# indrajeetadityaroy9/vit-inductive-bias-distillation

Measured on AMD Instinct MI355X. Metric: distillation images/sec (BASD loss fwd+bwd+grad all-reduce), DeiT-S<-ResNet-50 @ bs256/GPU, higher is better.
Workload: dtype f32; 1 GPU; cfg2 DeiT-S<-ResNet-50 224x224; per_gpu_batch=256, global_batch=256, input_dtype=float32, layout=strided (CLS-sliced / channel-major views), backward=True, grad_allreduce_bytes=88202672, grad_allreduce=none at world size 1 (bucket packed, nothing to exchange), rank_readback=auto, readback_deferred_steps=1756, selector=basd_selector_chain mode 0, parallelism=dp1

## Files before the change

### include/basd_hip.h

```cpp
#ifndef BASD_HIP_H
#define BASD_HIP_H

#include <stdint.h>

#ifdef __cplusplus
extern "C" {
#endif

#ifndef __HIP_PLATFORM_AMD__
typedef struct ihipStream_t* hipStream_t;
#endif

#define BASD_OK 0
#define BASD_EINVAL (-1)
#define BASD_EUNSUPPORTED (-2)
#define BASD_DTYPE_F32 0
#define BASD_DTYPE_BF16 1


int basd_gemm_nt(const void* a, int a_dtype, long a_sb, long a_sn, long a_sd, int a_rows_per_batch,
                 long a_batch_stride, const float* b, long ldb, long b_batch_stride, int M, int N, int K, int batch,
                 float* c, long ldc, long c_batch_stride, float scale, const float* bias, float beta,
                 float* colsum_part, float* col_mean, hipStream_t stream);

int basd_gemm_tn_splits(int krows);

int basd_gemm_tn(const void* a, const void* b, int dtype, long a_sb, long a_sn, long a_sd, long a_batch_stride,
                 long b_sb, long b_sn, long b_sd, long b_batch_stride, int rows_per_batch, int krows, int M, int N,
                 int batch, const float* mean_a, const float* mean_b, int splits, float* slabs, float* c, long ldc,
                 long c_batch_stride, float scale, hipStream_t stream);

int basd_colmean_parts(int rows);

int basd_colmean(const void* x, int dtype, long sb, long sn, long sd, int rows_per_batch, long batch_stride,
                 int rows, int cols, int batch, int parts, float* partial, float* mean, hipStream_t stream);

int basd_gemm_tuning(int split_bf16);
int basd_gemm_tuning_get(void);

int basd_colmean_multi(const void* const* x_ptrs, int dtype, long sb, long sn, long sd, int rows_per_batch, int rows,
                       int cols, int n_mats, int parts, float* partial, float* means, int vec_ok,
                       hipStream_t stream);

int basd_syrk_splits(int krows, int cols, int n_mats);

int basd_syrk_multi(const void* const* x_ptrs, int dtype, long sb, long sn, long sd, int rows_per_batch, int krows,
                    int cols, int n_mats, const float* means, const float* scales, int splits, float* slabs,
                    float* out, long out_stride, int vec_ok, const float* fold, int fold_parts, int fold_from,
                    hipStream_t stream);


int basd_jacobi_workspace_ints(int batch, int max_sweeps);
int basd_jacobi_plain4_fits(int n);

int basd_jacobi_tuning(int lanes_per_pair);
int basd_jacobi_ordering(int odd_even);

int basd_jacobi_onesided(float* W, long batch_stride, int rows_dot, int rows_tot, int n, int batch,
                         const int* n_arr, float* colnorm, int colnorm_stride, int max_sweeps, float tol_cos,
                         int* flags, int* sweeps_out, hipStream_t stream);

long basd_jacobi_twopass_workspace_bytes(int n, int batch, int max_sweeps);
int basd_jacobi_stacked_twopass(float* W, long batch_stride, int n, int batch, float* colnorm, int colnorm_stride,
                                int max_sweeps, float tol_cos, void* workspace, int* sweeps_out, hipStream_t stream);

int basd_sort_extract(const float* W, long batch_stride, int rows, int rows_tot, int n, int batch,
                      const float* colnorm, int colnorm_stride, float* vals_desc, float* vecs, int kmax,
                      hipStream_t stream);


long basd_tridiag_workspace_bytes(int n, int batch);

int basd_tridiag(float* a, long a_batch_stride, int n, int batch, float* d, float* e, float* tau, float* vh,
                 void* work, hipStream_t stream);

int basd_tridiag_ranked(float* a, long a_batch_stride, int n, int batch, float* d, float* e, float* tau, float* vh,
                        void* work, int rank_count, double factor, int cap, int* rank_out, int* host_mirror,
                        void* mid_event ,
                        hipStream_t stream);

int basd_tridiag_tuning(int members, int pad, int lag, int threads, int tail, int reset);

int basd_tridiag_eigenvalues(const float* d, const float* e, int n, int batch, float* vals_desc, hipStream_t stream);

int basd_tridiag_apply_q(const float* tau, const float* vh, int n, int k, int batch, const float* x, float* out,
                         int k_stride, int transpose, hipStream_t stream);

int basd_tridiag_shifted_solve(const float* d, const float* e, const float* shifts, int shift_stride, int n, int k,
                               int batch, const float* rhs, float* x, hipStream_t stream);

int basd_tridiag_mp_rank(const float* d, const float* e, int n, int batch, double factor, int cap, int* rank_out,
                         float* thr_out, const int* status, int* host_mirror, hipStream_t stream);

int basd_tridiag_eigenvectors(const float* d, const float* e, const float* tau, const float* vh,
                              const float* vals_desc, int n, int k, int batch, float* z, float* vecs, int k_stride,
                              hipStream_t stream);


int basd_mp_rank(const float* vals_desc, int n, int batch, double factor, int cap, int* rank_out, float* thr_out,
                 hipStream_t stream);

int basd_grassmann_distance(const float* colnorm, int stride, const int* k_arr, const float* sw, int sw_stride,
                            const int* sw_index, int items, float* d_out, float* theta_out, hipStream_t stream);

int basd_grassmann_distance_padded(const float* colnorm, int stride, int n_valid, const int* k_arr, const float* sw,
                                   int sw_stride, const int* sw_index, int items, float* d_out, hipStream_t stream);

int basd_sqrt_clamp(const float* in, float* out, long count, hipStream_t stream);

int basd_gram_finish(const float* c, const float* zbar, int n, int batch, long m_rows, float* out_u, float* out_c,
                     hipStream_t stream);

int basd_selector_tail(const float* t_d, const float* t_e, const float* t_tau, const float* t_vh, const float* t_vals,
                       const float* s_d, const float* s_e, const float* s_tau, const float* s_vh, const float* s_vals,
                       int d_s, int E, int L, int kmax, const int* ranks, const float* proj_s_t, float* z_s,
                       float* v_s, float* z_t, float* u_t, float* u_rot, float* sw, float* cos, int* k_arr,
                       const int* sw_index, float* sigma, int* flags, float* d_out, hipStream_t stream);

int basd_tridiag_mp_rank_rank1(const float* d, const float* e, const float* w, int n, int batch, double rho,
                               double factor, int cap, int* rank_out, const int* status, int* host_mirror,
                               hipStream_t stream);

int basd_tridiag_ranked_gated(float* a, long a_batch_stride, int n, int batch, float* d, float* e, float* tau, float* vh,
                              void* work, int rank_count, double factor, int cap, int* rank_out, int* host_mirror,
                              const unsigned* go_flag, unsigned go_value, int go_budget, hipStream_t stream);
int basd_flag_set(unsigned* flag, unsigned value, hipStream_t stream);

typedef struct BasdSelectorChain {
    const void* const* teacher_host_ptrs;
    long t_dtype, t_sb, t_sn, t_sd;
    const void* const* student_ptrs;
    long s_dtype, s_sb, s_sn, s_sd, s_vec_ok;
    const float* proj_t;
    const float* proj_s_t;
    long E, L, B, n_s, n_t, d_s, d_t;
    double mp_factor;
    long rank_cap;
    long kmax, kmax_cap, mode;
    float* z; float* z_sums; const void* const* z_ptrs; float* z_means; float* t_slabs; long t_splits;
    float* s_partial; float* s_means; float* s_slabs; long s_splits, s_parts;
    float* grams; float* d; float* e; float* tau; float* vh; float* vals; void* tri_work; void* tri_work_s;
    int* ranks; int* host_mirror;
    int* student_status_mirror;
    float* zv; float* vecs; float* u_rot; float* sw; float* cos; float* sigma; float* d_out;
    int* k_arr; const int* sw_index; int* jflags;
    hipStream_t main_stream, chain_stream, student_stream, tail_stream;
    void* ev_fork; void* ev_student; void* ev_ranks; void* ev_tail; void* ev_slot_free; void* ev_tgram; void* ev_tg0;
    long release_delay;
    hipStream_t fact_stream; unsigned* go_flag; long go_value; long go_budget;
    void* tm_proj; void* tm_tgram; void* tm_scol0; void* tm_scol1; void* tm_sgram; void* tm_tri0; void* tm_mid; void* tm_spec;
    hipStream_t cert_stream; int* cert_mirror; void* ev_cert;
    double* cert_scratch;
} BasdSelectorChain;
int basd_selector_chain(const BasdSelectorChain* args);
int basd_rank_certificate(const float* grams, const float* zbar, int n, int batch, double factor, double* scratch,
                          int* flag, hipStream_t stream);
long basd_rank_certificate_scratch_bytes(int batch);
int basd_debug_fill_lds(unsigned pattern, hipStream_t stream);
int basd_selector_chain_tail(const BasdSelectorChain* args, int kmax, int exact_k);
int basd_jacobi_lds_square_fits(int n);


int basd_token_weights(const void* const* attn_ptrs, int dtype, const float* mix, int L, long sb, long sh, long sq,
                       long sk, int B, int H, int A, int has_cls, int n_a, int n_t, int n_s, const int* atap0,
                       const int* atap1, const float* alam, const int* tap0, const int* tap1, const float* lam,
                       float* omega, float* omega_t, float* raw_out, hipStream_t stream);

int basd_student_project(const void* x, int dtype, long sb, long sn, int B, int n_s, int n_t, int D,
                         const float* omega, const int* tap0, const int* tap1, const float* lam, const int* range0,
                         const int* range1, float* mu, float* tr_s, float* a_prime, hipStream_t stream);

int basd_teacher_center(const void* const* tok_ptrs, int dtype, const float* mix, int L, long sb, long sn, long sd,
                        int B, int n, int D, const int* g0, const int* g1, const float* glam, const float* omega_t,
                        float* mu, float* tc, hipStream_t stream);
int basd_teacher_center_multi(const void* const* tok_ptrs, int dtype, const float* mix, int L, int G, long sb, long sn,
                              long sd, int B, int n, int D, const int* g0, const int* g1, const float* glam,
                              const float* omega_t, float* mu, float* tc, hipStream_t stream);
long basd_teacher_center_stream_scratch_floats(int G, int B, int n, int D);
int basd_teacher_center_stream(const void* const* tok_ptrs, int dtype, const float* mix, int L, int G, long sb, long sn,
                               long sd, int B, int n, int D, const int* g0, const int* g1, const float* glam,
                               const float* omega_t, float* mu, float* tc, float* scratch, hipStream_t stream);

int basd_gram_f64(const float* p, long p_batch_stride, int n, int D, int batch, double* g, long g_batch_stride,
                  hipStream_t stream);

int basd_gram_f64_split(const float* p, long p_batch_stride, int n, int D, int batch, int splits, double* slabs,
                        double* g, hipStream_t stream);

int basd_chol_f64(const double* g, long g_batch_stride, int n, int batch, double* l, long l_batch_stride,
                  hipStream_t stream);

int basd_stack_product(const double* la, const double* lb, long l_batch_stride, int n, int batch, int lb_period,
                       float* w, long w_batch_stride, hipStream_t stream);

int basd_procrustes_finalize(const float* w, long w_batch_stride, const float* sigma, int n, int n_s, int batch,
                             int t_period ,
                             const double* gb, long g_batch_stride, const float* omega, const int* tap0,
                             const int* tap1, const float* lam, const float* tr_s_part, int tr_slabs, float* tr_s,
                             float* tr_t, float* nuc, float* loss, float* k_prime, hipStream_t stream);

int basd_student_grad(const void* x, int dtype, long sb, long sn, int B, int n_s, int n_t, int D, const float* omega,
                      const float* mu, const float* h, const int* tap0, const int* tap1, const float* lam,
                      const float* scale_ptr, float scale_const, float* dx, const float* tnorm2, float* gomega,
                      hipStream_t stream);

int basd_student_project_multi(const void* const* x_ptrs, int dtype, long sb, long sn, int E, int B, int n_s, int n_t,
                               int D, int ptrs_16B_aligned, const float* omega, long omega_e_stride, const int* tap0,
                               const int* tap1, const float* lam, const int* range0, const int* range1, float* mu,
                               float* tr_s, float* a_prime, hipStream_t stream);
int basd_student_grad_multi(const void* const* x_ptrs, int dtype, long sb, long sn, int E, int B, int n_s, int n_t,
                            int D, const float* omega, long omega_e_stride, const float* mu, const float* h,
                            const int* tap0, const int* tap1, const float* lam, const float* scale_ptr,
                            float scale_const, float* dx, const float* tnorm2, float* gomega, hipStream_t stream);
int basd_student_grad_fused(const void* const* x_ptrs, int dtype, long sb, long sn, int E, int B, int n_s, int n_t,
                            int D, int ptrs_16B_aligned, const float* omega, long omega_e_stride, const float* mu,
                            const float* k_prime, const float* a_prime, const int* tap0, const int* tap1,
                            const float* lam, const float* scale_ptr, float scale_const, float* dx,
                            hipStream_t stream);

typedef struct BasdProcrustesArgs {
    const void* const* student_ptrs;
    const void* const* student_host_ptrs;
    long s_dtype, s_sb, s_sn, s_aligned;
    const void* const* tok_ptrs;
    long t_dtype, t_sb, t_sn, t_sd;
    const void* const* attn_ptrs;
    long a_dtype, a_sb, a_sh, a_sq, a_sk;
    const float* mix;
    long E, L, G, B, n_s, n_t, d_s, d_t, H, A, has_cls, n_a, n, max_sweeps;
    const int* atap0; const int* atap1; const float* alam;
    const int* tap0; const int* tap1; const float* lam; const int* range0; const int* range1;
    const int* g0; const int* g1; const float* glam;
    float* omega; float* omega_t; float* raw; float* mu_t; float* tc; float* mu_s; float* tr_part; float* tr_s;
    float* a_prime;
    double* g_all; double* l_all;
    float* W; float* sigma; int* jflags; int* sweeps;
    float* tr_t; float* nuc; float* loss_b; float* k_prime;
    float* h; float* dx; const float* grad_layers;
    double* g_slabs; long g_splits;
    const float* uw_ce; float* uw_out;
    void* jac_ws;
    float* w_stack; float* sigma_u;
} BasdProcrustesArgs;
int basd_procrustes_forward_fused(const BasdProcrustesArgs* args, hipStream_t stream);
int basd_procrustes_tuning(int transposed_cores);

int basd_stack_product_t(const double* la, const double* lb, long l_batch_stride, int n, int batch, int lb_period,
                         float* w, long w_batch_stride, hipStream_t stream);
int basd_kprime_from_transposed(const float* w, long w_batch_stride, const float* sigma, int n, int batch,
                                const double* lb, long l_batch_stride, int lb_period, float* z, long z_batch_stride,
                                float* k_prime, hipStream_t stream);
int basd_ustack_stash(const float* wc, long wc_batch_stride, int n, int batch, float* w_stack, long w_stack_stride,
                      hipStream_t stream);
int basd_ustack_from_transposed(const float* x, long x_batch_stride, const float* sigma, int n, int batch,
                                float* w_stack, long w_stack_stride, float* scratch, long scratch_batch_stride,
                                float* sigma_u, int max_sweeps, int* jflags, hipStream_t stream);

int basd_scale_unless_one(float* x, long count, const float* num, const float* den, hipStream_t stream);

int basd_cross_entropy(const void* logits, int dtype, long ld, int B, int C, const long* labels, const float* probs,
                       long pld, float label_smoothing, long ignore_index, float* row_loss, float* dlogits,
                       hipStream_t stream);


int basd_event_create(void** out);
int basd_event_destroy(void* event);
int basd_stream_wait_event(hipStream_t stream, void* event);
int basd_event_record(void* event, hipStream_t stream);
int basd_event_synchronize(void* event);
int basd_event_query(void* event);
int basd_stream_create_priority(void** out, int level);
int basd_event_create_timed(void** out);
int basd_event_elapsed_ms(void* from, void* to, float* ms_out);


int basd_teacher_factor(const float* w, long w_batch_stride, const float* sigma, int n, int n_s, int batch,
                        const double* la, const double* gb, long g_batch_stride, const float* omega,
                        const int* tap0, const int* tap1, const float* lam, const int* range0, const int* range1,
                        float* kt, float* tnorm2, hipStream_t stream);
int basd_teacher_factor_tiled(const float* w, long w_batch_stride, const float* sigma, int n, int n_s, int batch,
                              const double* la, const double* gb, long g_batch_stride, const float* omega,
                              const int* tap0, const int* tap1, const float* lam, const int* range0, const int* range1,
                              float* kt, float* tnorm2, float* z_scratch, hipStream_t stream);

int basd_mix_grad_tokens(const float* r, const void* const* tok_ptrs, int dtype, int L, long sb, long sn, long sd,
                         int E, int B, int n, int D, const int* g0, const int* g1, const float* glam, float* partial,
                         hipStream_t stream);

long basd_mix_grad_tokens_scratch_floats(int E, int B, int L, int n);
int basd_mix_grad_tokens_onepass(const float* r, const void* const* tok_ptrs, int dtype, int L, long sb, long sn, long sd,
                                 int E, int B, int n, int D, const int* g0, const int* g1, const float* glam,
                                 float* partial, float* scratch, hipStream_t stream);

int basd_token_weight_bwd(const float* gomega, const float* raw, int E, int B, int n_a, int n_s, const int* atap0,
                          const int* atap1, const float* alam, const int* arange0, const int* arange1,
                          const void* const* attn_ptrs, int dtype, int L, long sb, long sh, long sq, long sk, int H,
                          int A, int has_cls, float* partial,
                          float* graw_out ,
                          hipStream_t stream);

int basd_build_angle_stack(const float* cos, int kmax, const int* k_arr, int items, float* out, hipStream_t stream);

int basd_grassmann_distance_bwd(const float* stack, const float* colnorm, int kmax, const int* k_arr, const float* sw,
                                int sw_stride, const int* sw_index, const float* gd, int items, float* gwt,
                                hipStream_t stream);

int basd_eigvec_k2(const float* m, const float* lam, int D, int kmax, int batch, float* k2, hipStream_t stream);

int basd_resample_tokens(const void* x, int dtype, long sb, long sn, long sd, int B, int n_in, int n_out, int D,
                         const int* tap0, const int* tap1, const float* lam, float* out, hipStream_t stream);
int basd_resample_tokens_adjoint(const float* dy, int B, int n_in, int n_out, int D, const int* tap0,
                                 const int* tap1, const float* lam, const int* range0, const int* range1, float* dx,
                                 hipStream_t stream);

#ifdef __cplusplus
}
#endif
#endif
```

### vit-inductive-bias-distillation_amd/basd_amd/_lib.py

```python
from __future__ import annotations

import ctypes as C
import os
import threading

_HERE = os.path.dirname(os.path.abspath(__file__))
LIB_PATH = os.path.join(_HERE, "libbasd_hip.so")

vp, i32, i64, f32, f64 = C.c_void_p, C.c_int, C.c_long, C.c_float, C.c_double

SIGNATURES = {
    "basd_gemm_nt": [vp, i32, i64, i64, i64, i32, i64, vp, i64, i64, i32, i32, i32, i32, vp, i64, i64, f32, vp, f32,
                     vp, vp, vp],
    "basd_gemm_tn_splits": [i32],
    "basd_gemm_tn": [vp, vp, i32, i64, i64, i64, i64, i64, i64, i64, i64, i32, i32, i32, i32, i32, vp, vp, i32, vp,
                     vp, i64, i64, f32, vp],
    "basd_colmean_parts": [i32],
    "basd_colmean": [vp, i32, i64, i64, i64, i32, i64, i32, i32, i32, i32, vp, vp, vp],
    "basd_colmean_multi": [vp, i32, i64, i64, i64, i32, i32, i32, i32, i32, vp, vp, i32, vp],
    "basd_syrk_splits": [i32, i32, i32],
    "basd_syrk_multi": [vp, i32, i64, i64, i64, i32, i32, i32, i32, vp, vp, i32, vp, vp, i64, i32, vp, i32, i32, vp],
    "basd_jacobi_workspace_ints": [i32, i32],
    "basd_jacobi_twopass_workspace_bytes": [i32, i32, i32],
    "basd_jacobi_stacked_twopass": [vp, i64, i32, i32, vp, i32, i32, f32, vp, vp, vp],
    "basd_jacobi_tuning": [i32],
    "basd_jacobi_ordering": [i32],
    "basd_gemm_tuning": [i32],
    "basd_gemm_tuning_get": [],
    "basd_jacobi_onesided": [vp, i64, i32, i32, i32, i32, vp, vp, i32, i32, f32, vp, vp, vp],
    "basd_sort_extract": [vp, i64, i32, i32, i32, i32, vp, i32, vp, vp, i32, vp],
    "basd_tridiag_workspace_bytes": [i32, i32],
    "basd_tridiag_tuning": [i32, i32, i32, i32, i32, i32],
    "basd_tridiag": [vp, i64, i32, i32, vp, vp, vp, vp, vp, vp],
    "basd_tridiag_ranked": [vp, i64, i32, i32, vp, vp, vp, vp, vp, i32, f64, i32, vp, vp, vp, vp],
    "basd_tridiag_ranked_gated": [vp, i64, i32, i32, vp, vp, vp, vp, vp, i32, f64, i32, vp, vp, vp, C.c_uint, i32, vp],
    "basd_flag_set": [vp, C.c_uint, vp],
    "basd_scale_unless_one": [vp, i64, vp, vp, vp],
    "basd_event_create": [vp],
    "basd_event_destroy": [vp],
    "basd_stream_wait_event": [vp, vp],
    "basd_tridiag_eigenvalues": [vp, vp, i32, i32, vp, vp],
    "basd_tridiag_apply_q": [vp, vp, i32, i32, i32, vp, vp, i32, i32, vp],
    "basd_tridiag_shifted_solve": [vp, vp, vp, i32, i32, i32, i32, vp, vp, vp],
    "basd_tridiag_mp_rank": [vp, vp, i32, i32, f64, i32, vp, vp, vp, vp, vp],
    "basd_tridiag_mp_rank_rank1": [vp, vp, vp, i32, i32, f64, f64, i32, vp, vp, vp, vp],
    "basd_tridiag_eigenvectors": [vp, vp, vp, vp, vp, i32, i32, i32, vp, vp, i32, vp],
    "basd_mp_rank": [vp, i32, i32, f64, i32, vp, vp, vp],
    "basd_grassmann_distance": [vp, i32, vp, vp, i32, vp, i32, vp, vp, vp],
    "basd_grassmann_distance_padded": [vp, i32, i32, vp, vp, i32, vp, i32, vp, vp],
    "basd_selector_tail": [vp] * 10 + [i32, i32, i32, i32] + [vp] * 14 + [vp],
    "basd_sqrt_clamp": [vp, vp, i64, vp],
    "basd_gram_finish": [vp, vp, i32, i32, i64, vp, vp, vp],
    "basd_cross_entropy": [vp, i32, i64, i32, i32, vp, vp, i64, f32, i64, vp, vp, vp],
    "basd_token_weights": [vp, i32, vp, i32, i64, i64, i64, i64, i32, i32, i32, i32, i32, i32, i32, vp, vp, vp, vp,
                           vp, vp, vp, vp, vp, vp],
    "basd_student_project": [vp, i32, i64, i64, i32, i32, i32, i32, vp, vp, vp, vp, vp, vp, vp, vp, vp, vp],
    "basd_teacher_center": [vp, i32, vp, i32, i64, i64, i64, i32, i32, i32, vp, vp, vp, vp, vp, vp, vp],
    "basd_teacher_center_multi": [vp, i32, vp, i32, i32, i64, i64, i64, i32, i32, i32, vp, vp, vp, vp, vp, vp, vp],
    "basd_teacher_center_stream_scratch_floats": [i32, i32, i32, i32],
    "basd_teacher_center_stream": [vp, i32, vp, i32, i32, i64, i64, i64, i32, i32, i32, vp, vp, vp, vp, vp, vp, vp, vp],
    "basd_gram_f64": [vp, i64, i32, i32, i32, vp, i64, vp],
    "basd_gram_f64_split": [vp, i64, i32, i32, i32, i32, vp, vp, vp],
    "basd_chol_f64": [vp, i64, i32, i32, vp, i64, vp],
    "basd_stack_product": [vp, vp, i64, i32, i32, i32, vp, i64, vp],
    "basd_procrustes_finalize": [vp, i64, vp, i32, i32, i32, i32, vp, i64, vp, vp, vp, vp, vp, i32, vp, vp, vp, vp,
                                 vp, vp],
    "basd_student_project_multi": [vp, i32, i64, i64, i32, i32, i32, i32, i32, i32, vp, i64, vp, vp, vp, vp, vp, vp,
                                   vp, vp, vp],
    "basd_student_grad_multi": [vp, i32, i64, i64, i32, i32, i32, i32, i32, vp, i64, vp, vp, vp, vp, vp, vp, f32, vp,
                                vp, vp, vp],
    "basd_student_grad_fused": [vp, i32, i64, i64, i32, i32, i32, i32, i32, i32, vp, i64, vp, vp, vp, vp, vp, vp, vp,
                                f32, vp, vp],
    "basd_procrustes_forward_fused": [vp, vp],
    "basd_procrustes_tuning": [i32],
    "basd_jacobi_plain4_fits": [i32],
    "basd_stack_product_t": [vp, vp, i64, i32, i32, i32, vp, i64, vp],
    "basd_kprime_from_transposed": [vp, i64, vp, i32, i32, vp, i64, i32, vp, i64, vp, vp],
    "basd_ustack_stash": [vp, i64, i32, i32, vp, i64, vp],
    "basd_ustack_from_transposed": [vp, i64, vp, i32, i32, vp, i64, vp, i64, vp, i32, vp, vp],
    "basd_resample_tokens": [vp, i32, i64, i64, i64, i32, i32, i32, i32, vp, vp, vp, vp, vp],
    "basd_resample_tokens_adjoint": [vp, i32, i32, i32, i32, vp, vp, vp, vp, vp, vp, vp],
    "basd_student_grad": [vp, i32, i64, i64, i32, i32, i32, i32, vp, vp, vp, vp, vp, vp, vp, f32, vp, vp, vp, vp],
    "basd_teacher_factor": [vp, i64, vp, i32, i32, i32, vp, vp, i64, vp, vp, vp, vp, vp, vp, vp, vp, vp],
    "basd_teacher_factor_tiled": [vp, i64, vp, i32, i32, i32, vp, vp, i64, vp, vp, vp, vp, vp, vp, vp, vp, vp, vp],
    "basd_mix_grad_tokens": [vp, vp, i32, i32, i64, i64, i64, i32, i32, i32, i32, vp, vp, vp, vp, vp],
    "basd_mix_grad_tokens_scratch_floats": [i32, i32, i32, i32],
    "basd_mix_grad_tokens_onepass": [vp, vp, i32, i32, i64, i64, i64, i32, i32, i32, i32, vp, vp, vp, vp, vp, vp],
    "basd_token_weight_bwd": [vp, vp, i32, i32, i32, i32, vp, vp, vp, vp, vp, vp, i32, i32, i64, i64, i64, i64, i32,
                              i32, i32, vp, vp, vp],
    "basd_build_angle_stack": [vp, i32, vp, i32, vp, vp],
    "basd_grassmann_distance_bwd": [vp, vp, i32, vp, vp, i32, vp, vp, i32, vp, vp],
    "basd_eigvec_k2": [vp, vp, i32, i32, i32, vp, vp],
    "basd_selector_chain": [vp],
    "basd_rank_certificate": [vp, vp, i32, i32, f64, vp, vp, vp],
    "basd_rank_certificate_scratch_bytes": [i32],
    "basd_debug_fill_lds": [C.c_uint, vp],
    "basd_selector_chain_tail": [vp, i32, i32],
    "basd_jacobi_lds_square_fits": [i32],
    "basd_event_record": [vp, vp],
    "basd_event_synchronize": [vp],
    "basd_event_query": [vp],
    "basd_stream_create_priority": [vp, i32],
    "basd_event_create_timed": [vp],
    "basd_event_elapsed_ms": [vp, vp, vp],
}

class ProcrustesArgs(C.Structure):
    _PTRS = ("student_ptrs", "student_host_ptrs")
    _fields_ = (
        [("student_ptrs", vp), ("student_host_ptrs", vp)]
        + [(n, i64) for n in ("s_dtype", "s_sb", "s_sn", "s_aligned")]
        + [("tok_ptrs", vp)] + [(n, i64) for n in ("t_dtype", "t_sb", "t_sn", "t_sd")]
        + [("attn_ptrs", vp)] + [(n, i64) for n in ("a_dtype", "a_sb", "a_sh", "a_sq", "a_sk")]
        + [("mix", vp)]
        + [(n, i64) for n in ("E", "L", "G", "B", "n_s", "n_t", "d_s", "d_t", "H", "A", "has_cls", "n_a", "n",
                              "max_sweeps")]
        + [(n, vp) for n in ("atap0", "atap1", "alam", "tap0", "tap1", "lam", "range0", "range1", "g0", "g1", "glam",
                             "omega", "omega_t", "raw", "mu_t", "tc", "mu_s", "tr_part", "tr_s", "a_prime", "g_all",
                             "l_all", "W", "sigma", "jflags", "sweeps", "tr_t", "nuc", "loss_b", "k_prime", "h", "dx",
                             "grad_layers", "g_slabs")]
        + [("g_splits", i64)]
        + [("uw_ce", vp), ("uw_out", vp), ("jac_ws", vp), ("w_stack", vp), ("sigma_u", vp)]
    )


class SelectorChainArgs(C.Structure):
    _fields_ = (
        [("teacher_host_ptrs", vp)] + [(n, i64) for n in ("t_dtype", "t_sb", "t_sn", "t_sd")]
        + [("student_ptrs", vp)] + [(n, i64) for n in ("s_dtype", "s_sb", "s_sn", "s_sd", "s_vec_ok")]
        + [("proj_t", vp), ("proj_s_t", vp)]
        + [(n, i64) for n in ("E", "L", "B", "n_s", "n_t", "d_s", "d_t")]
        + [("mp_factor", f64)]
        + [(n, i64) for n in ("rank_cap", "kmax", "kmax_cap", "mode")]
        + [(n, vp) for n in ("z", "z_sums", "z_ptrs", "z_means", "t_slabs")] + [("t_splits", i64)]
        + [(n, vp) for n in ("s_partial", "s_means", "s_slabs")] + [("s_splits", i64), ("s_parts", i64)]
        + [(n, vp) for n in ("grams", "d", "e", "tau", "vh", "vals", "tri_work", "tri_work_s", "ranks", "host_mirror",
                             "student_status_mirror", "zv", "vecs", "u_rot", "sw", "cos", "sigma", "d_out", "k_arr",
                             "sw_index", "jflags", "main_stream", "chain_stream", "student_stream", "tail_stream",
                             "ev_fork", "ev_student", "ev_ranks", "ev_tail", "ev_slot_free", "ev_tgram", "ev_tg0",
                             "release_delay", "fact_stream", "go_flag", "go_value", "go_budget",
                             "tm_proj", "tm_tgram", "tm_scol0", "tm_scol1", "tm_sgram", "tm_tri0", "tm_mid", "tm_spec",
                             "cert_stream", "cert_mirror", "ev_cert", "cert_scratch")]
    )


EINVAL, EUNSUPPORTED = -1, -2

LONG_RESULTS = {"basd_tridiag_workspace_bytes", "basd_jacobi_twopass_workspace_bytes",
                "basd_mix_grad_tokens_scratch_floats", "basd_teacher_center_stream_scratch_floats",
                "basd_rank_certificate_scratch_bytes"}

_lock = threading.Lock()
_lib = None


def load() -> C.CDLL:
    global _lib
    if _lib is not None:
        return _lib
    with _lock:
        if _lib is None:
            if not os.path.exists(LIB_PATH):
                raise RuntimeError(
                    f"{LIB_PATH} not found: build it with `make -C vit-inductive-bias-distillation_amd/csrc` "
                    "(or `python -c 'import __graft_entry__ as g; g.build()'`). There is no CPU fallback.")
            lib = C.CDLL(LIB_PATH)
            for name, argtypes in SIGNATURES.items():
                fn = getattr(lib, name)
                fn.argtypes = argtypes
                fn.restype = C.c_long if name in LONG_RESULTS else C.c_int
            _lib = lib
    return _lib


timing: dict | None = None
timed_names: set | None = None


def call(name: str, *args) -> None:
    if timing is not None and (timed_names is None or name in timed_names):
        import torch
        e0 = torch.cuda.Event(enable_timing=True)
        e1 = torch.cuda.Event(enable_timing=True)
        e0.record()
        status = getattr(load(), name)(*args)
        e1.record()
        timing.setdefault(name, []).append((e0, e1))
    else:
        status = getattr(load(), name)(*args)
    if status != 0:
        kind = "invalid argument / unsupported shape" if status < 0 else "HIP error"
        raise RuntimeError(f"{name} failed with status {status} ({kind})")


def query(name: str, *args) -> int:
    return int(getattr(load(), name)(*args))
```

### vit-inductive-bias-distillation_amd/basd_amd/ops.py

```python
from __future__ import annotations

from dataclasses import dataclass
from functools import lru_cache

import torch

from . import _lib

import os

F32, BF16 = 0, 1
MAX_SWEEPS = 20
TWO_PASS_SVD = True
TRANSPOSED_MIX_GRAD = True
TWO_PASS_LOG_LIMIT = 16 << 30
EIG_SOLVER = os.environ.get("BASD_EIG_SOLVER", "tridiag")
if os.environ.get("BASD_GEMM_SPLIT") in ("0", "1"):
    _lib.call("basd_gemm_tuning", int(os.environ["BASD_GEMM_SPLIT"]))
if os.environ.get("BASD_JACOBI_ORDERING") in ("0", "1"):
    _lib.call("basd_jacobi_ordering", int(os.environ["BASD_JACOBI_ORDERING"]))


def _stream() -> int:
    return torch._C._cuda_getCurrentRawStream(torch._C._cuda_getDevice())


def _dtype_code(t: torch.Tensor) -> int:
    if t.dtype == torch.float32:
        return F32
    if t.dtype == torch.bfloat16:
        return BF16
    raise TypeError(f"unsupported dtype {t.dtype}")


def as_supported(t: torch.Tensor) -> torch.Tensor:
    if t.dtype in (torch.float32, torch.bfloat16):
        return t
    return t.float()


def _require_cuda(*tensors: torch.Tensor) -> None:
    for t in tensors:
        if not t.is_cuda:
            raise RuntimeError("basd_amd kernels need CUDA/HIP tensors (there is no CPU fallback)")


def _ptr(t: torch.Tensor | None) -> int | None:
    return None if t is None else t.data_ptr()


HOST_TRACE: list | None = None
CHAIN_EVENTS: list = []


def trace(label: str) -> None:
    if HOST_TRACE is not None:
        import time
        HOST_TRACE.append((label, time.perf_counter()))


GPU_MARKS: list | None = None


def gpu_mark(label: str) -> None:
    if GPU_MARKS is not None:
        ev = torch.cuda.Event(enable_timing=True)
        ev.record()
        GPU_MARKS.append((label, ev))


def _tok3(x: torch.Tensor) -> tuple[int, int, int, int, int, int]:
    if x.dim() == 2:
        return x.data_ptr(), _dtype_code(x), 0, x.stride(0), x.stride(1), 1 << 30
    assert x.dim() == 3
    return x.data_ptr(), _dtype_code(x), x.stride(0), x.stride(1), x.stride(2), x.shape[1]


def gemm_nt(a: torch.Tensor, b: torch.Tensor, *, scale: float = 1.0, out: torch.Tensor | None = None,
            a_batch_stride: int = 0, b_batch_stride: int = 0, batch: int = 1, rows: int | None = None,
            n_cols: int | None = None, bias: torch.Tensor | None = None, beta: float = 0.0,
            col_mean: bool = False, mean_out: torch.Tensor | None = None, col_sums: torch.Tensor | None = None):
    _require_cuda(a, b)
    ptr, dt, sb, sn, sd, rpb = _tok3(a)
    M = rows if rows is not None else (a.shape[0] * a.shape[1] if a.dim() == 3 else a.shape[0])
    K = a.shape[-1]
    N = n_cols if n_cols is not None else b.shape[-2]
    assert b.dtype == torch.float32 and b.stride(-1) == 1 and b.shape[-1] == K
    ldb = b.stride(-2)
    if out is None:
        out = torch.empty((batch, M, N) if batch > 1 else (M, N), device=a.device, dtype=torch.float32)
    part = mean = None
    tiles = gemm_nt_row_tiles(M, N, K, batch, beta)
    if col_sums is not None:
        assert col_sums.is_contiguous() and col_sums.numel() == batch * tiles * N
        part = col_sums
    if col_mean:
        part = torch.empty((batch, tiles, N), device=a.device, dtype=torch.float32)
        mean = mean_out if mean_out is not None else \
            torch.empty((batch, N) if batch > 1 else (N,), device=a.device, dtype=torch.float32)
        assert mean.dtype == torch.float32 and mean.is_contiguous() and mean.numel() == batch * N
    _lib.call("basd_gemm_nt", ptr, dt, sb, sn, sd, rpb, a_batch_stride, b.data_ptr(), ldb, b_batch_stride,
              M, N, K, batch, out.data_ptr(), N, M * N, scale, _ptr(bias), beta, _ptr(part), _ptr(mean), _stream())
    return (out, mean) if col_mean else out


def gemm_nt_row_tiles(M: int, N: int, K: int, batch: int = 1, beta: float = 0.0) -> int:
    return (M + 127) // 128


def gemm_tn(a: torch.Tensor, b: torch.Tensor, *, mean_a: torch.Tensor | None = None,
            mean_b: torch.Tensor | None = None, scale: float = 1.0, batch: int = 1, a_batch_stride: int = 0,
            b_batch_stride: int = 0, krows: int | None = None, m_cols: int | None = None,
            n_cols: int | None = None, split: bool = True) -> torch.Tensor:
    _require_cuda(a, b)
    pa, dt, asb, asn, asd, rpb = _tok3(a)
    pb, dtb, bsb, bsn, bsd, rpb_b = _tok3(b)
    assert dt == dtb and rpb == rpb_b
    kr = krows if krows is not None else (a.shape[0] * a.shape[1] if a.dim() == 3 else a.shape[0])
    M = m_cols if m_cols is not None else a.shape[-1]
    N = n_cols if n_cols is not None else b.shape[-1]
    splits = _lib.query("basd_gemm_tn_splits", kr) if (split and batch == 1) else 1
    out = torch.empty((batch, M, N) if batch > 1 else (M, N), device=a.device, dtype=torch.float32)
    slabs = torch.empty((batch * splits, M, N), device=a.device, dtype=torch.float32) if splits > 1 else None
    _lib.call("basd_gemm_tn", pa, pb, dt, asb, asn, asd, a_batch_stride, bsb, bsn, bsd, b_batch_stride, rpb, kr, M, N,
              batch, _ptr(mean_a), _ptr(mean_b), splits, _ptr(slabs), out.data_ptr(), N, M * N, scale, _stream())
    return out


def colmean(x: torch.Tensor) -> torch.Tensor:
    _require_cuda(x)
    ptr, dt, sb, sn, sd, rpb = _tok3(x)
    rows = x.shape[0] * x.shape[1] if x.dim() == 3 else x.shape[0]
    cols = x.shape[-1]
    parts = _lib.query("basd_colmean_parts", rows)
    partial = torch.empty((parts, cols), device=x.device, dtype=torch.float32)
    mean = torch.empty((cols,), device=x.device, dtype=torch.float32)
    _lib.call("basd_colmean", ptr, dt, sb, sn, sd, rpb, 0, rows, cols, 1, parts, partial.data_ptr(),
              mean.data_ptr(), _stream())
    return mean


def _gram_layout(xs: list[torch.Tensor]):
    _require_cuda(*xs)
    ptr, dt, sb, sn, sd, rpb = _tok3(xs[0])
    for x in xs[1:]:
        assert _tok3(x)[1:] == (dt, sb, sn, sd, rpb) and x.shape == xs[0].shape, "Gram operands must share a layout"
    rows = xs[0].shape[0] * xs[0].shape[1] if xs[0].dim() == 3 else xs[0].shape[0]
    vec_ok = int(all(x.data_ptr() % 16 == 0 for x in xs))
    return (dt, sb, sn, sd, rpb), rows, xs[0].shape[-1], vec_ok


_COLMEAN_SCRATCH: dict = {}


def column_means(xs: list[torch.Tensor], out: torch.Tensor | None = None) -> torch.Tensor:
    (dt, sb, sn, sd, rpb), rows, cols, vec_ok = _gram_layout(xs)
    n, dev = len(xs), xs[0].device
    table = _ptr_table(xs)
    if out is None:
        means = torch.empty((n, cols), device=dev, dtype=torch.float32)
    else:
        assert out.dtype == torch.float32 and out.is_contiguous() and out.numel() == n * cols and out.device == dev
        means = out
    parts = _lib.query("basd_colmean_parts", rows)
    key = (n, parts, cols, dev, _stream())
    partial = _COLMEAN_SCRATCH.get(key)
    if partial is None:
        if len(_COLMEAN_SCRATCH) >= 16:
            _COLMEAN_SCRATCH.clear()
        partial = _COLMEAN_SCRATCH[key] = torch.empty((n, parts, cols), device=dev, dtype=torch.float32)
    _lib.call("basd_colmean_multi", table.data_ptr(), dt, sb, sn, sd, rpb, rows, cols, n, parts, partial.data_ptr(),
              means.data_ptr(), vec_ok, _stream())
    return means.view(n, cols)


def centered_grams(xs: list[torch.Tensor], *, centered: list[bool] | None = None,
                   scales: list[float] | None = None, out: torch.Tensor | None = None,
                   splits: int | None = None, means: torch.Tensor | None = None,
                   fold: tuple[torch.Tensor, int] | None = None) -> tuple[torch.Tensor, torch.Tensor]:
    (dt, sb, sn, sd, rpb), rows, cols, vec_ok = _gram_layout(xs)
    n, dev = len(xs), xs[0].device
    table = _ptr_table(xs)
    if fold is not None:
        part, fold_from = fold
        assert part.is_contiguous() and part.dtype == torch.float32 and part.shape[0] == n - fold_from
        means_used = None
        centered = None
    elif means is None:
        means = column_means(xs)
    if fold is not None:
        pass
    elif centered is not None and not all(centered):
        keep = _device_consts(tuple(1.0 if c else 0.0 for c in centered), torch.float32, dev)
        means_used = means * keep.unsqueeze(1)
    else:
        means_used = means
    sc = None
    if scales is not None:
        sc = _device_consts(tuple(float(s) for s in scales), torch.float32, dev)
    if splits is None:
        splits = _lib.query("basd_syrk_splits", rows, cols, n)
    slabs = torch.empty((n * splits, cols, cols), device=dev, dtype=torch.float32)
    if out is None:
        out = torch.empty((n, cols, cols), device=dev, dtype=torch.float32)
    assert out.dtype == torch.float32 and out.shape == (n, cols, cols) and out[0].is_contiguous()
    _lib.call("basd_syrk_multi", table.data_ptr(), dt, sb, sn, sd, rpb, rows, cols, n, _ptr(means_used),
              _ptr(sc), splits, slabs.data_ptr(), out.data_ptr(), out.stride(0), vec_ok,
              _ptr(fold[0]) if fold is not None else None, fold[0].shape[1] if fold is not None else 0,
              fold[1] if fold is not None else 0, _stream())
    return out, means


def jacobi_onesided(W: torch.Tensor, rows_dot: int, *, n_arr: torch.Tensor | None = None,
                    want_sweeps: bool = False, tol: float = 0.0):
    _require_cuda(W)
    assert W.dtype == torch.float32 and W.is_contiguous() and W.dim() == 3
    batch, n, rows_tot = W.shape
    colnorm = torch.empty((batch, n), device=W.device, dtype=torch.float32)
    flags = torch.empty((_lib.query("basd_jacobi_workspace_ints", batch, MAX_SWEEPS),), device=W.device,
                        dtype=torch.int32)
    sweeps = torch.zeros((batch,), device=W.device, dtype=torch.int32) if want_sweeps else None
    _lib.call("basd_jacobi_onesided", W.data_ptr(), n * rows_tot, rows_dot, rows_tot, n, batch, _ptr(n_arr),
              colnorm.data_ptr(), n, MAX_SWEEPS, tol, flags.data_ptr(), _ptr(sweeps), _stream())
    return (colnorm, sweeps) if want_sweeps else colnorm


def sym_eig(G: torch.Tensor, kmax: int = 0) -> tuple[torch.Tensor, torch.Tensor | None, torch.Tensor, torch.Tensor]:
    assert G.dim() == 3 and G.shape[1] == G.shape[2]
    colnorm = jacobi_onesided(G, G.shape[1])
    vals, vecs = sort_extract(G, colnorm, kmax)
    return vals, vecs, G, colnorm


@dataclass
class TridiagState:
    d: torch.Tensor
    e: torch.Tensor
    tau: torch.Tensor
    vh: torch.Tensor
    vals: torch.Tensor
    err: torch.Tensor | None = None
    ranks: torch.Tensor | None = None


def tridiag_slice(ts: TridiagState, first: int, count: int) -> TridiagState:
    sl = slice(first, first + count)
    return TridiagState(ts.d[sl], ts.e[sl], ts.tau[sl], ts.vh[sl], ts.vals[sl], ts.err, None)


def tridiagonalise(G: torch.Tensor, mp_rank: tuple | None = None) -> TridiagState:
    _require_cuda(G)
    assert G.dtype == torch.float32 and G.is_contiguous() and G.dim() == 3 and G.shape[1] == G.shape[2]
    batch, n, _ = G.shape
    f32 = dict(device=G.device, dtype=torch.float32)
    d, e, tau = (torch.empty((batch, n), **f32) for _ in range(3))
    vh = torch.empty((batch, n, n), **f32)
    vals = torch.empty((batch, n), **f32)
    work = torch.empty((_lib.query("basd_tridiag_workspace_bytes", n, batch),), device=G.device, dtype=torch.uint8)
    ranks = None
    if mp_rank is None:
        _lib.call("basd_tridiag", G.data_ptr(), n * n, n, batch, d.data_ptr(), e.data_ptr(), tau.data_ptr(),
                  vh.data_ptr(), work.data_ptr(), _stream())
    else:
        M, D, cap, count, mirror, mid_event = (tuple(mp_rank) + (None,))[:6]
        factor = (1 + (D / M) ** 0.5) ** 2
        ranks = torch.empty((count,), device=G.device, dtype=torch.int32)
        if mirror is not None:
            assert mirror.is_pinned() and mirror.dtype == torch.int32 and mirror.numel() == count + 8
        _lib.call("basd_tridiag_ranked", G.data_ptr(), n * n, n, batch, d.data_ptr(), e.data_ptr(), tau.data_ptr(),
                  vh.data_ptr(), work.data_ptr(), count, factor, cap, ranks.data_ptr(), _ptr(mirror), mid_event,
                  _stream())
    return TridiagState(d, e, tau, vh, vals, work[-32:].view(torch.int32), ranks)


def new_event() -> int:
    import ctypes
    h = ctypes.c_void_p()
    _lib.call("basd_event_create", ctypes.byref(h))
    return h.value


def stream_wait_event(stream: "torch.cuda.Stream", event: int) -> None:
    _lib.call("basd_stream_wait_event", stream.cuda_stream, event)


def tridiag_spectrum(ts: TridiagState, first: int = 0, count: int | None = None) -> torch.Tensor:
    batch, n = ts.vals.shape
    count = batch - first if count is None else count
    _lib.call("basd_tridiag_eigenvalues", ts.d[first].data_ptr(), ts.e[first].data_ptr(), n, count,
              ts.vals[first].data_ptr(), _stream())
    return ts.vals[first:first + count]


def tridiag_mp_rank(ts: TridiagState, M: int, D: int, cap: int, first: int = 0, count: int | None = None,
                    host_mirror: torch.Tensor | None = None) -> torch.Tensor:
    batch, n = ts.vals.shape
    count = batch - first if count is None else count
    factor = (1 + (D / M) ** 0.5) ** 2
    out = torch.empty((count,), device=ts.d.device, dtype=torch.int32)
    if host_mirror is not None:
        assert host_mirror.is_pinned() and host_mirror.dtype == torch.int32 and host_mirror.numel() == count + 8
    _lib.call("basd_tridiag_mp_rank", ts.d[first].data_ptr(), ts.e[first].data_ptr(), n, count, factor, cap,
              out.data_ptr(), None, _ptr(ts.err) if host_mirror is not None else None, _ptr(host_mirror), _stream())
    return out


def tridiag_mp_rank_rank1(ts: TridiagState, w: torch.Tensor, M: int, D: int, cap: int,
                          host_mirror: torch.Tensor | None = None) -> torch.Tensor:
    batch, n = ts.d.shape
    assert w.dtype == torch.float32 and w.is_contiguous() and w.numel() == batch * n
    factor = (1 + (D / M) ** 0.5) ** 2
    out = torch.empty((batch,), device=ts.d.device, dtype=torch.int32)
    if host_mirror is not None:
        assert host_mirror.is_pinned() and host_mirror.dtype == torch.int32 and host_mirror.numel() == batch + 8
    _lib.call("basd_tridiag_mp_rank_rank1", ts.d.data_ptr(), ts.e.data_ptr(), w.data_ptr(), n, batch, float(M), factor,
              cap, out.data_ptr(), _ptr(ts.err) if host_mirror is not None else None, _ptr(host_mirror), _stream())
    return out


def tridiag_eigenvalues(G: torch.Tensor) -> TridiagState:
    ts = tridiagonalise(G)
    tridiag_spectrum(ts)
    return ts
# ... 468 lines not shown
```

### vit-inductive-bias-distillation_amd/csrc/basd_common.h

```cpp
#pragma once
#include <hip/hip_runtime.h>
#include <hip/hip_bf16.h>
#include <stdint.h>

#define BASD_OK 0
#define BASD_EINVAL (-1)
#define BASD_EUNSUPPORTED (-2)

#define BASD_DTYPE_F32 0
#define BASD_DTYPE_BF16 1

#define BASD_CHECK_ARG(cond) \
    do {                     \
        if (!(cond)) return BASD_EINVAL; \
    } while (0)

#define BASD_RETURN_LAST()                         \
    do {                                           \
        hipError_t e_ = hipGetLastError();         \
        return e_ == hipSuccess ? BASD_OK : (int)e_; \
    } while (0)

namespace basd {

constexpr int kWave = 64;

__device__ __forceinline__ float to_f32(float x) { return x; }
__device__ __forceinline__ float to_f32(__hip_bfloat16 x) { return __bfloat162float(x); }
#define BASD_GLOBAL_AS __attribute__((address_space(1)))
__device__ __forceinline__ float ldg_f32(const BASD_GLOBAL_AS float* p) { return *p; }
__device__ __forceinline__ float ldg_f32(const BASD_GLOBAL_AS __hip_bfloat16* p) {
    return __uint_as_float((unsigned)*(const BASD_GLOBAL_AS unsigned short*)p << 16);
}

template <typename T>
__device__ __forceinline__ T group_sum(T v, int width) {
    for (int m = width >> 1; m > 0; m >>= 1) v += __shfl_xor(v, m, width);
    return v;
}

template <int CTRL>
__device__ __forceinline__ float dpp_get(float x) {
    return __int_as_float(__builtin_amdgcn_update_dpp(0, __float_as_int(x), CTRL, 0xF, 0xF, true));
}
__device__ __forceinline__ float row16_allsum(float x) {
    x += dpp_get<0xB1>(x);
    x += dpp_get<0x4E>(x);
    x += dpp_get<0x141>(x);
    x += dpp_get<0x140>(x);
    return x;
}
__device__ __forceinline__ float wave64_allsum(float x) {
    x = row16_allsum(x);
    auto r = __builtin_amdgcn_permlane16_swap(__float_as_uint(x), __float_as_uint(x), false, false);
    x = __uint_as_float(r[0]) + __uint_as_float(r[1]);
    auto q = __builtin_amdgcn_permlane32_swap(__float_as_uint(x), __float_as_uint(x), false, false);
    return __uint_as_float(q[0]) + __uint_as_float(q[1]);
}

__device__ __forceinline__ float wave_sum(float v) { return wave64_allsum(v); }
__device__ __forceinline__ int wave_sum(int v) { return group_sum(v, kWave); }
__device__ __forceinline__ double wave_sum(double v) { return group_sum(v, kWave); }

__device__ __forceinline__ float wave_max(float v) {
    for (int m = 32; m > 0; m >>= 1) v = fmaxf(v, __shfl_xor(v, m, kWave));
    return v;
}

template <typename T>
__device__ __forceinline__ T block_sum(T v, T* scratch) {
    const int lane = threadIdx.x & 63, wid = threadIdx.x >> 6, nw = (blockDim.x + 63) >> 6;
    v = wave_sum(v);
    __syncthreads();
    if (lane == 0) scratch[wid] = v;
    __syncthreads();
    T r = T(0);
    for (int i = 0; i < nw; ++i) r += scratch[i];
    return r;
}

struct TokView {
    const void* ptr;
    long sb, sn, sd;
    int n_tok;
};

__host__ __device__ __forceinline__ long tok_row_offset(const TokView& v, long m) {
    const long b = m / v.n_tok, n = m - b * v.n_tok;
    return b * v.sb + n * v.sn;
}

__host__ __device__ __forceinline__ void rr_pair(int n_even, int r, int t, int& p, int& q) {
    const int m = n_even - 1;
    if (t == 0) { p = r; q = m; return; }
    p = (r + t) % m;
    q = (r - t + m) % m;
}

}
```

### vit-inductive-bias-distillation_amd/csrc/fused.hip

```cpp
#include "basd_common.h"
#include "../../include/basd_hip.h"

namespace basd {

__global__ void __launch_bounds__(256) uwso_combine_kernel(const float* __restrict__ ce, const float* __restrict__ loss_b,
                                                           int E, int B, float* __restrict__ out) {
    constexpr int CH = 32;
    __shared__ double red[CH][4];
    const int tid = threadIdx.x;
    double geo_sum = 0.;
    for (int e0 = 0; e0 < E; e0 += CH) {
        const int ne = E - e0 < CH ? E - e0 : CH;
        for (int e = 0; e < ne; ++e) {
            double acc = 0.;
            for (int b = tid; b < B; b += 256) acc += (double)loss_b[(long)(e0 + e) * B + b];
            for (int m = 32; m > 0; m >>= 1) acc += __shfl_xor(acc, m, 64);
            if ((tid & 63) == 0) red[e][tid >> 6] = acc;
        }
        __syncthreads();
        if (tid == 0)
            for (int e = 0; e < ne; ++e) {
                const float layer = (float)(((red[e][0] + red[e][1]) + (red[e][2] + red[e][3])) / (double)B);
                out[4 + E + e0 + e] = layer;
                geo_sum += (double)layer;
            }
        __syncthreads();
    }
    if (tid == 0) {
        const float c = ce[0], geo = (float)(geo_sum / (double)E);
        const float eps = 1.1920929e-7f;
        const float i0 = 1.f / fmaxf(c, eps), i1 = 1.f / fmaxf(geo, eps);
        const float w0 = i0 / (i0 + i1), w1 = i1 / (i0 + i1);
        out[0] = w0;
        out[1] = w1;
        out[2] = w0 * c + w1 * geo;
        out[3] = geo;
        for (int e = 0; e < E; ++e) out[4 + e] = w1 / (float)E;
    }
}

__global__ void __launch_bounds__(256) scale_unless_one_kernel(float* __restrict__ x, long count4, long count,
                                                               const float* __restrict__ num,
                                                               const float* __restrict__ den) {
    const float f = den ? num[0] / den[0] : num[0];
    if (f == 1.f) return;
    const long i = (long)blockIdx.x * 256 + threadIdx.x;
    if (i < count4) {
        float4 v = ((float4*)x)[i];
        v.x *= f; v.y *= f; v.z *= f; v.w *= f;
        ((float4*)x)[i] = v;
    }
    if (blockIdx.x == 0 && threadIdx.x < (int)(count - 4 * count4)) x[4 * count4 + threadIdx.x] *= f;
}

}

extern "C" {

int basd_scale_unless_one(float* x, long count, const float* num, const float* den, hipStream_t stream) {
    BASD_CHECK_ARG(x && num && count > 0 && ((uintptr_t)x & 15) == 0);
    const long count4 = count / 4;
    basd::scale_unless_one_kernel<<<(unsigned)((count4 + 255) / 256 + (count4 == 0)), 256, 0, stream>>>(x, count4, count, num, den);
    BASD_RETURN_LAST();
}

static int procrustes_tail(const BasdProcrustesArgs* a, const float* grad_layers, int E, int B, int n_s, int n, int d_s,
                           int EB, long nn, long om_stride, hipStream_t st) {
    int rc;
#define BASD_TRY(call)            \
    do {                          \
        rc = (call);              \
        if (rc != BASD_OK) return rc; \
    } while (0)
    if (a->uw_ce) {
        BASD_CHECK_ARG(a->uw_out != nullptr);
        basd::uwso_combine_kernel<<<1, 256, 0, st>>>(a->uw_ce, a->loss_b, E, B, a->uw_out);
        grad_layers = a->uw_out + 4;
    }
    if (a->dx) {
        BASD_CHECK_ARG(a->k_prime && a->h && grad_layers);
        rc = basd_student_grad_fused(a->student_ptrs, (int)a->s_dtype, a->s_sb, a->s_sn, E, B, n_s, n, d_s,
                                     (int)a->s_aligned, a->omega, om_stride, a->mu_s, a->k_prime, a->a_prime, a->tap0,
                                     a->tap1, a->lam, grad_layers, 2.0f / (float)B, a->dx, st);
        if (rc != BASD_EUNSUPPORTED) return rc;
        BASD_TRY(basd_gemm_tn(a->k_prime, a->a_prime, BASD_DTYPE_F32, 0, n, 1, nn, 0, d_s, 1, (long)n * d_s, 1 << 30, n,
                              n, d_s, EB, nullptr, nullptr, 1, nullptr, a->h, d_s, (long)n * d_s, 1.f, st));
        BASD_TRY(basd_student_grad_multi(a->student_ptrs, (int)a->s_dtype, a->s_sb, a->s_sn, E, B, n_s, n, d_s, a->omega,
                                         om_stride, a->mu_s, a->h, a->tap0, a->tap1, a->lam, grad_layers,
                                         2.0f / (float)B, a->dx, nullptr, nullptr, st));
    }
#undef BASD_TRY
    return BASD_OK;
}

static int g_transposed_cores = 1;
int basd_procrustes_tuning(int transposed_cores) {
    if (transposed_cores >= 0) g_transposed_cores = transposed_cores > 2 ? 2 : transposed_cores;
    return BASD_OK;
}

int basd_procrustes_forward_fused(const BasdProcrustesArgs* a, hipStream_t st) {
    BASD_CHECK_ARG(a && a->student_ptrs && a->tok_ptrs && a->attn_ptrs && a->mix);
    const int E = (int)a->E, L = (int)a->L, G = (int)a->G, B = (int)a->B, n_s = (int)a->n_s, n_t = (int)a->n_t;
    const int d_s = (int)a->d_s, d_t = (int)a->d_t, H = (int)a->H, A = (int)a->A, n_a = (int)a->n_a, n = (int)a->n;
    const float* grad_layers_in = a->grad_layers;
    BASD_CHECK_ARG(E > 0 && L > 0 && (G == 1 || G == E) && B > 0 && n == (n_s < n_t ? n_s : n_t));
    int rc;
#define BASD_TRY(call)            \
    do {                          \
        rc = (call);              \
        if (rc != BASD_OK) return rc; \
    } while (0)
    int centred = BASD_EUNSUPPORTED;
    for (int g = 0; g < G; ++g) {
        BASD_TRY(basd_token_weights(a->attn_ptrs, (int)a->a_dtype, a->mix + (long)g * L, L, a->a_sb, a->a_sh, a->a_sq,
                                    a->a_sk, B, H, A, (int)a->has_cls, n_a, n, n_s, a->atap0, a->atap1, a->alam,
                                    a->tap0, a->tap1, a->lam, a->omega + (long)g * B * n_s,
                                    a->omega_t + (long)g * B * n, a->raw ? a->raw + (long)g * B * n_a : nullptr, st));
    }
    if (G > 1 && L >= 4 && basd_teacher_center_stream_scratch_floats(G, B, n, d_t) <= (long)E * B * 2 * n * n) {
        centred = basd_teacher_center_stream(a->tok_ptrs, (int)a->t_dtype, a->mix, L, G, a->t_sb, a->t_sn, a->t_sd, B, n,
                                             d_t, a->g0, a->g1, a->glam, a->omega_t, a->mu_t, a->tc, a->W, st);
        if (centred != BASD_OK && centred != BASD_EUNSUPPORTED) return centred;
    }
    if (G > 1 && centred != BASD_OK) {
        centred = basd_teacher_center_multi(a->tok_ptrs, (int)a->t_dtype, a->mix, L, G, a->t_sb, a->t_sn, a->t_sd, B, n,
                                            d_t, a->g0, a->g1, a->glam, a->omega_t, a->mu_t, a->tc, st);
        if (centred != BASD_OK && centred != BASD_EUNSUPPORTED) return centred;
    }
    for (int g = 0; g < G && centred != BASD_OK; ++g) {
        BASD_TRY(basd_teacher_center(a->tok_ptrs, (int)a->t_dtype, a->mix + (long)g * L, L, a->t_sb, a->t_sn, a->t_sd,
                                     B, n, d_t, a->g0, a->g1, a->glam, a->omega_t + (long)g * B * n,
                                     a->mu_t + (long)g * B * d_t, a->tc + (long)g * B * n * d_t, st));
    }
    const long om_stride = G == 1 ? 0 : (long)B * n_s;
    int slabs = (d_s + 31) / 32;
    rc = basd_student_project_multi(a->student_ptrs, (int)a->s_dtype, a->s_sb, a->s_sn, E, B, n_s, n, d_s,
                                    (int)a->s_aligned, a->omega, om_stride, a->tap0, a->tap1, a->lam, a->range0,
                                    a->range1, a->mu_s, a->tr_part, a->a_prime, st);
    if (rc == BASD_EUNSUPPORTED) {
        slabs = (d_s + 63) / 64;
        for (int e = 0; e < E; ++e)
            BASD_TRY(basd_student_project(a->student_host_ptrs[e], (int)a->s_dtype, a->s_sb, a->s_sn, B, n_s, n, d_s,
                                          a->omega + e * om_stride, a->tap0, a->tap1, a->lam, a->range0, a->range1,
                                          a->mu_s + (long)e * B * d_s, a->tr_part + (long)e * B * slabs,
                                          a->a_prime + (long)e * B * n * d_s, st));
    } else if (rc != BASD_OK) {
        return rc;
    }
    const long nn = (long)n * n;
    const int EB = E * B, GB = G * B;
    BASD_TRY(basd_gram_f64(a->a_prime, (long)n * d_s, n, d_s, EB, a->g_all, nn, st));
    if (a->g_slabs && a->g_splits > 1)
        BASD_TRY(basd_gram_f64_split(a->tc, (long)n * d_t, n, d_t, GB, (int)a->g_splits, a->g_slabs,
                                     a->g_all + (long)EB * nn, st));
    else
        BASD_TRY(basd_gram_f64(a->tc, (long)n * d_t, n, d_t, GB, a->g_all + (long)EB * nn, nn, st));
    BASD_TRY(basd_chol_f64(a->g_all, nn, n, EB + GB, a->l_all, nn, st));
    if ((a->raw == nullptr || a->w_stack != nullptr) && EB <= 65535 && basd_jacobi_plain4_fits(n) &&
        (g_transposed_cores == 2 || (g_transposed_cores == 1 && EB >= 128))) {
        BASD_TRY(basd_stack_product_t(a->l_all, a->l_all + (long)EB * nn, nn, n, EB, GB, a->W, 2 * nn, st));
        if (a->raw != nullptr) BASD_TRY(basd_ustack_stash(a->W, 2 * nn, n, EB, a->w_stack, 2 * nn, st));
        BASD_TRY(basd_jacobi_onesided(a->W, 2 * nn, n, n, n, EB, nullptr, a->sigma, n, (int)a->max_sweeps, 0.f,
                                      a->jflags, a->sweeps, st));
        BASD_TRY(basd_procrustes_finalize(a->W, 2 * nn, a->sigma, n, n_s, EB, GB, a->g_all + (long)EB * nn, nn, a->omega,
                                          a->tap0, a->tap1, a->lam, a->tr_part, slabs, a->tr_s, a->tr_t, a->nuc,
                                          a->loss_b, nullptr, st));
        if (a->k_prime)
            BASD_TRY(basd_kprime_from_transposed(a->W, 2 * nn, a->sigma, n, EB, a->l_all + (long)EB * nn, nn, GB,
                                                 a->W + nn, 2 * nn, a->k_prime, st));
        if (a->raw != nullptr) {
            BASD_CHECK_ARG(a->sigma_u != nullptr);
            BASD_TRY(basd_ustack_from_transposed(a->W, 2 * nn, a->sigma, n, EB, a->w_stack, 2 * nn, a->W + nn, 2 * nn,
                                                 a->sigma_u, (int)a->max_sweeps, a->jflags, st));
        }
        return procrustes_tail(a, grad_layers_in, E, B, n_s, n, d_s, EB, nn, om_stride, st);
    }
    BASD_TRY(basd_stack_product(a->l_all, a->l_all + (long)EB * nn, nn, n, EB, GB, a->W, 2 * nn, st));
    rc = BASD_EUNSUPPORTED;
    if (a->jac_ws)
        rc = basd_jacobi_stacked_twopass(a->W, 2 * nn, n, EB, a->sigma, n, (int)a->max_sweeps, 0.f, a->jac_ws, a->sweeps,
                                         st);
    if (rc == BASD_EUNSUPPORTED)
        rc = basd_jacobi_onesided(a->W, 2 * nn, n, 2 * n, n, EB, nullptr, a->sigma, n, (int)a->max_sweeps, 0.f,
                                  a->jflags, a->sweeps, st);
    if (rc != BASD_OK) return rc;
    BASD_TRY(basd_procrustes_finalize(a->W, 2 * nn, a->sigma, n, n_s, EB, GB, a->g_all + (long)EB * nn, nn, a->omega,
                                      a->tap0, a->tap1, a->lam, a->tr_part, slabs, a->tr_s, a->tr_t, a->nuc,
                                      a->loss_b, a->k_prime, st));
    return procrustes_tail(a, grad_layers_in, E, B, n_s, n, d_s, EB, nn, om_stride, st);
#undef BASD_TRY
}


int basd_event_create(void** out) {
    BASD_CHECK_ARG(out);
    hipError_t e = hipEventCreateWithFlags((hipEvent_t*)out, hipEventDisableTiming);
    return e == hipSuccess ? BASD_OK : (int)e;
}
int basd_event_destroy(void* ev) {
    hipError_t e = hipEventDestroy((hipEvent_t)ev);
    return e == hipSuccess ? BASD_OK : (int)e;
}
int basd_stream_wait_event(hipStream_t stream, void* ev) {
    BASD_CHECK_ARG(ev);
    hipError_t e = hipStreamWaitEvent(stream, (hipEvent_t)ev, 0);
    return e == hipSuccess ? BASD_OK : (int)e;
}

}
```

### vit-inductive-bias-distillation_amd/csrc/jacobi.hip

```cpp
#include "basd_common.h"

namespace basd {

constexpr float kNull2 = 2.2737368e-13f;

struct Rot {
    float c, s, t;
    float h;
    bool apply;
    bool strong;
};

__device__ __forceinline__ Rot make_rotation(float alpha, float beta, float gamma, float tol) {
    Rot r{1.f, 0.f, 0.f, 0.f, false, false};
    const float cosv = gamma * __builtin_amdgcn_rsqf(alpha) * __builtin_amdgcn_rsqf(beta);
    if (!(fabsf(cosv) > tol)) return r;
    r.strong = cosv * cosv > tol;
    const float zeta = (beta - alpha) * __builtin_amdgcn_rcpf(2.f * gamma);
    const float az = fabsf(zeta);
    float t = az > 1e8f ? 0.5f * __builtin_amdgcn_rcpf(az)
                        : __builtin_amdgcn_rcpf(az + __builtin_amdgcn_sqrtf(fmaf(zeta, zeta, 1.f)));
    t = copysignf(t, zeta);
    r.t = t;
    r.c = __builtin_amdgcn_rsqf(fmaf(t, t, 1.f));
    r.s = r.c * t;
    const float pc = r.c * r.c, ec = fmaf(r.c, r.c, -pc);
    const float ps = r.s * r.s, es = fmaf(r.s, r.s, -ps);
    r.h = 0.5f * ((((1.f - pc) - ps) - ec) - es);
    r.apply = true;
    return r;
}

template <int LPP>
__device__ __forceinline__ float pair_allsum(float x) {
    static_assert(LPP == 4 || LPP == 8 || LPP == 16 || LPP == 32 || LPP == 64,
                  "a pair is owned by a quad, half a DPP row, a row, two rows or a wave");
    if constexpr (LPP == 4 || LPP == 8) {
        x += dpp_get<0xB1>(x);
        x += dpp_get<0x4E>(x);
        if constexpr (LPP == 8) x += dpp_get<0x141>(x);
        return x;
    } else if constexpr (LPP == 32) {
        x = row16_allsum(x);
        auto r = __builtin_amdgcn_permlane16_swap(__float_as_uint(x), __float_as_uint(x), false, false);
        return __uint_as_float(r[0]) + __uint_as_float(r[1]);
    } else {
        return LPP == 16 ? row16_allsum(x) : wave64_allsum(x);
    }
}

typedef float f32x2 __attribute__((ext_vector_type(2)));

template <int EPL, int DOT, int LPP, bool LOG = false>
__device__ __forceinline__ int rotate_pair(float* __restrict__ cp, float* __restrict__ cq, int gl, float tol,
                                            float null2, float& norm2_max, float* __restrict__ n2p,
                                            float* __restrict__ n2q, float* __restrict__ devp,
                                            float* __restrict__ devq, f32x2* __restrict__ logp = nullptr) {
    static_assert(EPL % 2 == 0 && DOT % 2 == 0, "row chunks come in pairs");
    constexpr int H = EPL / 2, HD = DOT / 2;
    f32x2 x[HD], y[HD];
    f32x2 acc = {0.f, 0.f};
#pragma unroll
    for (int i = 0; i < HD; ++i) {
        x[i] = *(const f32x2*)(cp + 2 * gl + 2 * LPP * i);
        y[i] = *(const f32x2*)(cq + 2 * gl + 2 * LPP * i);
        acc = __builtin_elementwise_fma(x[i], y[i], acc);
    }
    const float g = pair_allsum<LPP>(acc.x + acc.y);
    const float a = *n2p, b = *n2q;
    norm2_max = fmaxf(norm2_max, fmaxf(a, b));
    if (fminf(a, b) <= null2) {
        if (LOG && gl == 0) *logp = f32x2{1.f, 0.f};
        return 0;
    }
    const Rot rot = make_rotation(a, b, g, tol);
    if (!rot.apply) {
        if (LOG && gl == 0) *logp = f32x2{1.f, 0.f};
        return 0;
    }
    const f32x2 c2 = {rot.c, rot.c}, s2 = {rot.s, rot.s};
#pragma unroll
    for (int i = 0; i < HD; ++i) {
        *(f32x2*)(cp + 2 * gl + 2 * LPP * i) = __builtin_elementwise_fma(c2, x[i], -(s2 * y[i]));
        *(f32x2*)(cq + 2 * gl + 2 * LPP * i) = __builtin_elementwise_fma(s2, x[i], c2 * y[i]);
    }
#pragma unroll
    for (int i = HD; i < H; ++i) {
        const f32x2 xr = *(const f32x2*)(cp + 2 * gl + 2 * LPP * i);
        const f32x2 yr = *(const f32x2*)(cq + 2 * gl + 2 * LPP * i);
        *(f32x2*)(cp + 2 * gl + 2 * LPP * i) = __builtin_elementwise_fma(c2, xr, -(s2 * yr));
        *(f32x2*)(cq + 2 * gl + 2 * LPP * i) = __builtin_elementwise_fma(s2, xr, c2 * yr);
    }
    if (gl == 0) {
        *n2p = fmaxf(a - rot.t * g, 0.f);
        *n2q = b + rot.t * g;
        *devp += rot.h;
        *devq += rot.h;
        if (LOG) *logp = f32x2{rot.c, rot.s};
    }
    return rot.strong ? 3 : 1;
}

template <int DOT, int LPP>
__device__ __forceinline__ float column_norm2(const float* __restrict__ col, int gl) {
    f32x2 acc = {0.f, 0.f};
#pragma unroll
    for (int i = 0; i < DOT / 2; ++i) {
        const f32x2 v = *(const f32x2*)(col + 2 * gl + 2 * LPP * i);
        acc = __builtin_elementwise_fma(v, v, acc);
    }
    return pair_allsum<LPP>(acc.x + acc.y);
}

template <int EPL, int DOT, int LPP>
__device__ __forceinline__ int lds_row(int r, int rows_dot) {
    return (DOT == EPL || r < rows_dot) ? r : LPP * DOT + (r - rows_dot);
}

template <int EPL, int DOT, int LPP = 16>
__global__ void __launch_bounds__((LPP == 4 && EPL >= 48) ? 512 : 1024) jacobi_lds_kernel(float* __restrict__ W, long batch_stride, int rows_dot,
                                                           int rows_tot, int n_fixed, const int* __restrict__ n_arr,
                                                           int max_sweeps, float tol, float* __restrict__ colnorm,
                                                           int colnorm_stride, int* __restrict__ sweeps_out) {
    constexpr int LD = LPP * EPL + (LPP == 4 ? (((LPP * EPL / 8) % 2 == 0) ? 8 : 0) : LPP == 8 ? 16 : 2);
    static_assert(LPP != 4 || ((LD / 8) % 2 == 1 && LD % 8 == 0), "stride must come out as 8 x odd");
    static_assert(LPP != 8 || ((LPP * EPL / 16) % 2 == 0), "stride must come out as 16 x odd");
    extern __shared__ __attribute__((aligned(16))) float lds[];
    const int m = blockIdx.x;
    int n = n_arr ? n_arr[m] : n_fixed;
    int rd = rows_dot, rt = rows_tot;
    if (n_arr) {
        rd = n;
        rt = n;
    }
    float* Wm = W + (long)m * batch_stride;
    const int tid = threadIdx.x, nthr = blockDim.x;
    if (n <= 0) {
        if (sweeps_out && tid == 0) sweeps_out[m] = 0;
        return;
    }
    const int n_even = (n + 1) & ~1;
    for (int idx = tid; idx < n_even * LD; idx += nthr) lds[idx] = 0.f;
    __syncthreads();
    for (int idx = tid; idx < n * rt; idx += nthr) {
        const int c = idx / rt, r = idx - c * rt;
        lds[c * LD + lds_row<EPL, DOT, LPP>(r, rd)] = Wm[(long)c * rows_tot + r];
    }
    __syncthreads();

    const int groups = nthr / LPP, grp = tid / LPP, gl = tid % LPP;
    float* n2 = lds + n_even * LD;
    float* dev = n2 + n_even;
    __shared__ int s_norm2_bits;
    if (tid == 0) s_norm2_bits = 0;
    for (int c = tid; c < n_even; c += nthr) dev[c] = 0.f;
    float null2 = 0.f;
    int sweep = 0;
    for (; sweep < max_sweeps && n > 1; ++sweep) {
        int rotated = 0;
        float norm2_max = 0.f;
        for (int c = grp; c < n_even; c += groups) {
            const float v = column_norm2<DOT, LPP>(lds + c * LD, gl);
            if (gl == 0) n2[c] = v;
        }
        __syncthreads();
        for (int r = 0; r < n_even - 1; ++r) {
            for (int t = grp; t < n_even / 2; t += groups) {
                int p, q;
                rr_pair(n_even, r, t, p, q);
                if (p >= n || q >= n) continue;
                if (p > q) { const int tmp = p; p = q; q = tmp; }
                rotated |= rotate_pair<EPL, DOT, LPP>(lds + p * LD, lds + q * LD, gl, tol, null2, norm2_max, n2 + p, n2 + q,
                                                 dev + p, dev + q);
            }
            __syncthreads();
        }
        if (gl == 0 && norm2_max > 0.f) atomicMax(&s_norm2_bits, __float_as_int(norm2_max));
        if (!__syncthreads_or(rotated & 2)) {
            ++sweep;
            break;
        }
        null2 = kNull2 * __int_as_float(s_norm2_bits);
    }
    if (sweeps_out && tid == 0) sweeps_out[m] = sweep;

    for (int c = grp; c < n; c += groups) {
        const float a = column_norm2<DOT, LPP>(lds + c * LD, gl);
        if (gl == 0) {
            const float nv = sqrtf(a);
            colnorm[(long)m * colnorm_stride + c] = fmaf(nv, dev[c], nv);
        }
    }
    for (int idx = tid; idx < n * rt; idx += nthr) {
        const int c = idx / rt, r = idx - c * rt;
        const float v = lds[c * LD + lds_row<EPL, DOT, LPP>(r, rd)];
        Wm[(long)c * rows_tot + r] = fmaf(v, dev[c], v);
    }
}

template <int H>
__device__ __forceinline__ int rotate_regs(f32x2 (&x)[H], f32x2 (&y)[H], float& a, float& b, float& dx, float& dy,
                                           float tol, float null2, float& norm2_max, bool forced) {
    f32x2 acc = {0.f, 0.f};
#pragma unroll
    for (int i = 0; i < H; ++i) acc = __builtin_elementwise_fma(x[i], y[i], acc);
    const float g = pair_allsum<4>(acc.x + acc.y);
    norm2_max = fmaxf(norm2_max, fmaxf(a, b));
    Rot rot{1.f, 0.f, 0.f, 0.f, false, false};
    if (fminf(a, b) > null2) rot = make_rotation(a, b, g, tol);
    float c = rot.c, s = rot.s;
    if (forced) { c = 0.f; s = 1.f; }
    if (rot.apply || forced) {
        const f32x2 c2 = {c, c}, s2 = {s, s};
#pragma unroll
        for (int i = 0; i < H; ++i) {
            const f32x2 xi = x[i], yi = y[i];
            x[i] = __builtin_elementwise_fma(c2, xi, -(s2 * yi));
            y[i] = __builtin_elementwise_fma(s2, xi, c2 * yi);
        }
    }
    if (forced) {
        b = a; a = 0.f; dy = dx; dx = 0.f;
    } else if (rot.apply) {
        a = fmaxf(a - rot.t * g, 0.f);
        b = b + rot.t * g;
        dx += rot.h;
        dy += rot.h;
    }
    return rot.strong ? 3 : (rot.apply ? 1 : 0);
}

template <int EPL>
__global__ void __launch_bounds__(512, 4) jacobi_oe_kernel(float* __restrict__ W, long batch_stride, int rows, int n,
                                                           int max_sweeps, float tol, float* __restrict__ colnorm,
                                                           int colnorm_stride, int* __restrict__ sweeps_out) {
    static_assert(EPL % 2 == 0, "row chunks come in pairs");
    constexpr int H = EPL / 2;
    constexpr int LD = 4 * EPL + (((4 * EPL / 8) % 2 == 0) ? 8 : 0);
    extern __shared__ __attribute__((aligned(16))) float lds[];
    const int m = blockIdx.x, tid = threadIdx.x, nthr = blockDim.x;
    const int n_even = (n + 1) & ~1, G = n_even / 2;
    float* mail_n2 = lds + (G + 1) * LD;
    float* mail_dev = mail_n2 + (G + 1);
    __shared__ int s_norm2_bits;
    float* Wm = W + (long)m * batch_stride;
    const int g = tid >> 2, gl = tid & 3;
    const bool active = g < G, last = g == G - 1;
    for (int idx = tid; idx < (G + 1) * (LD + 2); idx += nthr) lds[idx] = 0.f;
    if (tid == 0) s_norm2_bits = 0;

    f32x2 x[H], y[H];
    float a = 0.f, b = 0.f, dx = 0.f, dy = 0.f;
#pragma unroll
    for (int i = 0; i < H; ++i) {
        const int r = 2 * gl + 8 * i;
        const int cx = 2 * g, cy = 2 * g + 1;
        x[i].x = (active && cx < n && r < rows) ? Wm[(long)cx * rows + r] : 0.f;
        x[i].y = (active && cx < n && r + 1 < rows) ? Wm[(long)cx * rows + r + 1] : 0.f;
        y[i].x = (active && cy < n && r < rows) ? Wm[(long)cy * rows + r] : 0.f;
        y[i].y = (active && cy < n && r + 1 < rows) ? Wm[(long)cy * rows + r + 1] : 0.f;
    }
    float* slot_lo = lds + (active ? g : 0) * LD + 2 * gl;
    float* slot_hi = lds + (active ? g + 1 : 0) * LD + 2 * gl;
    __syncthreads();

    float null2 = 0.f;
    int sweep = 0;
    for (; sweep < max_sweeps && n > 1; ++sweep) {
        int rotated = 0;
        float norm2_max = 0.f;
        if (active) {
            f32x2 sa = {0.f, 0.f}, sb = {0.f, 0.f};
#pragma unroll
            for (int i = 0; i < H; ++i) {
                sa = __builtin_elementwise_fma(x[i], x[i], sa);
                sb = __builtin_elementwise_fma(y[i], y[i], sb);
            }
            a = pair_allsum<4>(sa.x + sa.y);
            b = pair_allsum<4>(sb.x + sb.y);
        }
        for (int dr = 0; dr < G; ++dr) {
            if (active) {
                rotated |= rotate_regs<H>(x, y, a, b, dx, dy, tol, null2, norm2_max, false);
#pragma unroll
                for (int i = 0; i < H; ++i) *(f32x2*)(slot_lo + 8 * i) = y[i];
                if (gl == 0) { mail_n2[g] = b; mail_dev[g] = dy; }
            }
            __syncthreads();
            if (active) {
#pragma unroll
                for (int i = 0; i < H; ++i) y[i] = *(const f32x2*)(slot_hi + 8 * i);
                b = mail_n2[g + 1];
                dy = mail_dev[g + 1];
                rotated |= rotate_regs<H>(x, y, a, b, dx, dy, tol, null2, norm2_max, last);
                if (!last) {
#pragma unroll
                    for (int i = 0; i < H; ++i) *(f32x2*)(slot_hi + 8 * i) = x[i];
                    if (gl == 0) { mail_n2[g + 1] = a; mail_dev[g + 1] = dx; }
                }
            }
            __syncthreads();
            if (active) {
#pragma unroll
                for (int i = 0; i < H; ++i) x[i] = *(const f32x2*)(slot_lo + 8 * i);
                a = mail_n2[g];
                dx = mail_dev[g];
            }
        }
        if (active && gl == 0 && norm2_max > 0.f) atomicMax(&s_norm2_bits, __float_as_int(norm2_max));
        if (!__syncthreads_or(rotated & 2)) {
            ++sweep;
            break;
        }
        null2 = kNull2 * __int_as_float(s_norm2_bits);
    }
    if (sweeps_out && tid == 0) sweeps_out[m] = sweep;
    if (!active) return;

    f32x2 sa = {0.f, 0.f}, sb = {0.f, 0.f};
#pragma unroll
    for (int i = 0; i < H; ++i) {
        sa = __builtin_elementwise_fma(x[i], x[i], sa);
        sb = __builtin_elementwise_fma(y[i], y[i], sb);
    }
    const float na = sqrtf(pair_allsum<4>(sa.x + sa.y)), nb = sqrtf(pair_allsum<4>(sb.x + sb.y));
    const bool rev = sweep & 1;
    const int cx = rev ? n_even - 1 - 2 * g : 2 * g, cy = rev ? n_even - 2 - 2 * g : 2 * g + 1;
    if (gl == 0) {
        if (cx < n) colnorm[(long)m * colnorm_stride + cx] = fmaf(na, dx, na);
        if (cy < n) colnorm[(long)m * colnorm_stride + cy] = fmaf(nb, dy, nb);
    }
#pragma unroll
    for (int i = 0; i < H; ++i) {
        const int r = 2 * gl + 8 * i;
        if (cx < n && r < rows) Wm[(long)cx * rows + r] = fmaf(x[i].x, dx, x[i].x);
        if (cx < n && r + 1 < rows) Wm[(long)cx * rows + r + 1] = fmaf(x[i].y, dx, x[i].y);
        if (cy < n && r < rows) Wm[(long)cy * rows + r] = fmaf(y[i].x, dy, y[i].x);
        if (cy < n && r + 1 < rows) Wm[(long)cy * rows + r + 1] = fmaf(y[i].y, dy, y[i].y);
    }
}

template <int EPL>
struct TwoPassShape {
    static constexpr int LPP = 4;
    static constexpr int LD = LPP * EPL + (((LPP * EPL / 8) % 2 == 0) ? 8 : 0);
    static_assert((LD / 8) % 2 == 1 && LD % 8 == 0, "stride must come out as 8 x odd");
};

template <int EPL>
__global__ void __launch_bounds__(512) jacobi_top_logged_kernel(float* __restrict__ W, long batch_stride, int ld, int n,
                                                                int max_sweeps, float tol, float* __restrict__ colnorm,
                                                                int colnorm_stride, f32x2* __restrict__ rotlog,
                                                                long log_stride, float* __restrict__ dev_out,
                                                                int* __restrict__ sweeps_out) {
    constexpr int LPP = TwoPassShape<EPL>::LPP, LD = TwoPassShape<EPL>::LD;
    extern __shared__ __attribute__((aligned(16))) float lds[];
    const int m = blockIdx.x, tid = threadIdx.x, nthr = blockDim.x;
    float* Wm = W + (long)m * batch_stride;
    f32x2* logm = rotlog + (long)m * log_stride;
    const int n_even = (n + 1) & ~1;
    for (int idx = tid; idx < n_even * LD; idx += nthr) lds[idx] = 0.f;
    __syncthreads();
    for (int idx = tid; idx < n * n; idx += nthr) {
        const int c = idx / n, r = idx - c * n;
        lds[c * LD + r] = Wm[(long)c * ld + r];
    }
    __syncthreads();
    const int groups = nthr / LPP, grp = tid / LPP, gl = tid % LPP;
    float* n2 = lds + n_even * LD;
    float* dev = n2 + n_even;
    __shared__ int s_norm2_bits;
    if (tid == 0) s_norm2_bits = 0;
    for (int c = tid; c < n_even; c += nthr) dev[c] = 0.f;
    float null2 = 0.f;
    int sweep = 0;
    const int pairs = n_even / 2;
    for (; sweep < max_sweeps && n > 1; ++sweep) {
        int rotated = 0;
        float norm2_max = 0.f;
        for (int c = grp; c < n_even; c += groups) {
            const float v = column_norm2<EPL, LPP>(lds + c * LD, gl);
            if (gl == 0) n2[c] = v;
        }
        __syncthreads();
        for (int r = 0; r < n_even - 1; ++r) {
            f32x2* logr = logm + ((long)sweep * (n_even - 1) + r) * pairs;
            for (int t = grp; t < pairs; t += groups) {
                int p, q;
                rr_pair(n_even, r, t, p, q);
                if (p >= n || q >= n) {
                    if (gl == 0) logr[t] = f32x2{1.f, 0.f};
                    continue;
                }
                if (p > q) { const int tmp = p; p = q; q = tmp; }
                rotated |= rotate_pair<EPL, EPL, LPP, true>(lds + p * LD, lds + q * LD, gl, tol, null2, norm2_max, n2 + p,
                                                            n2 + q, dev + p, dev + q, logr + t);
            }
            __syncthreads();
        }
        if (gl == 0 && norm2_max > 0.f) atomicMax(&s_norm2_bits, __float_as_int(norm2_max));
        if (!__syncthreads_or(rotated & 2)) {
            ++sweep;
            break;
        }
        null2 = kNull2 * __int_as_float(s_norm2_bits);
    }
    if (tid == 0) sweeps_out[m] = sweep;
    for (int c = grp; c < n; c += groups) {
        const float a = column_norm2<EPL, LPP>(lds + c * LD, gl);
        if (gl == 0) {
            const float nv = sqrtf(a);
            colnorm[(long)m * colnorm_stride + c] = fmaf(nv, dev[c], nv);
            dev_out[(long)m * n + c] = dev[c];
        }
    }
    for (int idx = tid; idx < n * n; idx += nthr) {
        const int c = idx / n, r = idx - c * n;
        const float v = lds[c * LD + r];
        Wm[(long)c * ld + r] = fmaf(v, dev[c], v);
    }
}

template <int EPL>
__global__ void __launch_bounds__(512) jacobi_apply_log_kernel(float* __restrict__ W, long batch_stride, int ld, int row0,
                                                               int n, const f32x2* __restrict__ rotlog, long log_stride,
                                                               const float* __restrict__ dev_in,
                                                               const int* __restrict__ sweeps) {
    constexpr int LPP = TwoPassShape<EPL>::LPP, LD = TwoPassShape<EPL>::LD, H = EPL / 2;
    extern __shared__ __attribute__((aligned(16))) float lds[];
    const int m = blockIdx.x, tid = threadIdx.x, nthr = blockDim.x;
    const int r_lo = blockIdx.y * LPP * EPL, rows = n - r_lo < LPP * EPL ? n - r_lo : LPP * EPL;
    float* Wm = W + (long)m * batch_stride + row0 + r_lo;
    const f32x2* logm = rotlog + (long)m * log_stride;
    const int n_even = (n + 1) & ~1, pairs = n_even / 2;
    for (int idx = tid; idx < n_even * LD; idx += nthr) lds[idx] = 0.f;
    __syncthreads();
    for (int idx = tid; idx < n * rows; idx += nthr) {
        const int c = idx / rows, r = idx - c * rows;
        lds[c * LD + r] = Wm[(long)c * ld + r];
    }
    __syncthreads();
    const int grp = tid / LPP, gl = tid % LPP;
    const long steps = (long)sweeps[m] * (n_even - 1);
    const bool seat = grp < pairs;
    const f32x2 ident = {1.f, 0.f};
    f32x2 cs0 = seat && steps > 0 ? logm[grp] : ident;
    f32x2 cs1 = seat && steps > 1 ? logm[pairs + grp] : ident;
    for (long st = 0; st < steps; ++st) {
        const f32x2 cs2 = seat && st + 2 < steps ? logm[(st + 2) * pairs + grp] : ident;
        const int r = (int)(st % (n_even - 1));
        if (seat && (cs0.y != 0.f || cs0.x != 1.f)) {
            int p, q;
            rr_pair(n_even, r, grp, p, q);
            if (p > q) { const int tmp = p; p = q; q = tmp; }
            float* cp = lds + p * LD;
            float* cq = lds + q * LD;
            const f32x2 c2 = {cs0.x, cs0.x}, s2 = {cs0.y, cs0.y};
#pragma unroll
            for (int i = 0; i < H; ++i) {
                const f32x2 xr = *(const f32x2*)(cp + 2 * gl + 2 * LPP * i);
                const f32x2 yr = *(const f32x2*)(cq + 2 * gl + 2 * LPP * i);
                *(f32x2*)(cp + 2 * gl + 2 * LPP * i) = __builtin_elementwise_fma(c2, xr, -(s2 * yr));
                *(f32x2*)(cq + 2 * gl + 2 * LPP * i) = __builtin_elementwise_fma(s2, xr, c2 * yr);
            }
        }
        __syncthreads();
        cs0 = cs1;
        cs1 = cs2;
    }
    const float* dv = dev_in + (long)m * n;
    for (int idx = tid; idx < n * rows; idx += nthr) {
        const int c = idx / rows, r = idx - c * rows;
        const float v = lds[c * LD + r];
        Wm[(long)c * ld + r] = fmaf(v, dv[c], v);
    }
}

template <int EPL, int DOT, int LPP>
__global__ void __launch_bounds__(1024) jacobi_block_round_kernel(float* __restrict__ W, long batch_stride,
                                                                  int rows_dot, int rows_tot, int n, int nblk, int BW,
                                                                  int round, int sweep, int max_sweeps,
                                                                  float tol, int* __restrict__ flags,
                                                                  int* __restrict__ norm2_bits) {
    constexpr int LD = LPP * EPL + 2;
    extern __shared__ __attribute__((aligned(16))) float lds[];
    const int m = blockIdx.y;
    if (sweep > 0 && flags[m * max_sweeps + sweep - 1] == 0) return;
    const float null2 = sweep > 0 ? kNull2 * __int_as_float(norm2_bits[m * max_sweeps + sweep - 1]) : 0.f;
    float norm2_max = 0.f;
    int bi, bj;
    rr_pair(nblk, round, blockIdx.x, bi, bj);
    if (bi > bj) { const int t = bi; bi = bj; bj = t; }
    float* Wm = W + (long)m * batch_stride;
    const int tid = threadIdx.x;
    const int grp = tid / LPP, gl = tid % LPP;

    const int NT = LPP * BW;
    const bool padded = rows_tot != LPP * EPL || (bi + 1) * BW > n || (bj + 1) * BW > n;
    if (padded) {
        for (int idx = tid; idx < 2 * BW * LD; idx += NT) lds[idx] = 0.f;
        __syncthreads();
    }
    const bool vec4 = (rows_tot & 3) == 0 && (batch_stride & 3) == 0 && (((uintptr_t)W) & 15) == 0;
    if (vec4) {
        const int q4 = rows_tot >> 2, total4 = 2 * BW * q4;
#pragma unroll 4
        for (int idx = tid; idx < total4; idx += NT) {
            const int lc = idx / q4, r = (idx - lc * q4) << 2;
            const int gc = (lc < BW ? bi * BW + lc : bj * BW + (lc - BW));
            if (gc < n) {
                const float4 v = *(const float4*)(Wm + (long)gc * rows_tot + r);
                float* col = lds + lc * LD;
                col[lds_row<EPL, DOT, LPP>(r, rows_dot)] = v.x;
                col[lds_row<EPL, DOT, LPP>(r + 1, rows_dot)] = v.y;
                col[lds_row<EPL, DOT, LPP>(r + 2, rows_dot)] = v.z;
                col[lds_row<EPL, DOT, LPP>(r + 3, rows_dot)] = v.w;
            }
        }
    } else {
#pragma unroll 4
        for (int idx = tid; idx < 2 * BW * rows_tot; idx += NT) {
            const int lc = idx / rows_tot, r = idx - lc * rows_tot;
            const int gc = (lc < BW ? bi * BW + lc : bj * BW + (lc - BW));
            if (gc < n) lds[lc * LD + lds_row<EPL, DOT, LPP>(r, rows_dot)] = Wm[(long)gc * rows_tot + r];
        }
    }
    float* n2 = lds + 2 * BW * LD;
    float* dev = n2 + 2 * BW;
    __syncthreads();
    for (int c = grp; c < 2 * BW; c += BW) {
        const float v = column_norm2<DOT, LPP>(lds + c * LD, gl);
        if (gl == 0) { n2[c] = v; dev[c] = 0.f; }
    }
    __syncthreads();

    int rotated = 0;
    if (round == 0) {
        const int half = grp / (BW / 2), t = grp % (BW / 2), base = half * BW;
        for (int r = 0; r < BW - 1; ++r) {
            int p, q;
            rr_pair(BW, r, t, p, q);
            if (p > q) { const int tmp = p; p = q; q = tmp; }
            const int gp = (half ? bj : bi) * BW + p, gq = (half ? bj : bi) * BW + q;
            if (gp < n && gq < n)
                rotated |= rotate_pair<EPL, DOT, LPP>(lds + (base + p) * LD, lds + (base + q) * LD, gl, tol, null2, norm2_max,
                                                 n2 + base + p, n2 + base + q, dev + base + p, dev + base + q);
            __syncthreads();
        }
    }
    for (int r = 0; r < BW; ++r) {
        const int p = grp, q = (grp + r) % BW;
        const int gp = bi * BW + p, gq = bj * BW + q;
        if (gp < n && gq < n)
            rotated |= rotate_pair<EPL, DOT, LPP>(lds + p * LD, lds + (BW + q) * LD, gl, tol, null2, norm2_max, n2 + p,
                                             n2 + BW + q, dev + p, dev + BW + q);
        __syncthreads();
    }
    if (gl == 0 && norm2_max > 0.f) atomicMax(&norm2_bits[m * max_sweeps + sweep], __float_as_int(norm2_max));
    if (__syncthreads_or(rotated & 2) && tid == 0) atomicOr(&flags[m * max_sweeps + sweep], 1);

    if (vec4) {
        const int q4 = rows_tot >> 2, total4 = 2 * BW * q4;
#pragma unroll 4
        for (int idx = tid; idx < total4; idx += NT) {
            const int lc = idx / q4, r = (idx - lc * q4) << 2;
            const int gc = (lc < BW ? bi * BW + lc : bj * BW + (lc - BW));
            if (gc < n) {
                const float* col = lds + lc * LD;
                const float dv = dev[lc];
                float4 v;
                v.x = col[lds_row<EPL, DOT, LPP>(r, rows_dot)];
                v.y = col[lds_row<EPL, DOT, LPP>(r + 1, rows_dot)];
                v.z = col[lds_row<EPL, DOT, LPP>(r + 2, rows_dot)];
                v.w = col[lds_row<EPL, DOT, LPP>(r + 3, rows_dot)];
                v.x = fmaf(v.x, dv, v.x); v.y = fmaf(v.y, dv, v.y); v.z = fmaf(v.z, dv, v.z); v.w = fmaf(v.w, dv, v.w);
                *(float4*)(Wm + (long)gc * rows_tot + r) = v;
            }
        }
    } else {
#pragma unroll 4
        for (int idx = tid; idx < 2 * BW * rows_tot; idx += NT) {
            const int lc = idx / rows_tot, r = idx - lc * rows_tot;
            const int gc = (lc < BW ? bi * BW + lc : bj * BW + (lc - BW));
            if (gc < n) {
                const float v = lds[lc * LD + lds_row<EPL, DOT, LPP>(r, rows_dot)];
                Wm[(long)gc * rows_tot + r] = fmaf(v, dev[lc], v);
            }
        }
    }
}

__global__ void block_sweeps_kernel(const int* __restrict__ flags, int batch, int max_sweeps, int* __restrict__ sweeps_out) {
    const int m = blockIdx.x * 256 + threadIdx.x;
    if (m >= batch) return;
    int s = 0;
    while (s < max_sweeps && flags[m * max_sweeps + s] != 0) ++s;
    sweeps_out[m] = s < max_sweeps ? s + 1 : max_sweeps;
}

__global__ void colnorm_kernel(const float* __restrict__ W, long batch_stride, int rows_dot, int rows_tot, int n,
                               float* __restrict__ colnorm, int colnorm_stride) {
    const int m = blockIdx.y, c = blockIdx.x * 4 + (threadIdx.x >> 6), lane = threadIdx.x & 63;
    if (c >= n) return;
    const float* col = W + (long)m * batch_stride + (long)c * rows_tot;
    float a = 0.f;
    for (int r = lane; r < rows_dot; r += 64) a = fmaf(col[r], col[r], a);
    a = wave_sum(a);
    if (lane == 0) colnorm[(long)m * colnorm_stride + c] = sqrtf(a);
}

__global__ void __launch_bounds__(256) sort_extract_kernel(const float* __restrict__ W, long batch_stride, int rows,
                                                            int rows_tot, int n, const float* __restrict__ colnorm,
                                                            int colnorm_stride, float* __restrict__ vals_desc,
                                                            float* __restrict__ vecs, int kmax) {
    __shared__ float key[1024];
    __shared__ int idx[1024];
    const int m = blockIdx.x, tid = threadIdx.x;
    int np2 = 1;
    while (np2 < n) np2 <<= 1;
    for (int i = tid; i < np2; i += 256) {
        key[i] = i < n ? colnorm[(long)m * colnorm_stride + i] : -1.f;
        idx[i] = i;
    }
    __syncthreads();
    for (int k = 2; k <= np2; k <<= 1) {
        for (int j = k >> 1; j > 0; j >>= 1) {
            for (int i = tid; i < np2; i += 256) {
                const int l = i ^ j;
                if (l > i) {
                    const bool desc = (i & k) == 0;
                    const float a = key[i], b = key[l];
                    const bool a_first = a > b || (a == b && idx[i] < idx[l]);
                    if (desc ? !a_first : a_first) {
                        key[i] = b; key[l] = a;
                        const int t = idx[i]; idx[i] = idx[l]; idx[l] = t;
                    }
                }
            }
            __syncthreads();
        }
    }
    for (int i = tid; i < n; i += 256) vals_desc[(long)m * n + i] = key[i];
    if (vecs) {
        const int kk = kmax < n ? kmax : n;
        const float* Wm = W + (long)m * batch_stride;
        for (int e = tid; e < kk * rows; e += 256) {
            const int i = e / rows, r = e - i * rows;
            const float nv = key[i];
            vecs[((long)m * kmax + i) * rows + r] = nv > 0.f ? Wm[(long)idx[i] * rows_tot + r] / nv : 0.f;
        }
    }
}

}

using namespace basd;


extern "C" {

#define BASD_JACOBI_LDS_LIMIT (156 * 1024)

int basd_jacobi_workspace_ints(int batch, int max_sweeps) { return 2 * batch * max_sweeps; }

static inline size_t plain4_ld(int e) { return 4 * (size_t)e + (((4 * e / 8) % 2 == 0) ? 8 : 0); }
int basd_jacobi_plain4_fits(int n) {
    const int n_even = (n + 1) & ~1;
    if (n_even < 40 || n > 200) return 0;
    static const int p_epl[] = {8, 16, 24, 36, 50};
    for (int e : p_epl)
        if (4 * e >= n) return (size_t)n_even * (plain4_ld(e) + 2) * sizeof(float) <= BASD_JACOBI_LDS_LIMIT;
    return 0;
}

int basd_jacobi_lds_square_fits(int n) {
    if (n < 1) return 0;
    const int n_even = (n + 1) & ~1, epl = (n + 15) / 16;
    static const int lds_epl[] = {2, 4, 6, 8, 12, 16, 20};
    for (int e : lds_epl)
        if (e >= epl) return (size_t)n_even * (16 * e + 4) * sizeof(float) <= BASD_JACOBI_LDS_LIMIT;
    return 0;
}

static int g_jacobi_lanes = 0;
int basd_jacobi_tuning(int lanes_per_pair) {
    if (lanes_per_pair != 0 && lanes_per_pair != 4 && lanes_per_pair != 8 && lanes_per_pair != 16) return BASD_EINVAL;
    g_jacobi_lanes = lanes_per_pair;
    return BASD_OK;
}

static int g_jacobi_ordering = 1;
int basd_jacobi_ordering(int odd_even) {
    if (odd_even != 0 && odd_even != 1) return BASD_EINVAL;
    g_jacobi_ordering = odd_even;
    return BASD_OK;
}

int basd_jacobi_onesided(float* W, long batch_stride, int rows_dot, int rows_tot, int n, int batch,
                         const int* n_arr, float* colnorm, int colnorm_stride, int max_sweeps, float tol_cos,
                         int* flags, int* sweeps_out, hipStream_t stream) {
    BASD_CHECK_ARG(W && colnorm && rows_dot > 0 && rows_tot >= rows_dot && n > 0 && batch > 0 && max_sweeps > 0);
    const float tol = tol_cos > 0.f ? tol_cos : 1.2e-7f * sqrtf((float)rows_dot);
    const int n_even = (n + 1) & ~1;
    const bool stacked = rows_tot > rows_dot;
    const int dot16 = (rows_dot + 15) / 16, ride16 = (rows_tot - rows_dot + 15) / 16;
    const int half = dot16 > ride16 ? dot16 : ride16;
    const int epl = stacked ? 2 * half : dot16;
    BASD_CHECK_ARG(!(stacked && n_arr));

    int lanes = g_jacobi_lanes;
    if (lanes == 0 && stacked && batch >= 256) lanes = n_even >= 40 ? 4 : (n_even >= 16 ? 8 : 16);
    if (stacked && n_even >= 8 && lanes == 8) {
        const int dot16 = (rows_dot + 15) / 16, ride16 = (rows_tot - rows_dot + 15) / 16;
        const int half16 = dot16 > ride16 ? dot16 : ride16;
        const int d8 = 2 * half16;
        const size_t lds8 = (size_t)n_even * (8 * 2 * d8 + 16 + 2) * sizeof(float);
        if (d8 <= 8 && lds8 <= BASD_JACOBI_LDS_LIMIT) {
            int threads = (((n_even / 2) * 8 + 63) / 64) * 64;
            if (threads > 1024) threads = 1024;
#define LAUNCH_LDS8(D)                                                                                               \
    do {                                                                                                             \
        if (lds8 > 48 * 1024)                                                                                        \
            (void)hipFuncSetAttribute((const void*)jacobi_lds_kernel<2 * (D), D, 8>,                                 \
                                      hipFuncAttributeMaxDynamicSharedMemorySize, BASD_JACOBI_LDS_LIMIT);            \
        jacobi_lds_kernel<2 * (D), D, 8><<<batch, threads, lds8, stream>>>(W, batch_stride, rows_dot, rows_tot, n,   \
                                                                           n_arr, max_sweeps, tol, colnorm,          \
                                                                           colnorm_stride, sweeps_out);              \
    } while (0)
            switch (d8) {
                case 2: LAUNCH_LDS8(2); break;
                case 4: LAUNCH_LDS8(4); break;
                case 6: LAUNCH_LDS8(6); break;
                default: LAUNCH_LDS8(8); break;
            }
#undef LAUNCH_LDS8
            BASD_RETURN_LAST();
        }
    }

    if (stacked && n_even >= 8 && lanes == 4) {
        const int dot8 = (rows_dot + 7) / 8, ride8 = (rows_tot - rows_dot + 7) / 8;
        const int half8 = dot8 > ride8 ? dot8 : ride8;
        static const int q_dot[] = {8, 12, 14, 16};
        int d4 = 0;
        for (int dq : q_dot)
            if (dq >= 2 * half8) { d4 = dq; break; }
        const size_t lds4 = (size_t)n_even * (4 * 2 * d4 + 8 + 2) * sizeof(float);
        if (d4 && lds4 <= BASD_JACOBI_LDS_LIMIT) {
            int threads = (((n_even / 2) * 4 + 63) / 64) * 64;
            if (threads > 1024) threads = 1024;
#define LAUNCH_LDS4(D)                                                                                               \
    do {                                                                                                             \
        if (lds4 > 48 * 1024)                                                                                        \
            (void)hipFuncSetAttribute((const void*)jacobi_lds_kernel<2 * (D), D, 4>,                                 \
                                      hipFuncAttributeMaxDynamicSharedMemorySize, BASD_JACOBI_LDS_LIMIT);            \
        jacobi_lds_kernel<2 * (D), D, 4><<<batch, threads, lds4, stream>>>(W, batch_stride, rows_dot, rows_tot, n,   \
                                                                           n_arr, max_sweeps, tol, colnorm,          \
                                                                           colnorm_stride, sweeps_out);              \
    } while (0)
            switch (d4) {
                case 8: LAUNCH_LDS4(8); break;
                case 12: LAUNCH_LDS4(12); break;
                case 14: LAUNCH_LDS4(14); break;
                default: LAUNCH_LDS4(16); break;
            }
#undef LAUNCH_LDS4
            BASD_RETURN_LAST();
        }
    }

    if (g_jacobi_ordering == 0 && !stacked && !n_arr && rows_tot > 96 && rows_tot <= 160 && n_even <= 160 &&
        (lanes == 8 || (lanes == 0 && batch >= 128 && batch <= 320))) {
        const size_t lds8p = (size_t)n_even * (8 * 20 + 16 + 2) * sizeof(float);
        if (lds8p <= BASD_JACOBI_LDS_LIMIT) {
            int threads = (((n_even / 2) * 8 + 63) / 64) * 64;
            if (threads > 1024) threads = 1024;
            (void)hipFuncSetAttribute((const void*)jacobi_lds_kernel<20, 20, 8>,
                                      hipFuncAttributeMaxDynamicSharedMemorySize, BASD_JACOBI_LDS_LIMIT);
            jacobi_lds_kernel<20, 20, 8><<<batch, threads, lds8p, stream>>>(W, batch_stride, rows_dot, rows_tot, n, n_arr,
                                                                            max_sweeps, tol, colnorm, colnorm_stride,
                                                                            sweeps_out);
            BASD_RETURN_LAST();
        }
    }

    if (g_jacobi_ordering == 1 && !stacked && !n_arr && n_even >= 8 && rows_tot == rows_dot &&
        (lanes == 0 || lanes == 4) && (g_jacobi_lanes == 4 || (batch >= 128 && n_even >= 40) || n_even >= 96)) {
        static const int o_epl[] = {8, 16, 24, 36, 50};
        int e4 = 0;
        for (int e : o_epl)
            if (4 * e >= rows_tot) { e4 = e; break; }
        const int G = n_even / 2;
        const size_t lds_oe = (size_t)(G + 1) * (plain4_ld(e4) + 2) * sizeof(float);
        const int threads = ((G * 4 + 63) / 64) * 64;
        if (e4 && threads <= 512 && lds_oe <= BASD_JACOBI_LDS_LIMIT) {
#define LAUNCH_OE(E)                                                                                                  \
    do {                                                                                                              \
        if (lds_oe > 48 * 1024)                                                                                       \
            (void)hipFuncSetAttribute((const void*)jacobi_oe_kernel<E>, hipFuncAttributeMaxDynamicSharedMemorySize,   \
                                      BASD_JACOBI_LDS_LIMIT);                                                         \
        jacobi_oe_kernel<E><<<batch, threads, lds_oe, stream>>>(W, batch_stride, rows_tot, n, max_sweeps, tol, colnorm, \
                                                                colnorm_stride, sweeps_out);                          \
    } while (0)
            switch (e4) {
                case 8: LAUNCH_OE(8); break;
                case 16: LAUNCH_OE(16); break;
                case 24: LAUNCH_OE(24); break;
                case 36: LAUNCH_OE(36); break;
                default: LAUNCH_OE(50); break;
            }
#undef LAUNCH_OE
            BASD_RETURN_LAST();
        }
    }

    if (!stacked && !n_arr && n_even >= 8 && (lanes == 4 || (lanes == 0 && batch >= 128 && n_even >= 40))) {
        static const int p_epl[] = {8, 16, 24, 36, 50};
        int e4 = 0;
        for (int e : p_epl)
            if (4 * e >= rows_tot) { e4 = e; break; }
        const size_t lds4 = (size_t)n_even * (plain4_ld(e4) + 2) * sizeof(float);
        if (e4 && lds4 <= BASD_JACOBI_LDS_LIMIT) {
            int threads = (((n_even / 2) * 4 + 63) / 64) * 64;
            if (threads > 1024) threads = 1024;
#define LAUNCH_P4(E)                                                                                                  \
    do {                                                                                                              \
        if (lds4 > 48 * 1024)                                                                                         \
            (void)hipFuncSetAttribute((const void*)jacobi_lds_kernel<E, E, 4>,                                        \
                                      hipFuncAttributeMaxDynamicSharedMemorySize, BASD_JACOBI_LDS_LIMIT);             \
        jacobi_lds_kernel<E, E, 4><<<batch, threads, lds4, stream>>>(W, batch_stride, rows_dot, rows_tot, n, n_arr,   \
                                                                     max_sweeps, tol, colnorm, colnorm_stride,        \
                                                                     sweeps_out);                                     \
    } while (0)
            switch (e4) {
                case 8: LAUNCH_P4(8); break;
                case 16: LAUNCH_P4(16); break;
                case 24: LAUNCH_P4(24); break;
                case 36: LAUNCH_P4(36); break;
                default: LAUNCH_P4(50); break;
            }
#undef LAUNCH_P4
            BASD_RETURN_LAST();
        }
    }

    static const int lds_epl[] = {2, 4, 6, 8, 12, 16, 20};
    int e_lds = 0;
    for (int e : lds_epl)
        if (e >= epl && (!stacked || e % 4 == 0)) { e_lds = e; break; }
    if (e_lds && (size_t)n_even * (16 * e_lds + 4) * sizeof(float) <= BASD_JACOBI_LDS_LIMIT) {
        const size_t lds_bytes = (size_t)n_even * (16 * e_lds + 4) * sizeof(float);
        int threads = (((n_even / 2) * 16 + 63) / 64) * 64;
        if (threads > 1024) threads = 1024;
#define LAUNCH_LDS(E, D)                                                                                          \
    do {                                                                                                          \
        if (lds_bytes > 48 * 1024)                                                                                \
            (void)hipFuncSetAttribute((const void*)jacobi_lds_kernel<E, D>,                                       \
                                      hipFuncAttributeMaxDynamicSharedMemorySize, BASD_JACOBI_LDS_LIMIT);         \
        jacobi_lds_kernel<E, D><<<batch, threads, lds_bytes, stream>>>(W, batch_stride, rows_dot, rows_tot, n,    \
                                                                        n_arr, max_sweeps, tol, colnorm,           \
                                                                        colnorm_stride, sweeps_out);               \
    } while (0)
#define LAUNCH_LDS_E(E)                                      \
    do {                                                     \
        if (stacked) {                                       \
            if constexpr ((E) % 4 == 0) LAUNCH_LDS(E, (E) / 2); \
        } else {                                             \
            LAUNCH_LDS(E, E);                                \
        }                                                    \
    } while (0)
        switch (e_lds) {
            case 2: LAUNCH_LDS_E(2); break;
            case 4: LAUNCH_LDS_E(4); break;
            case 6: LAUNCH_LDS_E(6); break;
            case 8: LAUNCH_LDS_E(8); break;
            case 12: LAUNCH_LDS_E(12); break;
            case 16: LAUNCH_LDS_E(16); break;
            default: LAUNCH_LDS_E(20); break;
        }
#undef LAUNCH_LDS_E
#undef LAUNCH_LDS
        BASD_RETURN_LAST();
    }

    BASD_CHECK_ARG(n_arr == nullptr && flags != nullptr);
    struct Shape { int lpp, epl, dot, bw, nblk; };
    Shape best{0, 0, 0, 0, 1 << 30};
    static const int st64[] = {2, 4, 6, 8, 10, 12, 16, 0}, pl64[] = {2, 4, 6, 8, 12, 16, 0};
    static const int st32[] = {4, 8, 12, 16, 20, 0}, pl32[] = {4, 8, 12, 16, 20, 0};
    static const int st16[] = {8, 10, 14, 16, 20, 0}, pl16[] = {8, 10, 14, 16, 20, 28, 32, 0};
    static const int lpps[] = {64, 32, 16};
    for (int lpp : lpps) {
        const int cd = (rows_dot + 2 * lpp - 1) / (2 * lpp), cr = (rows_tot - rows_dot + 2 * lpp - 1) / (2 * lpp);
        const int need = 2 * (stacked && cr > cd ? cr : cd);
        const int* q = lpp == 64 ? (stacked ? st64 : pl64) : lpp == 32 ? (stacked ? st32 : pl32) : (stacked ? st16 : pl16);
        int sel = 0;
        for (; *q; ++q)
            if (*q >= need) { sel = *q; break; }
        if (!sel) continue;
        const int epl = stacked ? 2 * sel : sel;
        const size_t col_bytes = sizeof(float) * (size_t)(lpp * epl + 2);
        int bw = (int)((BASD_JACOBI_LDS_LIMIT - 64) / (2 * (col_bytes + 8)));
        if (bw > 1024 / lpp) bw = 1024 / lpp;
        if (bw > ((n + 1) & ~1)) bw = (n + 1) & ~1;
        bw &= ~1;
        if (bw < 2) continue;
        int nb = (n + bw - 1) / bw;
        nb = (nb + 1) & ~1;
        if (nb < best.nblk) best = Shape{lpp, epl, sel, bw, nb};
    }
    if (!best.lpp) return BASD_EUNSUPPORTED;
    const int BW = best.bw, nblk = best.nblk;
    const size_t panel_bytes = (size_t)2 * BW * (best.lpp * best.epl + 2 + 2) * sizeof(float);
    hipError_t err = hipMemsetAsync(flags, 0, sizeof(int) * (size_t)2 * batch * max_sweeps, stream);
    if (err != hipSuccess) return (int)err;
#define LAUNCH_BLOCK(E, D, LP)                                                                                   \
    do {                                                                                                         \
        if (panel_bytes > 48 * 1024)                                                                             \
            (void)hipFuncSetAttribute((const void*)jacobi_block_round_kernel<E, D, LP>,                          \
                                      hipFuncAttributeMaxDynamicSharedMemorySize, BASD_JACOBI_LDS_LIMIT);        \
        for (int s = 0; s < max_sweeps; ++s)                                                                     \
            for (int r = 0; r < nblk - 1; ++r)                                                                   \
                jacobi_block_round_kernel<E, D, LP><<<dim3(nblk / 2, batch), LP * BW, panel_bytes, stream>>>(    \
                    W, batch_stride, rows_dot, rows_tot, n, nblk, BW, r, s, max_sweeps, tol, flags,              \
                    flags + (size_t)batch * max_sweeps);                                                         \
    } while (0)
#define LAUNCH_BLOCK_SEL(Q, LP)                      \
    do {                                             \
        if (stacked) LAUNCH_BLOCK(2 * (Q), Q, LP);   \
        else LAUNCH_BLOCK(Q, Q, LP);                 \
    } while (0)
    bool launched = true;
    if (best.lpp == 64) {
        switch (best.dot) {
            case 2: LAUNCH_BLOCK_SEL(2, 64); break;
            case 4: LAUNCH_BLOCK_SEL(4, 64); break;
            case 6: LAUNCH_BLOCK_SEL(6, 64); break;
            case 8: LAUNCH_BLOCK_SEL(8, 64); break;
            case 10: LAUNCH_BLOCK(20, 10, 64); break;
            case 12: LAUNCH_BLOCK_SEL(12, 64); break;
            case 16: LAUNCH_BLOCK_SEL(16, 64); break;
            default: launched = false; break;
        }
    } else if (best.lpp == 32) {
        switch (best.dot) {
            case 4: LAUNCH_BLOCK_SEL(4, 32); break;
            case 8: LAUNCH_BLOCK_SEL(8, 32); break;
            case 12: LAUNCH_BLOCK_SEL(12, 32); break;
            case 16: LAUNCH_BLOCK_SEL(16, 32); break;
            case 20: LAUNCH_BLOCK_SEL(20, 32); break;
            default: launched = false; break;
        }
    } else {
        switch (best.dot) {
            case 8: LAUNCH_BLOCK_SEL(8, 16); break;
            case 10: LAUNCH_BLOCK_SEL(10, 16); break;
            case 14: LAUNCH_BLOCK_SEL(14, 16); break;
            case 16: LAUNCH_BLOCK_SEL(16, 16); break;
            case 20: LAUNCH_BLOCK_SEL(20, 16); break;
            case 28: LAUNCH_BLOCK(28, 28, 16); break;
            case 32: LAUNCH_BLOCK(32, 32, 16); break;
            default: launched = false; break;
        }
    }
#undef LAUNCH_BLOCK_SEL
#undef LAUNCH_BLOCK
    if (!launched) return BASD_EUNSUPPORTED;
    if (sweeps_out) block_sweeps_kernel<<<(batch + 255) / 256, 256, 0, stream>>>(flags, batch, max_sweeps, sweeps_out);
    colnorm_kernel<<<dim3((n + 3) / 4, batch), 256, 0, stream>>>(W, batch_stride, rows_dot, rows_tot, n, colnorm,
                                                                 colnorm_stride);
    BASD_RETURN_LAST();
}

static int twopass_epl(int n) {
    static const int epls[] = {28, 36, 44, 50};
    const size_t n_even = (n + 1) & ~1;
    for (int e : epls)
        if (n <= 4 * e) {
            const size_t ld = 4 * e + (((4 * e / 8) % 2 == 0) ? 8 : 0);
            return sizeof(float) * (n_even * ld + 2 * n_even) <= BASD_JACOBI_LDS_LIMIT ? e : 0;
        }
    return 0;
}
static bool stacked_lds_fits(int n) {
    const int n_even = (n + 1) & ~1, epl = 2 * ((n + 15) / 16);
    static const int lds_epl[] = {4, 8, 12, 16, 20};
    for (int e : lds_epl)
        if (e >= epl) return (size_t)n_even * (16 * e + 4) * sizeof(float) <= BASD_JACOBI_LDS_LIMIT;
    return false;
}
long basd_jacobi_twopass_workspace_bytes(int n, int batch, int max_sweeps) {
    if (n < 2 || batch <= 0 || max_sweeps <= 0 || stacked_lds_fits(n) || !twopass_epl(n)) return 0;
    const long n_even = (n + 1) & ~1;
    const long entries = (long)max_sweeps * (n_even - 1) * (n_even / 2);
    return (long)batch * (entries * 8 + (long)n * 4 + 4) + 64;
}
int basd_jacobi_stacked_twopass(float* W, long batch_stride, int n, int batch, float* colnorm, int colnorm_stride,
                                int max_sweeps, float tol_cos, void* workspace, int* sweeps_out, hipStream_t stream) {
    BASD_CHECK_ARG(W && colnorm && workspace && n > 1 && batch > 0 && max_sweeps > 0);
    BASD_CHECK_ARG(((uintptr_t)workspace & 7) == 0);
    const int epl = twopass_epl(n);
    if (!epl || stacked_lds_fits(n)) return BASD_EUNSUPPORTED;
    const float tol = tol_cos > 0.f ? tol_cos : 1.2e-7f * sqrtf((float)n);
    const long n_even = (n + 1) & ~1;
    const long entries = (long)max_sweeps * (n_even - 1) * (n_even / 2);
    f32x2* rotlog = (f32x2*)workspace;
    float* dev = (float*)(rotlog + (long)batch * entries);
    int* sweeps = (int*)(dev + (long)batch * n);
    int threads = (int)(((n_even / 2) * 4 + 63) / 64) * 64;
    BASD_CHECK_ARG(threads <= 512);
#define LAUNCH_2P(E)                                                                                                  \
    do {                                                                                                              \
        const size_t lds = sizeof(float) * ((size_t)n_even * TwoPassShape<E>::LD + 2 * (size_t)n_even);               \
        if (lds > BASD_JACOBI_LDS_LIMIT) return BASD_EUNSUPPORTED;                                                    \
        (void)hipFuncSetAttribute((const void*)jacobi_top_logged_kernel<E>, hipFuncAttributeMaxDynamicSharedMemorySize, \
                                  BASD_JACOBI_LDS_LIMIT);                                                             \
        jacobi_top_logged_kernel<E><<<batch, threads, lds, stream>>>(W, batch_stride, 2 * n, n, max_sweeps, tol, colnorm, \
                                                                     colnorm_stride, rotlog, entries, dev, sweeps);   \
        if (n <= 160) {                                                                                               \
            const size_t lds2 = sizeof(float) * (size_t)n_even * TwoPassShape<10>::LD;                                \
            jacobi_apply_log_kernel<10><<<dim3(batch, (n + 39) / 40), threads, lds2, stream>>>(                       \
                W, batch_stride, 2 * n, n, n, rotlog, entries, dev, sweeps);                                          \
        } else {                                                                                                      \
            const size_t lds2 = sizeof(float) * (size_t)n_even * TwoPassShape<14>::LD;                                \
            jacobi_apply_log_kernel<14><<<dim3(batch, (n + 55) / 56), threads, lds2, stream>>>(                       \
                W, batch_stride, 2 * n, n, n, rotlog, entries, dev, sweeps);                                          \
        }                                                                                                             \
    } while (0)
    switch (epl) {
        case 28: LAUNCH_2P(28); break;
        case 36: LAUNCH_2P(36); break;
        case 44: LAUNCH_2P(44); break;
        default: LAUNCH_2P(50); break;
    }
#undef LAUNCH_2P
    if (sweeps_out) {
        hipError_t e = hipMemcpyAsync(sweeps_out, sweeps, sizeof(int) * (size_t)batch, hipMemcpyDeviceToDevice, stream);
        if (e != hipSuccess) return (int)e;
    }
    BASD_RETURN_LAST();
}

int basd_sort_extract(const float* W, long batch_stride, int rows, int rows_tot, int n, int batch,
                      const float* colnorm, int colnorm_stride, float* vals_desc, float* vecs, int kmax,
                      hipStream_t stream) {
    BASD_CHECK_ARG(W && colnorm && vals_desc && n > 0 && n <= 1024 && batch > 0 && rows <= rows_tot);
    sort_extract_kernel<<<batch, 256, 0, stream>>>(W, batch_stride, rows, rows_tot, n, colnorm, colnorm_stride,
                                                   vals_desc, vecs, kmax);
    BASD_RETURN_LAST();
}

}
```

### vit-inductive-bias-distillation_amd/csrc/procrustes.hip

```cpp
#include "basd_common.h"
#include "../../include/basd_hip.h"

namespace basd {

typedef double f64x4 __attribute__((ext_vector_type(4)));

template <typename T>
__global__ void __launch_bounds__(256) token_weights_kernel(const void* const* __restrict__ attn_ptrs,
                                                            const float* __restrict__ mix, int L, long sb, long sh,
                                                            long sq, long sk, int H, int A, int has_cls, int n_a,
                                                            int n_t, int n_s, const int* __restrict__ atap0,
                                                            const int* __restrict__ atap1,
                                                            const float* __restrict__ alam,
                                                            const int* __restrict__ tap0,
                                                            const int* __restrict__ tap1,
                                                            const float* __restrict__ lam, float* __restrict__ omega,
                                                            float* __restrict__ omega_t, float* __restrict__ raw_out) {
    extern __shared__ float sm[];
    float* raw = sm;
    float* w = sm + n_a;
    __shared__ float red[32];
    const int b = blockIdx.x, tid = threadIdx.x;
    for (int j = tid; j < n_a; j += blockDim.x) {
        float acc = 0.f;
        if (has_cls) {
            for (int h = 0; h < H; ++h) {
                float m = 0.f;
                for (int l = 0; l < L; ++l)
                    m += mix[l] * ldg_f32((const BASD_GLOBAL_AS T*)attn_ptrs[l] + (b * sb + h * sh + (long)(1 + j) * sk));
                acc += m;
            }
            acc /= (float)H;
        } else {
            for (int h = 0; h < H; ++h)
                for (int q = 0; q < A; ++q) {
                    float m = 0.f;
                    for (int l = 0; l < L; ++l)
                        m += mix[l] * ldg_f32((const BASD_GLOBAL_AS T*)attn_ptrs[l] + (b * sb + h * sh + q * sq + (long)j * sk));
                    acc += m;
                }
            acc /= (float)(H * A);
        }
        raw[j] = acc;
        if (raw_out) raw_out[(long)b * n_a + j] = acc;
    }
    __syncthreads();
    float part = 0.f;
    for (int n = tid; n < n_s; n += blockDim.x) {
        float v;
        if (atap0) {
            const float l1 = alam[n];
            v = (1.f - l1) * raw[atap0[n]] + l1 * raw[atap1[n]];
        } else {
            v = raw[n];
        }
        w[n] = v;
        part += v;
    }
    const float total = block_sum(part, red);
    for (int n = tid; n < n_s; n += blockDim.x) {
        const float v = w[n] / total;
        w[n] = v;
        omega[(long)b * n_s + n] = v;
    }
    __syncthreads();
    for (int j = tid; j < n_t; j += blockDim.x) {
        float acc = 0.f;
        if (tap0) {
            for (int n = 0; n < n_s; ++n) {
                const float l1 = lam[n];
                if (tap0[n] == j) acc += (1.f - l1) * w[n];
                if (tap1[n] == j) acc += l1 * w[n];
            }
        } else {
            acc = w[j];
        }
        omega_t[(long)b * n_t + j] = acc;
    }
}

template <typename T>
__global__ void __launch_bounds__(256) student_project_kernel(const T* __restrict__ X, long sb, long sn, int n_s,
                                                              int n_t, int D, const float* __restrict__ omega,
                                                              const int* __restrict__ tap0,
                                                              const int* __restrict__ tap1,
                                                              const float* __restrict__ lam,
                                                              const int* __restrict__ range0,
                                                              const int* __restrict__ range1,
                                                              float* __restrict__ mu_out, float* __restrict__ tr_part,
                                                              float* __restrict__ Ap) {
    extern __shared__ float sm[];
    float* w = sm;
    __shared__ float red[4][64];
    __shared__ float mu[64];
    __shared__ float scratch[32];
    const int b = blockIdx.y, d0 = blockIdx.x * 64, tid = threadIdx.x;
    const int cl = tid & 63, rg = tid >> 6, d = d0 + cl;
    const bool live = d < D;
    const T* Xb = X + (long)b * sb + d;
    for (int n = tid; n < n_s; n += 256) w[n] = omega[(long)b * n_s + n];
    __syncthreads();
    float acc = 0.f;
    if (live)
        for (int n = rg; n < n_s; n += 4) acc = fmaf(w[n], to_f32(Xb[(long)n * sn]), acc);
    red[rg][cl] = acc;
    __syncthreads();
    if (rg == 0) {
        const float m = (red[0][cl] + red[1][cl]) + (red[2][cl] + red[3][cl]);
        mu[cl] = m;
        if (live) mu_out[(long)b * D + d] = m;
    }
    __syncthreads();
    const float m = mu[cl];
    float part = 0.f;
    if (live)
        for (int n = rg; n < n_s; n += 4) {
            const float c = to_f32(Xb[(long)n * sn]) - m;
            part = fmaf(w[n] * c, c, part);
        }
    const float tr = block_sum(part, scratch);
    if (tid == 0) tr_part[(long)b * gridDim.x + blockIdx.x] = tr;
    if (!live) return;
    float* Ab = Ap + (long)b * n_t * D + d;
    for (int j = rg; j < n_t; j += 4) {
        const int n0 = range0 ? range0[j] : j, n1 = range1 ? range1[j] : j + 1;
        float a = 0.f;
        for (int n = n0; n < n1; ++n) {
            float coef = 1.f;
            if (tap0) {
                const float l1 = lam[n];
                coef = (tap0[n] == j ? 1.f - l1 : 0.f) + (tap1[n] == j ? l1 : 0.f);
            }
            a = fmaf(coef * w[n], to_f32(Xb[(long)n * sn]) - m, a);
        }
        Ab[(long)j * D] = a;
    }
}

__device__ __forceinline__ float4 ld4f(const float* p) { return *(const float4*)p; }
typedef float native_f32x4 __attribute__((ext_vector_type(4)));
typedef unsigned native_u32x2 __attribute__((ext_vector_type(2)));
__device__ __forceinline__ float4 ld4f(const BASD_GLOBAL_AS float* p) {
    const native_f32x4 v = *(const BASD_GLOBAL_AS native_f32x4*)p;
    return make_float4(v.x, v.y, v.z, v.w);
}
__device__ __forceinline__ float4 ld4f(const BASD_GLOBAL_AS __hip_bfloat16* p) {
    const native_u32x2 v = *(const BASD_GLOBAL_AS native_u32x2*)p;
    return make_float4(__uint_as_float(v.x << 16), __uint_as_float(v.x & 0xffff0000u), __uint_as_float(v.y << 16),
                       __uint_as_float(v.y & 0xffff0000u));
}
__device__ __forceinline__ float4 ld4f(const __hip_bfloat16* p) {
    const uint2 v = *(const uint2*)p;
    return make_float4(__uint_as_float(v.x << 16), __uint_as_float(v.x & 0xffff0000u), __uint_as_float(v.y << 16),
                       __uint_as_float(v.y & 0xffff0000u));
}

template <typename T>
__global__ void __launch_bounds__(256) student_project_lds_kernel(const T* __restrict__ X, long sb, long sn, int n_s,
                                                                  int n_t, int D, const float* __restrict__ omega,
                                                                  const int* __restrict__ tap0,
                                                                  const int* __restrict__ tap1,
                                                                  const float* __restrict__ lam,
                                                                  const int* __restrict__ range0,
                                                                  const int* __restrict__ range1,
                                                                  float* __restrict__ mu_out,
                                                                  float* __restrict__ tr_part, float* __restrict__ Ap) {
    extern __shared__ __attribute__((aligned(16))) float sm[];
    float* xs = sm;
    float* w = sm + (long)n_s * 64;
    __shared__ float red[4][64];
    __shared__ float mu[64];
    __shared__ float scratch[32];
    const int b = blockIdx.y, d0 = blockIdx.x * 64, tid = threadIdx.x;
    const int cl = tid & 63, rg = tid >> 6, d = d0 + cl;
    const bool live = d < D;
    const T* Xb = X + (long)b * sb + d0;
    for (int n = tid; n < n_s; n += 256) w[n] = omega[(long)b * n_s + n];
    for (int idx = tid; idx < n_s * 16; idx += 256) {
        const int row = idx >> 4, c4 = (idx & 15) * 4;
        float4 v = make_float4(0.f, 0.f, 0.f, 0.f);
        if (d0 + c4 < D) v = ld4f(Xb + (long)row * sn + c4);
        *(float4*)(xs + row * 64 + c4) = v;
    }
    __syncthreads();
    float acc = 0.f;
    for (int n = rg; n < n_s; n += 4) acc = fmaf(w[n], xs[n * 64 + cl], acc);
    red[rg][cl] = acc;
    __syncthreads();
    if (rg == 0) {
        const float m = (red[0][cl] + red[1][cl]) + (red[2][cl] + red[3][cl]);
        mu[cl] = m;
        if (live) mu_out[(long)b * D + d] = m;
    }
    __syncthreads();
    const float m = mu[cl];
    float part = 0.f;
    if (live)
        for (int n = rg; n < n_s; n += 4) {
            const float c = xs[n * 64 + cl] - m;
            part = fmaf(w[n] * c, c, part);
        }
    const float tr = block_sum(part, scratch);
    if (tid == 0) tr_part[(long)b * gridDim.x + blockIdx.x] = tr;
    if (!live) return;
    float* Ab = Ap + (long)b * n_t * D + d;
    for (int j = rg; j < n_t; j += 4) {
        const int n0 = range0 ? range0[j] : j, n1 = range1 ? range1[j] : j + 1;
        float a = 0.f;
        for (int n = n0; n < n1; ++n) {
            float coef = 1.f;
            if (tap0) {
                const float l1 = lam[n];
                coef = (tap0[n] == j ? 1.f - l1 : 0.f) + (tap1[n] == j ? l1 : 0.f);
            }
            a = fmaf(coef * w[n], xs[n * 64 + cl] - m, a);
        }
        Ab[(long)j * D] = a;
    }
}

constexpr int SP_W = 32;
template <typename T>
__global__ void __launch_bounds__(256) student_project_v4_kernel(const void* const* __restrict__ x_ptrs, long sb,
                                                                 long sn, int n_s, int n_t, int D,
                                                                 const float* __restrict__ omega, long omega_e_stride,
                                                                 const int* __restrict__ tap0,
                                                                 const int* __restrict__ tap1,
                                                                 const float* __restrict__ lam,
                                                                 const int* __restrict__ range0,
                                                                 const int* __restrict__ range1,
                                                                 float* __restrict__ mu_out,
                                                                 float* __restrict__ tr_part, float* __restrict__ Ap) {
    extern __shared__ __attribute__((aligned(16))) float sm[];
    float* xs = sm;
    float* w = sm + (long)n_s * SP_W;
    float* c0 = w + n_s;
    float* c1 = c0 + n_s;
    int* t0 = (int*)(c1 + n_s);
    int* t1 = t0 + n_s;
    __shared__ __attribute__((aligned(16))) float red[32][SP_W];
    __shared__ __attribute__((aligned(16))) float mu[SP_W];
    __shared__ float scratch[32];
    const int b = blockIdx.y, e = blockIdx.z, B = gridDim.y, d0 = blockIdx.x * SP_W, tid = threadIdx.x;
    const int fq = tid & 7, rg = tid >> 3, c4 = 4 * fq;
    const bool live = d0 + c4 < D;
    const BASD_GLOBAL_AS T* Xb = (const BASD_GLOBAL_AS T*)x_ptrs[e] + (long)b * sb + d0;
    const float* om = omega + (long)e * omega_e_stride + (long)b * n_s;
    for (int n = tid; n < n_s; n += 256) {
        const float wn = om[n];
        w[n] = wn;
        if (tap0) {
            const float l1 = lam[n];
            c0[n] = (1.f - l1) * wn;
            c1[n] = l1 * wn;
            t0[n] = tap0[n];
            t1[n] = tap1[n];
        }
    }
    for (int n = rg; n < n_s; n += 32) {
        float4 v = make_float4(0.f, 0.f, 0.f, 0.f);
        if (live) v = ld4f(Xb + (long)n * sn + c4);
        *(float4*)(xs + n * SP_W + c4) = v;
    }
    __syncthreads();
    float4 acc = make_float4(0.f, 0.f, 0.f, 0.f);
    for (int n = rg; n < n_s; n += 32) {
        const float4 v = *(const float4*)(xs + n * SP_W + c4);
        const float wn = w[n];
        acc.x = fmaf(wn, v.x, acc.x); acc.y = fmaf(wn, v.y, acc.y);
        acc.z = fmaf(wn, v.z, acc.z); acc.w = fmaf(wn, v.w, acc.w);
    }
    *(float4*)(&red[rg][c4]) = acc;
    __syncthreads();
    if (tid < SP_W) {
        float m = 0.f;
#pragma unroll
        for (int q = 0; q < 32; ++q) m += red[q][tid];
        mu[tid] = m;
        if (d0 + tid < D) mu_out[((long)e * B + b) * D + d0 + tid] = m;
    }
    __syncthreads();
    const float4 m4 = *(const float4*)(mu + c4);
    float part = 0.f;
    if (live)
        for (int n = rg; n < n_s; n += 32) {
            const float4 v = *(const float4*)(xs + n * SP_W + c4);
            const float cx = v.x - m4.x, cy = v.y - m4.y, cz = v.z - m4.z, cw = v.w - m4.w;
            part = fmaf(w[n], fmaf(cx, cx, fmaf(cy, cy, fmaf(cz, cz, cw * cw))), part);
        }
    const float tr = block_sum(part, scratch);
    if (tid == 0) tr_part[((long)e * B + b) * gridDim.x + blockIdx.x] = tr;
    if (!live) return;
    float* Ab = Ap + ((long)e * B + b) * n_t * D + d0 + c4;
    for (int j = rg; j < n_t; j += 32) {
        const int n0 = range0 ? range0[j] : j, n1 = range1 ? range1[j] : j + 1;
        float4 a = make_float4(0.f, 0.f, 0.f, 0.f);
        for (int n = n0; n < n1; ++n) {
            const float cw = tap0 ? (t0[n] == j ? c0[n] : 0.f) + (t1[n] == j ? c1[n] : 0.f) : w[n];
            const float4 v = *(const float4*)(xs + n * SP_W + c4);
            a.x = fmaf(cw, v.x - m4.x, a.x); a.y = fmaf(cw, v.y - m4.y, a.y);
            a.z = fmaf(cw, v.z - m4.z, a.z); a.w = fmaf(cw, v.w - m4.w, a.w);
        }
        *(float4*)(Ab + (long)j * D) = a;
// ... 415 lines not shown
            __syncthreads();
        }
        for (int idx = tid; idx < rows * CB_NB; idx += 1024) {
            const int ii = idx / CB_NB, cc = idx & (CB_NB - 1);
            if (cc < nb) Lm[(long)(j0 + ii) * n + j0 + cc] = ii >= cc ? panel[idx] : 0.;
        }
        __syncthreads();
    }
}

__global__ void __launch_bounds__(256) stack_product_global_kernel(const double* __restrict__ La,
                                                                   const double* __restrict__ Lb,
                                                                   long l_batch_stride, int n, float* __restrict__ W,
                                                                   long w_batch_stride, int lb_period) {
    __shared__ double ta[32][33], tb[32][33];
    const int b = blockIdx.z, i0 = blockIdx.x * 32, j0 = blockIdx.y * 32, tid = threadIdx.x;
    const double* A = La + (long)b * l_batch_stride;
    const double* B = Lb + (long)(b % lb_period) * l_batch_stride;
    const int tx = tid & 31, ty = tid >> 5;
    double acc[4] = {0., 0., 0., 0.};
    for (int k0 = i0 > j0 ? i0 : j0; k0 < n; k0 += 32) {
        __syncthreads();
        for (int idx = tid; idx < 1024; idx += 256) {
            const int kk = idx >> 5, c = idx & 31, k = k0 + kk;
            ta[kk][c] = (k < n && i0 + c < n) ? A[(long)k * n + i0 + c] : 0.;
            tb[kk][c] = (k < n && j0 + c < n) ? B[(long)k * n + j0 + c] : 0.;
        }
        __syncthreads();
#pragma unroll 8
        for (int kk = 0; kk < 32; ++kk) {
            const double av = ta[kk][tx];
#pragma unroll
            for (int r = 0; r < 4; ++r) acc[r] = fma(av, tb[kk][ty + 8 * r], acc[r]);
        }
    }
    float* Wb = W + (long)b * w_batch_stride;
#pragma unroll
    for (int r = 0; r < 4; ++r) {
        const int i = i0 + tx, j = j0 + ty + 8 * r;
        if (i < n && j < n) {
            Wb[(long)j * 2 * n + i] = (float)acc[r];
            Wb[(long)j * 2 * n + n + i] = (float)B[(long)i * n + j];
        }
    }
}

__global__ void __launch_bounds__(256) stack_product_kernel(const double* __restrict__ La,
                                                            const double* __restrict__ Lb, long l_batch_stride,
                                                            int n, float* __restrict__ W, long w_batch_stride,
                                                            int lb_period) {
    extern __shared__ __attribute__((aligned(16))) double sd[];
    double* sa = sd;
    double* sb = sd + (size_t)n * n;
    const int b = blockIdx.x, tid = threadIdx.x;
    const double* A = La + (long)b * l_batch_stride;
    const double* B = Lb + (long)(b % lb_period) * l_batch_stride;
    for (int idx = tid; idx < n * n; idx += 256) {
        sa[idx] = A[idx];
        sb[idx] = B[idx];
    }
    __syncthreads();
    float* Wb = W + (long)b * w_batch_stride;
    for (int idx = tid; idx < n * n; idx += 256) {
        const int j = idx / n, i = idx - j * n;
        double acc = 0.;
        for (int k = (i > j ? i : j); k < n; ++k) acc = fma(sa[k * n + i], sb[k * n + j], acc);
        Wb[(long)j * 2 * n + i] = (float)acc;
        Wb[(long)j * 2 * n + n + i] = (float)sb[i * n + j];
    }
}

__global__ void __launch_bounds__(256) stack_product_t_kernel(const double* __restrict__ La, const double* __restrict__ Lb,
                                                              long l_batch_stride, int n, float* __restrict__ W,
                                                              long w_batch_stride, int lb_period) {
    __shared__ double ta[32][33], tb[32][33];
    const int b = blockIdx.z, i0 = blockIdx.y * 32, j0 = blockIdx.x * 32, tid = threadIdx.x;
    const double* A = La + (long)b * l_batch_stride;
    const double* B = Lb + (long)(b % lb_period) * l_batch_stride;
    const int tx = tid & 31, ty = tid >> 5;
    double acc[4] = {0., 0., 0., 0.};
    for (int k0 = i0 > j0 ? i0 : j0; k0 < n; k0 += 32) {
        __syncthreads();
        for (int idx = tid; idx < 1024; idx += 256) {
            const int kk = idx >> 5, c = idx & 31, k = k0 + kk;
            ta[kk][c] = (k < n && i0 + c < n) ? A[(long)k * n + i0 + c] : 0.;
            tb[kk][c] = (k < n && j0 + c < n) ? B[(long)k * n + j0 + c] : 0.;
        }
        __syncthreads();
#pragma unroll 8
        for (int kk = 0; kk < 32; ++kk) {
            const double bv = tb[kk][tx];
#pragma unroll
            for (int r = 0; r < 4; ++r) acc[r] = fma(ta[kk][ty + 8 * r], bv, acc[r]);
        }
    }
    float* Wb = W + (long)b * w_batch_stride;
#pragma unroll
    for (int r = 0; r < 4; ++r) {
        const int i = i0 + ty + 8 * r, j = j0 + tx;
        if (i < n && j < n) Wb[(long)i * n + j] = (float)acc[r];
    }
}

__global__ void __launch_bounds__(256) kprime_z_kernel(const float* __restrict__ W, long w_batch_stride,
                                                       const float* __restrict__ sigma, int n,
                                                       const double* __restrict__ Lb, long l_batch_stride, int lb_period,
                                                       float* __restrict__ Z, long z_batch_stride) {
    __shared__ float lt[32][33], wt[32][33];
    __shared__ float red[4];
    const int b = blockIdx.z, a0 = blockIdx.x * 32, c0 = blockIdx.y * 32, tid = threadIdx.x;
    const float* sg = sigma + (long)b * n;
    float smax = 0.f;
    for (int j = tid; j < n; j += 256) smax = fmaxf(smax, sg[j]);
    smax = wave_max(smax);
    if ((tid & 63) == 0) red[tid >> 6] = smax;
    __syncthreads();
    smax = fmaxf(fmaxf(red[0], red[1]), fmaxf(red[2], red[3]));
    const float thr = smax * (float)n * 1.1920929e-7f;
    const float* Wb = W + (long)b * w_batch_stride;
    const double* L = Lb + (long)(b % lb_period) * l_batch_stride;
    const int tx = tid & 31, ty = tid >> 5;
    float acc[4] = {0.f, 0.f, 0.f, 0.f};
    for (int r0 = 0; r0 < a0 + 32 && r0 < n; r0 += 32) {
        __syncthreads();
        for (int idx = tid; idx < 1024; idx += 256) {
            const int i = idx >> 5, rr = idx & 31, r = r0 + rr;
            lt[i][rr] = (a0 + i < n && r <= a0 + i) ? (float)L[(long)(a0 + i) * n + r] : 0.f;
            wt[i][rr] = (c0 + i < n && r < n) ? Wb[(long)(c0 + i) * n + r] : 0.f;
        }
        __syncthreads();
#pragma unroll 8
        for (int rr = 0; rr < 32; ++rr) {
            const float lv = lt[tx][rr];
#pragma unroll
            for (int i = 0; i < 4; ++i) acc[i] = fmaf(lv, wt[ty + 8 * i][rr], acc[i]);
        }
    }
    float* Zb = Z + (long)b * z_batch_stride;
#pragma unroll
    for (int i = 0; i < 4; ++i) {
        const int c = c0 + ty + 8 * i, a = a0 + tx;
        if (c < n && a < n) {
            const float sv = sg[c];
            Zb[(long)c * n + a] = acc[i] * (sv > thr ? 1.f / (sv * sqrtf(sv)) : 0.f);
        }
    }
}

__global__ void __launch_bounds__(256) m_stash_kernel(const float* __restrict__ Wc, long wc_batch_stride, int n,
                                                      float* __restrict__ Wst, long w_batch_stride) {
    const long idx = (long)blockIdx.x * 256 + threadIdx.x;
    if (idx >= (long)n * n) return;
    const int b = blockIdx.y, i = (int)(idx / n), r = (int)(idx - (long)i * n);
    Wst[(long)b * w_batch_stride + (long)i * 2 * n + n + r] = Wc[(long)b * wc_batch_stride + idx];
}
__global__ void __launch_bounds__(256) ustack_from_x_kernel(const float* __restrict__ X, long x_batch_stride,
                                                            const float* __restrict__ sigma, int n,
                                                            const float* __restrict__ Wst, long w_batch_stride,
                                                            float* __restrict__ Out, long out_batch_stride) {
    __shared__ float mt[32][33], xt[32][33];
    __shared__ float red[4];
    const int b = blockIdx.z, i0 = blockIdx.x * 32, c0 = blockIdx.y * 32, tid = threadIdx.x;
    const float* sg = sigma + (long)b * n;
    float smax = 0.f;
    for (int j = tid; j < n; j += 256) smax = fmaxf(smax, sg[j]);
    smax = wave_max(smax);
    if ((tid & 63) == 0) red[tid >> 6] = smax;
    __syncthreads();
    smax = fmaxf(fmaxf(red[0], red[1]), fmaxf(red[2], red[3]));
    const float thr = smax * (float)n * 1.1920929e-7f;
    const float* Xb = X + (long)b * x_batch_stride;
    const float* Wb = Wst + (long)b * w_batch_stride;
    float* Ob = Out + (long)b * out_batch_stride;
    const int tx = tid & 31, ty = tid >> 5;
    float acc[4] = {0.f, 0.f, 0.f, 0.f};
    for (int r0 = 0; r0 < n; r0 += 32) {
        __syncthreads();
        for (int idx = tid; idx < 1024; idx += 256) {
            const int q = idx >> 5, rr = idx & 31, r = r0 + rr;
            mt[q][rr] = (i0 + q < n && r < n) ? Wb[(long)(i0 + q) * 2 * n + n + r] : 0.f;
            xt[q][rr] = (c0 + q < n && r < n) ? Xb[(long)(c0 + q) * n + r] : 0.f;
        }
        __syncthreads();
#pragma unroll 8
        for (int rr = 0; rr < 32; ++rr) {
            const float mv = mt[tx][rr];
#pragma unroll
            for (int q = 0; q < 4; ++q) acc[q] = fmaf(mv, xt[ty + 8 * q][rr], acc[q]);
        }
    }
#pragma unroll
    for (int q = 0; q < 4; ++q) {
        const int c = c0 + ty + 8 * q, i = i0 + tx;
        if (c < n && i < n) {
            const float sv = sg[c];
            Ob[(long)c * n + i] = sv > thr ? acc[q] / sv : 0.f;
        }
    }
}
__global__ void __launch_bounds__(256) ustack_place_kernel(const float* __restrict__ Uc, long uc_batch_stride, int n,
                                                           float* __restrict__ Wst, long w_batch_stride) {
    const long idx = (long)blockIdx.x * 256 + threadIdx.x;
    if (idx >= (long)n * n) return;
    const int b = blockIdx.y, c = (int)(idx / n), i = (int)(idx - (long)c * n);
    Wst[(long)b * w_batch_stride + (long)c * 2 * n + i] = Uc[(long)b * uc_batch_stride + idx];
}

__global__ void __launch_bounds__(256) kprime_from_z_kernel(const float* __restrict__ Z, long z_batch_stride, int n,
                                                            float* __restrict__ Kp) {
    __shared__ float za[32][33], zb[32][33];
    const int b = blockIdx.z, a0 = blockIdx.y * 32, b0 = blockIdx.x * 32, tid = threadIdx.x;
    const float* Zb = Z + (long)b * z_batch_stride;
    const int tx = tid & 31, ty = tid >> 5;
    float acc[4] = {0.f, 0.f, 0.f, 0.f};
    for (int c0 = 0; c0 < n; c0 += 32) {
        __syncthreads();
        for (int idx = tid; idx < 1024; idx += 256) {
            const int cc = idx >> 5, i = idx & 31, c = c0 + cc;
            za[cc][i] = (c < n && a0 + i < n) ? Zb[(long)c * n + a0 + i] : 0.f;
            zb[cc][i] = (c < n && b0 + i < n) ? Zb[(long)c * n + b0 + i] : 0.f;
        }
        __syncthreads();
#pragma unroll 8
        for (int cc = 0; cc < 32; ++cc) {
            const float bv = zb[cc][tx];
#pragma unroll
            for (int i = 0; i < 4; ++i) acc[i] = fmaf(za[cc][ty + 8 * i], bv, acc[i]);
        }
    }
    float* K = Kp + (long)b * n * n;
#pragma unroll
    for (int i = 0; i < 4; ++i) {
        const int a = a0 + ty + 8 * i, bb = b0 + tx;
        if (a < n && bb < n) K[(long)a * n + bb] = acc[i];
    }
}

__global__ void __launch_bounds__(256) procrustes_finalize_kernel(
    const float* __restrict__ W, long w_batch_stride, const float* __restrict__ sigma, int n, int n_s,
    const double* __restrict__ Gb, long g_batch_stride, const float* __restrict__ omega,
    const int* __restrict__ tap0, const int* __restrict__ tap1, const float* __restrict__ lam,
    const float* __restrict__ tr_s, int tr_slabs, float* __restrict__ tr_s_out, float* __restrict__ tr_t_out,
    float* __restrict__ nuc_out, float* __restrict__ loss_out, float* __restrict__ Kp, int t_period) {
    extern __shared__ float sm[];
    float* isig = sm;
    __shared__ float red[32];
    __shared__ double redd[32];
    const int b = blockIdx.x, tid = threadIdx.x;
    const float* sg = sigma + (long)b * n;
    float smax = 0.f, ssum = 0.f;
    for (int j = tid; j < n; j += 256) {
        smax = fmaxf(smax, sg[j]);
        ssum += sg[j];
    }
    smax = wave_max(smax);
    __syncthreads();
    if ((tid & 63) == 0) red[tid >> 6] = smax;
    __syncthreads();
    smax = fmaxf(fmaxf(red[0], red[1]), fmaxf(red[2], red[3]));
    const float nuc = block_sum(ssum, red);
    const float thr = smax * (float)n * 1.1920929e-7f;
    for (int j = tid; j < n; j += 256) isig[j] = sg[j] > thr ? 1.f / sg[j] : 0.f;
    const int bt = b % t_period;
    const double* G = Gb + (long)bt * g_batch_stride;
    double part = 0.;
    for (int s = tid; s < n_s; s += 256) {
        const double w = (double)omega[(long)bt * n_s + s];
        if (tap0) {
            const int i0 = tap0[s], i1 = tap1[s];
            const double l1 = (double)lam[s], l0 = 1. - l1;
            part += w * (l0 * l0 * G[(long)i0 * n + i0] + 2. * l0 * l1 * G[(long)i0 * n + i1] + l1 * l1 * G[(long)i1 * n + i1]);
        } else {
            part += w * G[(long)s * n + s];
        }
    }
    const double trt = block_sum(part, redd);
    if (tid == 0) {
        float trs = 0.f;
        for (int k = 0; k < tr_slabs; ++k) trs += tr_s[(long)b * tr_slabs + k];
        tr_s_out[b] = trs;
        tr_t_out[b] = (float)trt;
        nuc_out[b] = nuc;
        loss_out[b] = trs + (float)trt - 2.f * nuc;
    }
    __syncthreads();
    if (Kp) {
        const float* Wb = W + (long)b * w_batch_stride;
        float* Yh = sm + n;
        for (int idx = tid; idx < n * n; idx += 256) {
            const int j = idx / n, r = idx - j * n;
            Yh[idx] = Wb[(long)j * 2 * n + n + r] * sqrtf(isig[j]);
        }
        __syncthreads();
        float* K = Kp + (long)b * n * n;
        for (int idx = tid; idx < n * n; idx += 256) {
            const int r = idx / n, c = idx - r * n;
            float acc = 0.f;
            for (int j = 0; j < n; ++j) acc = fmaf(Yh[j * n + r], Yh[j * n + c], acc);
            K[idx] = acc;
        }
    }
}

__global__ void __launch_bounds__(256) kprime_tiled_kernel(const float* __restrict__ W, long w_batch_stride,
                                                           const float* __restrict__ sigma, int n,
                                                           float* __restrict__ Kp) {
    __shared__ float ya[32][33], yb[32][33];
    __shared__ float red[4];
    const int b = blockIdx.z, r0 = blockIdx.y * 32, c0 = blockIdx.x * 32, tid = threadIdx.x;
    const float* sg = sigma + (long)b * n;
    float smax = 0.f;
    for (int j = tid; j < n; j += 256) smax = fmaxf(smax, sg[j]);
    smax = wave_max(smax);
    if ((tid & 63) == 0) red[tid >> 6] = smax;
    __syncthreads();
    smax = fmaxf(fmaxf(red[0], red[1]), fmaxf(red[2], red[3]));
    const float thr = smax * (float)n * 1.1920929e-7f;
    const float* Wb = W + (long)b * w_batch_stride;
    const int tx = tid & 31, ty = tid >> 5;
    float acc[4] = {0.f, 0.f, 0.f, 0.f};
    for (int j0 = 0; j0 < n; j0 += 32) {
        __syncthreads();
        for (int idx = tid; idx < 1024; idx += 256) {
            const int jj = idx >> 5, rr = idx & 31, j = j0 + jj;
            float sc = 0.f;
            if (j < n && sg[j] > thr) sc = sqrtf(1.f / sg[j]);
            ya[jj][rr] = (j < n && r0 + rr < n) ? Wb[(long)j * 2 * n + n + r0 + rr] * sc : 0.f;
            yb[jj][rr] = (j < n && c0 + rr < n) ? Wb[(long)j * 2 * n + n + c0 + rr] * sc : 0.f;
        }
        __syncthreads();
#pragma unroll 8
        for (int jj = 0; jj < 32; ++jj) {
            const float bv = yb[jj][tx];
#pragma unroll
            for (int i = 0; i < 4; ++i) acc[i] = fmaf(ya[jj][ty + 8 * i], bv, acc[i]);
        }
    }
    float* K = Kp + (long)b * n * n;
#pragma unroll
    for (int i = 0; i < 4; ++i) {
        const int r = r0 + ty + 8 * i, c = c0 + tx;
        if (r < n && c < n) K[(long)r * n + c] = acc[i];
    }
}

template <typename T>
__global__ void __launch_bounds__(128) student_grad_kernel(const T* __restrict__ X, const void* const* __restrict__ x_ptrs,
                                                           long sb, long sn, int n_s, int n_t,
                                                           int D, const float* __restrict__ omega, long omega_e_stride,
                                                           const float* __restrict__ mu, const float* __restrict__ H,
                                                           const int* __restrict__ tap0, const int* __restrict__ tap1,
                                                           const float* __restrict__ lam,
                                                           const float* __restrict__ scale_ptr, float scale_const,
                                                           float* __restrict__ dX, const float* __restrict__ tnorm2,
                                                           float* __restrict__ gomega) {
    __shared__ float red[32];
    const int s = blockIdx.x, e = blockIdx.z;
    const long B = gridDim.y, b = (long)e * B + blockIdx.y;
    if (x_ptrs) X = (const T*)x_ptrs[e];
    const float coef = scale_ptr[e] * scale_const * omega[(long)e * omega_e_stride + (long)blockIdx.y * n_s + s];
    const T* x = X + (long)blockIdx.y * sb + (long)s * sn;
    const float* m = mu + (long)b * D;
    int i0 = s, i1 = s;
    float l1 = 0.f;
    if (tap0) {
        i0 = tap0[s];
        i1 = tap1[s];
        l1 = lam[s];
    }
    const float* h0 = H + ((long)b * n_t + i0) * D;
    const float* h1 = H + ((long)b * n_t + i1) * D;
    float* out = dX + ((long)b * n_s + s) * D;
    float xx = 0.f, xt = 0.f;
    for (int d = threadIdx.x; d < D; d += 128) {
        const float tgt = (1.f - l1) * h0[d] + l1 * h1[d];
        const float xc = to_f32(x[d]) - m[d];
        out[d] = coef * (xc - tgt);
        xx = fmaf(xc, xc, xx);
        xt = fmaf(xc, tgt, xt);
    }
    if (gomega) {
        xx = block_sum(xx, red);
        xt = block_sum(xt, red);
        if (threadIdx.x == 0) gomega[(long)b * n_s + s] = xx + tnorm2[(long)b * n_s + s] - 2.f * xt;
    }
}

constexpr int SG_W = 64;
constexpr int SG_LD = SG_W + 4;
template <typename T, int RP>
__global__ void __launch_bounds__(256) student_grad_fused_kernel(
    const void* const* __restrict__ x_ptrs, long sb, long sn, int n_s, int n_t, int D, const float* __restrict__ omega,
    long omega_e_stride, const float* __restrict__ mu, const float* __restrict__ Kp, const float* __restrict__ Ap,
    const int* __restrict__ tap0, const int* __restrict__ tap1, const float* __restrict__ lam,
    const float* __restrict__ scale_ptr, float scale_const, float* __restrict__ dX) {
    extern __shared__ __attribute__((aligned(16))) float sm[];
    float* as = sm;
    float* hs = sm + (long)n_t * SG_W;
    const int by = blockIdx.y, e = blockIdx.z, d0 = blockIdx.x * SG_W, tid = threadIdx.x;
    const long b = (long)e * gridDim.y + by;
    const int q4 = 4 * (tid & 15);
    const bool live = d0 + q4 < D;
    const float* A = Ap + b * n_t * D + d0;
    for (int k = tid >> 4; k < n_t; k += 16) {
        float4 v = make_float4(0.f, 0.f, 0.f, 0.f);
        if (live) v = *(const float4*)(A + (long)k * D + q4);
        *(float4*)(as + k * SG_W + q4) = v;
    }
    __syncthreads();
    {
        const int g = __builtin_amdgcn_readfirstlane(tid >> 6), c = tid & 63;
        const int i0 = RP * g < n_t - RP ? RP * g : n_t - RP;
        const float* K = Kp + b * n_t * n_t + i0;
        float acc[RP];
#pragma unroll
        for (int r = 0; r < RP; ++r) acc[r] = 0.f;
        for (int k = 0; k < n_t; ++k) {
            const float a = as[k * SG_W + c];
            const float* Kk = K + (long)k * n_t;
#pragma unroll
            for (int r = 0; r < RP; ++r) acc[r] = fmaf(Kk[r], a, acc[r]);
        }
#pragma unroll
        for (int r = 0; r < RP; ++r) hs[(i0 + r) * SG_LD + c] = acc[r];
    }
    __syncthreads();
    const BASD_GLOBAL_AS T* Xb = (const BASD_GLOBAL_AS T*)x_ptrs[e] + (long)by * sb + d0 + q4;
    const float* om = omega + (long)e * omega_e_stride + (long)by * n_s;
    float* out = dX + b * n_s * D + d0 + q4;
    const float sc = scale_ptr[e] * scale_const;
    float4 m4 = make_float4(0.f, 0.f, 0.f, 0.f);
    if (live) m4 = *(const float4*)(mu + b * D + d0 + q4);
    if (!live) return;
    for (int s0 = tid >> 4; s0 < n_s; s0 += 64) {
        float4 x[4];
#pragma unroll
        for (int u = 0; u < 4; ++u) {
            const int s = s0 + 16 * u;
            if (s < n_s) x[u] = ld4f(Xb + (long)s * sn);
        }
#pragma unroll
        for (int u = 0; u < 4; ++u) {
            const int s = s0 + 16 * u;
            if (s >= n_s) break;
            int i0 = s, i1 = s;
            float l1 = 0.f;
            if (tap0) {
                i0 = tap0[s];
                i1 = tap1[s];
                l1 = lam[s];
            }
            const float coef = sc * om[s];
            const float4 h0 = *(const float4*)(hs + i0 * SG_LD + q4), h1 = *(const float4*)(hs + i1 * SG_LD + q4);
            float4 o;
            o.x = coef * ((x[u].x - m4.x) - ((1.f - l1) * h0.x + l1 * h1.x));
            o.y = coef * ((x[u].y - m4.y) - ((1.f - l1) * h0.y + l1 * h1.y));
            o.z = coef * ((x[u].z - m4.z) - ((1.f - l1) * h0.z + l1 * h1.z));
            o.w = coef * ((x[u].w - m4.w) - ((1.f - l1) * h0.w + l1 * h1.w));
            *(float4*)(out + (long)s * D) = o;
        }
    }
}

template <typename T>
__global__ void __launch_bounds__(128) resample_tokens_kernel(const T* __restrict__ X, long sb, long sn, long sd,
                                                              int n_in, int n_out, int D,
                                                              const int* __restrict__ tap0,
                                                              const int* __restrict__ tap1,
                                                              const float* __restrict__ lam, float* __restrict__ out) {
    const int s = blockIdx.x, b = blockIdx.y;
    const int i0 = tap0[s], i1 = tap1[s];
    const float l1 = lam[s], l0 = 1.f - l1;
    const T* x0 = X + (long)b * sb + (long)i0 * sn;
    const T* x1 = X + (long)b * sb + (long)i1 * sn;
    float* o = out + ((long)b * n_out + s) * D;
    for (int d = threadIdx.x; d < D; d += 128) o[d] = l0 * to_f32(x0[(long)d * sd]) + l1 * to_f32(x1[(long)d * sd]);
}

__global__ void __launch_bounds__(128) resample_tokens_adjoint_kernel(const float* __restrict__ dY, int n_in,
                                                                      int n_out, int D,
                                                                      const int* __restrict__ tap0,
                                                                      const int* __restrict__ tap1,
                                                                      const float* __restrict__ lam,
                                                                      const int* __restrict__ range0,
                                                                      const int* __restrict__ range1,
                                                                      float* __restrict__ dX) {
    const int j = blockIdx.x, b = blockIdx.y;
    const int s0 = range0[j], s1 = range1[j];
    for (int d = threadIdx.x; d < D; d += 128) {
        float acc = 0.f;
        for (int s = s0; s < s1; ++s) {
            const float l1 = lam[s];
            const float coef = (tap0[s] == j ? 1.f - l1 : 0.f) + (tap1[s] == j ? l1 : 0.f);
            acc = fmaf(coef, dY[((long)b * n_out + s) * D + d], acc);
        }
        dX[((long)b * n_in + j) * D + d] = acc;
    }
}

}

using namespace basd;

extern "C" {

int basd_token_weights(const void* const* attn_ptrs, int dtype, const float* mix, int L, long sb, long sh, long sq,
                       long sk, int B, int H, int A, int has_cls, int n_a, int n_t, int n_s, const int* atap0,
                       const int* atap1, const float* alam, const int* tap0, const int* tap1, const float* lam,
                       float* omega, float* omega_t, float* raw_out, hipStream_t stream) {
    BASD_CHECK_ARG(attn_ptrs && mix && omega && omega_t && L > 0 && B > 0 && H > 0 && n_a > 0 && n_t > 0 && n_s > 0);
    BASD_CHECK_ARG(A == n_a + (has_cls ? 1 : 0));
    BASD_CHECK_ARG((n_a == n_s) == (atap0 == nullptr));
    BASD_CHECK_ARG((n_t == n_s) == (tap0 == nullptr));
    const size_t lds = sizeof(float) * (size_t)(n_a + n_s);
    if (dtype == BASD_DTYPE_F32)
        token_weights_kernel<float><<<B, 256, lds, stream>>>(attn_ptrs, mix, L, sb, sh, sq, sk, H, A, has_cls, n_a, n_t, n_s, atap0, atap1, alam, tap0, tap1, lam, omega, omega_t, raw_out);
    else if (dtype == BASD_DTYPE_BF16)
        token_weights_kernel<__hip_bfloat16><<<B, 256, lds, stream>>>(attn_ptrs, mix, L, sb, sh, sq, sk, H, A, has_cls, n_a, n_t, n_s, atap0, atap1, alam, tap0, tap1, lam, omega, omega_t, raw_out);
    else
        return BASD_EINVAL;
    BASD_RETURN_LAST();
}

int basd_student_project(const void* x, int dtype, long sb, long sn, int B, int n_s, int n_t, int D,
                         const float* omega, const int* tap0, const int* tap1, const float* lam, const int* range0,
                         const int* range1, float* mu, float* tr_s, float* a_prime, hipStream_t stream) {
    BASD_CHECK_ARG(x && omega && mu && tr_s && a_prime && B > 0 && n_s > 0 && n_t > 0 && D > 0);
    BASD_CHECK_ARG((n_t == n_s) == (tap0 == nullptr));
    const size_t lds = sizeof(float) * (size_t)n_s;
    const dim3 grid((D + 63) / 64, B);
    const int esz = dtype == BASD_DTYPE_F32 ? 4 : 2;
    const size_t lds_slab = sizeof(float) * (size_t)n_s * 65;
    const bool staged = D % 4 == 0 && ((uintptr_t)x * 1) % 16 == 0 && (sb * esz) % 16 == 0 && (sn * esz) % 16 == 0 &&
                        (esz == 4 || D % 8 == 0) && lds_slab <= 64 * 1024;
    if (dtype == BASD_DTYPE_F32) {
        if (staged) {
            (void)hipFuncSetAttribute((const void*)student_project_lds_kernel<float>, hipFuncAttributeMaxDynamicSharedMemorySize, (int)lds_slab);
            student_project_lds_kernel<float><<<grid, 256, lds_slab, stream>>>((const float*)x, sb, sn, n_s, n_t, D, omega, tap0, tap1, lam, range0, range1, mu, tr_s, a_prime);
        } else {
            student_project_kernel<float><<<grid, 256, lds, stream>>>((const float*)x, sb, sn, n_s, n_t, D, omega, tap0, tap1, lam, range0, range1, mu, tr_s, a_prime);
        }
    } else if (dtype == BASD_DTYPE_BF16) {
        if (staged) {
            (void)hipFuncSetAttribute((const void*)student_project_lds_kernel<__hip_bfloat16>, hipFuncAttributeMaxDynamicSharedMemorySize, (int)lds_slab);
            student_project_lds_kernel<__hip_bfloat16><<<grid, 256, lds_slab, stream>>>((const __hip_bfloat16*)x, sb, sn, n_s, n_t, D, omega, tap0, tap1, lam, range0, range1, mu, tr_s, a_prime);
        } else {
            student_project_kernel<__hip_bfloat16><<<grid, 256, lds, stream>>>((const __hip_bfloat16*)x, sb, sn, n_s, n_t, D, omega, tap0, tap1, lam, range0, range1, mu, tr_s, a_prime);
        }
    } else {
        return BASD_EINVAL;
    }
    BASD_RETURN_LAST();
}

int basd_teacher_center(const void* const* tok_ptrs, int dtype, const float* mix, int L, long sb, long sn, long sd,
                        int B, int n, int D, const int* g0, const int* g1, const float* glam, const float* omega_t,
                        float* mu, float* tc, hipStream_t stream) {
    BASD_CHECK_ARG(tok_ptrs && mix && omega_t && mu && tc && L > 0 && B > 0 && n > 0 && D > 0);
    BASD_CHECK_ARG((g0 == nullptr) == (g1 == nullptr) && (g0 == nullptr) == (glam == nullptr));
    const size_t lds = sizeof(float) * ((size_t)n * 65 + n + 64);
    if (lds > 150 * 1024) return BASD_EUNSUPPORTED;
    const dim3 grid((D + 63) / 64, B);
    if (dtype == BASD_DTYPE_F32) {
        (void)hipFuncSetAttribute((const void*)teacher_center_kernel<float>, hipFuncAttributeMaxDynamicSharedMemorySize, 150 * 1024);
        teacher_center_kernel<float><<<grid, 256, lds, stream>>>(tok_ptrs, mix, L, sb, sn, sd, n, D, g0, g1, glam, omega_t, mu, tc);
    } else if (dtype == BASD_DTYPE_BF16) {
        (void)hipFuncSetAttribute((const void*)teacher_center_kernel<__hip_bfloat16>, hipFuncAttributeMaxDynamicSharedMemorySize, 150 * 1024);
        teacher_center_kernel<__hip_bfloat16><<<grid, 256, lds, stream>>>(tok_ptrs, mix, L, sb, sn, sd, n, D, g0, g1, glam, omega_t, mu, tc);
    } else {
        return BASD_EINVAL;
    }
    BASD_RETURN_LAST();
}

int basd_teacher_center_multi(const void* const* tok_ptrs, int dtype, const float* mix, int L, int G, long sb, long sn,
                              long sd, int B, int n, int D, const int* g0, const int* g1, const float* glam,
                              const float* omega_t, float* mu, float* tc, hipStream_t stream) {
    BASD_CHECK_ARG(tok_ptrs && mix && omega_t && mu && tc && L > 0 && G > 0 && B > 0 && n > 0 && D > 0);
    BASD_CHECK_ARG((g0 == nullptr) == (g1 == nullptr) && (g0 == nullptr) == (glam == nullptr));
    BASD_CHECK_ARG(B <= 65535);
    const size_t lds = sizeof(float) * ((size_t)G * n * (TCM_W + 1) + (size_t)G * n + (size_t)G * TCM_W);
    if (G > TCM_G || lds > 150 * 1024) return BASD_EUNSUPPORTED;
    const dim3 grid((D + TCM_W - 1) / TCM_W, B);
    if (dtype == BASD_DTYPE_F32) {
        (void)hipFuncSetAttribute((const void*)teacher_center_multi_kernel<float>, hipFuncAttributeMaxDynamicSharedMemorySize, 150 * 1024);
        teacher_center_multi_kernel<float><<<grid, 256, lds, stream>>>(tok_ptrs, mix, L, G, sb, sn, sd, n, D, g0, g1, glam, omega_t, mu, tc);
    } else if (dtype == BASD_DTYPE_BF16) {
        (void)hipFuncSetAttribute((const void*)teacher_center_multi_kernel<__hip_bfloat16>, hipFuncAttributeMaxDynamicSharedMemorySize, 150 * 1024);
        teacher_center_multi_kernel<__hip_bfloat16><<<grid, 256, lds, stream>>>(tok_ptrs, mix, L, G, sb, sn, sd, n, D, g0, g1, glam, omega_t, mu, tc);
    } else {
        return BASD_EINVAL;
    }
    BASD_RETURN_LAST();
}

__global__ void __launch_bounds__(256) teacher_mix_stream_v4_kernel(
    const void* const* __restrict__ tok_ptrs, const float* __restrict__ mix, int L, int G, long sb, long sn, int n, int D,
    const float* __restrict__ omega_t, float* __restrict__ Tc, float* __restrict__ chunk_sum) {
    const int chunk = blockIdx.x, b = blockIdx.y, B = gridDim.y, tid = threadIdx.x;
    const int j_lo = chunk * TCS_ROWS, j_hi = j_lo + TCS_ROWS < n ? j_lo + TCS_ROWS : n;
    bool aligned = true;
    for (int l = 0; l < L; ++l) aligned = aligned && (((uintptr_t)tok_ptrs[l]) & 15) == 0;
    if (!aligned) {
        for (int d = tid; d < D; d += 256) {
            float musum[TCM_G] = {0.f, 0.f, 0.f, 0.f};
            for (int j = j_lo; j < j_hi; ++j) {
// ... 325 lines not shown
```

Measured before the change: 168,100 images/s.

## Fuse student Gram, Cholesky, stack product, Jacobi SVD and k-prime into one kernel

Adds a single per-batch kernel that computes the student Gram and its Cholesky factor in LDS, forms the transposed stack product, runs the odd-even Jacobi SVD, then produces sigma, the trace and loss terms and k_prime. The path is on by default and can be switched off with BASD_FUSED_CORES. The goal is to remove several launches and the global round-trips for g_all, l_all and W on the student side. In exchange the kernel uses a lot of LDS and does its Gram work in a single block, which may reduce occupancy. Only teacher Cholesky still runs separately.

```diff
diff --git a/include/basd_hip.h b/include/basd_hip.h
--- a/include/basd_hip.h
+++ b/include/basd_hip.h
@@ -244,6 +244,7 @@
 } BasdProcrustesArgs;
 int basd_procrustes_forward_fused(const BasdProcrustesArgs* args, hipStream_t stream);
 int basd_procrustes_tuning(int transposed_cores);
+int basd_procrustes_fused_cores(int on);
 
 int basd_stack_product_t(const double* la, const double* lb, long l_batch_stride, int n, int batch, int lb_period,
                          float* w, long w_batch_stride, hipStream_t stream);
diff --git a/vit-inductive-bias-distillation_amd/basd_amd/_lib.py b/vit-inductive-bias-distillation_amd/basd_amd/_lib.py
--- a/vit-inductive-bias-distillation_amd/basd_amd/_lib.py
+++ b/vit-inductive-bias-distillation_amd/basd_amd/_lib.py
@@ -73,6 +73,7 @@
                                 f32, vp, vp],
     "basd_procrustes_forward_fused": [vp, vp],
     "basd_procrustes_tuning": [i32],
+    "basd_procrustes_fused_cores": [i32],
     "basd_jacobi_plain4_fits": [i32],
     "basd_stack_product_t": [vp, vp, i64, i32, i32, i32, vp, i64, vp],
     "basd_kprime_from_transposed": [vp, i64, vp, i32, i32, vp, i64, i32, vp, i64, vp, vp],
diff --git a/vit-inductive-bias-distillation_amd/basd_amd/ops.py b/vit-inductive-bias-distillation_amd/basd_amd/ops.py
--- a/vit-inductive-bias-distillation_amd/basd_amd/ops.py
+++ b/vit-inductive-bias-distillation_amd/basd_amd/ops.py
@@ -19,6 +19,8 @@
     _lib.call("basd_gemm_tuning", int(os.environ["BASD_GEMM_SPLIT"]))
 if os.environ.get("BASD_JACOBI_ORDERING") in ("0", "1"):
     _lib.call("basd_jacobi_ordering", int(os.environ["BASD_JACOBI_ORDERING"]))
+if os.environ.get("BASD_FUSED_CORES") in ("0", "1"):
+    _lib.call("basd_procrustes_fused_cores", int(os.environ["BASD_FUSED_CORES"]))
 
 
 def _stream() -> int:
diff --git a/vit-inductive-bias-distillation_amd/csrc/basd_common.h b/vit-inductive-bias-distillation_amd/csrc/basd_common.h
--- a/vit-inductive-bias-distillation_amd/csrc/basd_common.h
+++ b/vit-inductive-bias-distillation_amd/csrc/basd_common.h
@@ -97,4 +97,12 @@
     q = (r - t + m) % m;
 }
 
+int jacobi_oe_epl(int n, int rows, int batch);
+bool procrustes_core_fused_fits(int n, int d_s, int batch, const float* a_prime);
+int procrustes_core_fused(const float* a_prime, int n, int d_s, int batch, const double* lb, long l_batch_stride,
+                          int lb_period, int max_sweeps, float* sigma, int* sweeps, int n_s, const double* gt,
+                          long g_batch_stride, const float* omega, const int* tap0, const int* tap1, const float* lam,
+                          const float* tr_part, int tr_slabs, float* tr_s, float* tr_t, float* nuc, float* loss,
+                          float* k_prime, hipStream_t stream);
+
 }
diff --git a/vit-inductive-bias-distillation_amd/csrc/fused.hip b/vit-inductive-bias-distillation_amd/csrc/fused.hip
--- a/vit-inductive-bias-distillation_amd/csrc/fused.hip
+++ b/vit-inductive-bias-distillation_amd/csrc/fused.hip
@@ -99,6 +99,13 @@
     return BASD_OK;
 }
 
+static int g_fused_cores = 1;
+int basd_procrustes_fused_cores(int on) {
+    if (on != 0 && on != 1) return BASD_EINVAL;
+    g_fused_cores = on;
+    return BASD_OK;
+}
+
 int basd_procrustes_forward_fused(const BasdProcrustesArgs* a, hipStream_t st) {
     BASD_CHECK_ARG(a && a->student_ptrs && a->tok_ptrs && a->attn_ptrs && a->mix);
     const int E = (int)a->E, L = (int)a->L, G = (int)a->G, B = (int)a->B, n_s = (int)a->n_s, n_t = (int)a->n_t;
@@ -150,15 +157,26 @@
     }
     const long nn = (long)n * n;
     const int EB = E * B, GB = G * B;
-    BASD_TRY(basd_gram_f64(a->a_prime, (long)n * d_s, n, d_s, EB, a->g_all, nn, st));
+    const bool transposed = (a->raw == nullptr || a->w_stack != nullptr) && EB <= 65535 && basd_jacobi_plain4_fits(n) &&
+                            (g_transposed_cores == 2 || (g_transposed_cores == 1 && EB >= 128));
+    const bool fused_cores = transposed && a->raw == nullptr && g_fused_cores &&
+                             basd::procrustes_core_fused_fits(n, d_s, EB, a->a_prime);
+    if (!fused_cores) BASD_TRY(basd_gram_f64(a->a_prime, (long)n * d_s, n, d_s, EB, a->g_all, nn, st));
     if (a->g_slabs && a->g_splits > 1)
         BASD_TRY(basd_gram_f64_split(a->tc, (long)n * d_t, n, d_t, GB, (int)a->g_splits, a->g_slabs,
                                      a->g_all + (long)EB * nn, st));
     else
         BASD_TRY(basd_gram_f64(a->tc, (long)n * d_t, n, d_t, GB, a->g_all + (long)EB * nn, nn, st));
+    if (fused_cores) {
+        BASD_TRY(basd_chol_f64(a->g_all + (long)EB * nn, nn, n, GB, a->l_all + (long)EB * nn, nn, st));
+        BASD_TRY(basd::procrustes_core_fused(a->a_prime, n, d_s, EB, a->l_all + (long)EB * nn, nn, GB,
+                                             (int)a->max_sweeps, a->sigma, a->sweeps, n_s, a->g_all + (long)EB * nn, nn,
+                                             a->omega, a->tap0, a->tap1, a->lam, a->tr_part, slabs, a->tr_s, a->tr_t,
+                                             a->nuc, a->loss_b, a->k_prime, st));
+        return procrustes_tail(a, grad_layers_in, E, B, n_s, n, d_s, EB, nn, om_stride, st);
+    }
     BASD_TRY(basd_chol_f64(a->g_all, nn, n, EB + GB, a->l_all, nn, st));
-    if ((a->raw == nullptr || a->w_stack != nullptr) && EB <= 65535 && basd_jacobi_plain4_fits(n) &&
-        (g_transposed_cores == 2 || (g_transposed_cores == 1 && EB >= 128))) {
+    if (transposed) {
         BASD_TRY(basd_stack_product_t(a->l_all, a->l_all + (long)EB * nn, nn, n, EB, GB, a->W, 2 * nn, st));
         if (a->raw != nullptr) BASD_TRY(basd_ustack_stash(a->W, 2 * nn, n, EB, a->w_stack, 2 * nn, st));
         BASD_TRY(basd_jacobi_onesided(a->W, 2 * nn, n, n, n, EB, nullptr, a->sigma, n, (int)a->max_sweeps, 0.f,
diff --git a/vit-inductive-bias-distillation_amd/csrc/jacobi.hip b/vit-inductive-bias-distillation_amd/csrc/jacobi.hip
--- a/vit-inductive-bias-distillation_amd/csrc/jacobi.hip
+++ b/vit-inductive-bias-distillation_amd/csrc/jacobi.hip
@@ -1,55 +1,8 @@
-#include "basd_common.h"
+#include "jacobi_oe.h"
 
 namespace basd {
 
-constexpr float kNull2 = 2.2737368e-13f;
-
-struct Rot {
-    float c, s, t;
-    float h;
-    bool apply;
-    bool strong;
-};
-
-__device__ __forceinline__ Rot make_rotation(float alpha, float beta, float gamma, float tol) {
-    Rot r{1.f, 0.f, 0.f, 0.f, false, false};
-    const float cosv = gamma * __builtin_amdgcn_rsqf(alpha) * __builtin_amdgcn_rsqf(beta);
-    if (!(fabsf(cosv) > tol)) return r;
-    r.strong = cosv * cosv > tol;
-    const float zeta = (beta - alpha) * __builtin_amdgcn_rcpf(2.f * gamma);
-    const float az = fabsf(zeta);
-    float t = az > 1e8f ? 0.5f * __builtin_amdgcn_rcpf(az)
-                        : __builtin_amdgcn_rcpf(az + __builtin_amdgcn_sqrtf(fmaf(zeta, zeta, 1.f)));
-    t = copysignf(t, zeta);
-    r.t = t;
-    r.c = __builtin_amdgcn_rsqf(fmaf(t, t, 1.f));
-    r.s = r.c * t;
-    const float pc = r.c * r.c, ec = fmaf(r.c, r.c, -pc);
-    const float ps = r.s * r.s, es = fmaf(r.s, r.s, -ps);
-    r.h = 0.5f * ((((1.f - pc) - ps) - ec) - es);
-    r.apply = true;
-    return r;
-}
-
-template <int LPP>
-__device__ __forceinline__ float pair_allsum(float x) {
-    static_assert(LPP == 4 || LPP == 8 || LPP == 16 || LPP == 32 || LPP == 64,
-                  "a pair is owned by a quad, half a DPP row, a row, two rows or a wave");
-    if constexpr (LPP == 4 || LPP == 8) {
-        x += dpp_get<0xB1>(x);
-        x += dpp_get<0x4E>(x);
-        if constexpr (LPP == 8) x += dpp_get<0x141>(x);
-        return x;
-    } else if constexpr (LPP == 32) {
-        x = row16_allsum(x);
-        auto r = __builtin_amdgcn_permlane16_swap(__float_as_uint(x), __float_as_uint(x), false, false);
-        return __uint_as_float(r[0]) + __uint_as_float(r[1]);
-    } else {
-        return LPP == 16 ? row16_allsum(x) : wave64_allsum(x);
-    }
-}
-
-typedef float f32x2 __attribute__((ext_vector_type(2)));
+
 
 template <int EPL, int DOT, int LPP, bool LOG = false>
 __device__ __forceinline__ int rotate_pair(float* __restrict__ cp, float* __restrict__ cq, int gl, float tol,
@@ -198,59 +151,20 @@
     }
 }
 
-template <int H>
-__device__ __forceinline__ int rotate_regs(f32x2 (&x)[H], f32x2 (&y)[H], float& a, float& b, float& dx, float& dy,
-                                           float tol, float null2, float& norm2_max, bool forced) {
-    f32x2 acc = {0.f, 0.f};
-#pragma unroll
-    for (int i = 0; i < H; ++i) acc = __builtin_elementwise_fma(x[i], y[i], acc);
-    const float g = pair_allsum<4>(acc.x + acc.y);
-    norm2_max = fmaxf(norm2_max, fmaxf(a, b));
-    Rot rot{1.f, 0.f, 0.f, 0.f, false, false};
-    if (fminf(a, b) > null2) rot = make_rotation(a, b, g, tol);
-    float c = rot.c, s = rot.s;
-    if (forced) { c = 0.f; s = 1.f; }
-    if (rot.apply || forced) {
-        const f32x2 c2 = {c, c}, s2 = {s, s};
-#pragma unroll
-        for (int i = 0; i < H; ++i) {
-            const f32x2 xi = x[i], yi = y[i];
-            x[i] = __builtin_elementwise_fma(c2, xi, -(s2 * yi));
-            y[i] = __builtin_elementwise_fma(s2, xi, c2 * yi);
-        }
-    }
-    if (forced) {
-        b = a; a = 0.f; dy = dx; dx = 0.f;
-    } else if (rot.apply) {
-        a = fmaxf(a - rot.t * g, 0.f);
-        b = b + rot.t * g;
-        dx += rot.h;
-        dy += rot.h;
-    }
-    return rot.strong ? 3 : (rot.apply ? 1 : 0);
-}
-
 template <int EPL>
 __global__ void __launch_bounds__(512, 4) jacobi_oe_kernel(float* __restrict__ W, long batch_stride, int rows, int n,
                                                            int max_sweeps, float tol, float* __restrict__ colnorm,
                                                            int colnorm_stride, int* __restrict__ sweeps_out) {
-    static_assert(EPL % 2 == 0, "row chunks come in pairs");
     constexpr int H = EPL / 2;
-    constexpr int LD = 4 * EPL + (((4 * EPL / 8) % 2 == 0) ? 8 : 0);
     extern __shared__ __attribute__((aligned(16))) float lds[];
-    const int m = blockIdx.x, tid = threadIdx.x, nthr = blockDim.x;
+    const int m = blockIdx.x, tid = threadIdx.x;
     const int n_even = (n + 1) & ~1, G = n_even / 2;
-    float* mail_n2 = lds + (G + 1) * LD;
-    float* mail_dev = mail_n2 + (G + 1);
-    __shared__ int s_norm2_bits;
     float* Wm = W + (long)m * batch_stride;
     const int g = tid >> 2, gl = tid & 3;
-    const bool active = g < G, last = g == G - 1;
-    for (int idx = tid; idx < (G + 1) * (LD + 2); idx += nthr) lds[idx] = 0.f;
-    if (tid == 0) s_norm2_bits = 0;
+    const bool active = g < G;
+    jacobi_oe_clear<EPL>(lds, n);
 
     f32x2 x[H], y[H];
-    float a = 0.f, b = 0.f, dx = 0.f, dy = 0.f;
 #pragma unroll
     for (int i = 0; i < H; ++i) {
         const int r = 2 * gl + 8 * i;
@@ -260,60 +174,8 @@
         y[i].x = (active && cy < n && r < rows) ? Wm[(long)cy * rows + r] : 0.f;
         y[i].y = (active && cy < n && r + 1 < rows) ? Wm[(long)cy * rows + r + 1] : 0.f;
     }
-    float* slot_lo = lds + (active ? g : 0) * LD + 2 * gl;
-    float* slot_hi = lds + (active ? g + 1 : 0) * LD + 2 * gl;
-    __syncthreads();
-
-    float null2 = 0.f;
-    int sweep = 0;
-    for (; sweep < max_sweeps && n > 1; ++sweep) {
-        int rotated = 0;
-        float norm2_max = 0.f;
-        if (active) {
-            f32x2 sa = {0.f, 0.f}, sb = {0.f, 0.f};
-#pragma unroll
-            for (int i = 0; i < H; ++i) {
-                sa = __builtin_elementwise_fma(x[i], x[i], sa);
-                sb = __builtin_elementwise_fma(y[i], y[i], sb);
-            }
-            a = pair_allsum<4>(sa.x + sa.y);
-            b = pair_allsum<4>(sb.x + sb.y);
-        }
-        for (int dr = 0; dr < G; ++dr) {
-            if (active) {
-                rotated |= rotate_regs<H>(x, y, a, b, dx, dy, tol, null2, norm2_max, false);
-#pragma unroll
-                for (int i = 0; i < H; ++i) *(f32x2*)(slot_lo + 8 * i) = y[i];
-                if (gl == 0) { mail_n2[g] = b; mail_dev[g] = dy; }
-            }
-            __syncthreads();
-            if (active) {
-#pragma unroll
-                for (int i = 0; i < H; ++i) y[i] = *(const f32x2*)(slot_hi + 8 * i);
-                b = mail_n2[g + 1];
-                dy = mail_dev[g + 1];
-                rotated |= rotate_regs<H>(x, y, a, b, dx, dy, tol, null2, norm2_max, last);
-                if (!last) {
-#pragma unroll
-                    for (int i = 0; i < H; ++i) *(f32x2*)(slot_hi + 8 * i) = x[i];
-                    if (gl == 0) { mail_n2[g + 1] = a; mail_dev[g + 1] = dx; }
-                }
-            }
-            __syncthreads();
-            if (active) {
-#pragma unroll
-                for (int i = 0; i < H; ++i) x[i] = *(const f32x2*)(slot_lo + 8 * i);
-                a = mail_n2[g];
-                dx = mail_dev[g];
-            }
-        }
-        if (active && gl == 0 && norm2_max > 0.f) atomicMax(&s_norm2_bits, __float_as_int(norm2_max));
-        if (!__syncthreads_or(rotated & 2)) {
-            ++sweep;
-            break;
-        }
-        null2 = kNull2 * __int_as_float(s_norm2_bits);
-    }
+    float dx, dy;
+    const int sweep = jacobi_oe_sweeps<EPL>(x, y, dx, dy, lds, n, max_sweeps, tol);
     if (sweeps_out && tid == 0) sweeps_out[m] = sweep;
     if (!active) return;
 
@@ -695,6 +557,25 @@
     g_jacobi_ordering = odd_even;
     return BASD_OK;
 }
+
+}
+
+int basd::jacobi_oe_epl(int n, int rows, int batch) {
+    const int n_even = (n + 1) & ~1;
+    if (!(g_jacobi_ordering == 1 && n_even >= 8 && (g_jacobi_lanes == 0 || g_jacobi_lanes == 4) &&
+          (g_jacobi_lanes == 4 || (batch >= 128 && n_even >= 40) || n_even >= 96)))
+        return 0;
+    static const int o_epl[] = {8, 16, 24, 36, 50};
+    int e4 = 0;
+    for (int e : o_epl)
+        if (4 * e >= rows) { e4 = e; break; }
+    const int G = n_even / 2;
+    const size_t lds_oe = (size_t)(G + 1) * (plain4_ld(e4) + 2) * sizeof(float);
+    const int threads = ((G * 4 + 63) / 64) * 64;
+    return (e4 && threads <= 512 && lds_oe <= BASD_JACOBI_LDS_LIMIT) ? e4 : 0;
+}
+
+extern "C" {
 
 int basd_jacobi_onesided(float* W, long batch_stride, int rows_dot, int rows_tot, int n, int batch,
                          const int* n_arr, float* colnorm, int colnorm_stride, int max_sweeps, float tol_cos,
@@ -784,16 +665,12 @@
         }
     }
 
-    if (g_jacobi_ordering == 1 && !stacked && !n_arr && n_even >= 8 && rows_tot == rows_dot &&
-        (lanes == 0 || lanes == 4) && (g_jacobi_lanes == 4 || (batch >= 128 && n_even >= 40) || n_even >= 96)) {
-        static const int o_epl[] = {8, 16, 24, 36, 50};
-        int e4 = 0;
-        for (int e : o_epl)
-            if (4 * e >= rows_tot) { e4 = e; break; }
+    const int e4 = (!stacked && !n_arr && rows_tot == rows_dot) ? jacobi_oe_epl(n, rows_tot, batch) : 0;
+    {
         const int G = n_even / 2;
         const size_t lds_oe = (size_t)(G + 1) * (plain4_ld(e4) + 2) * sizeof(float);
         const int threads = ((G * 4 + 63) / 64) * 64;
-        if (e4 && threads <= 512 && lds_oe <= BASD_JACOBI_LDS_LIMIT) {
+        if (e4) {
 #define LAUNCH_OE(E)                                                                                                  \
     do {                                                                                                              \
         if (lds_oe > 48 * 1024)                                                                                       \
diff --git a/vit-inductive-bias-distillation_amd/csrc/jacobi_oe.h b/vit-inductive-bias-distillation_amd/csrc/jacobi_oe.h
--- /dev/null
+++ b/vit-inductive-bias-distillation_amd/csrc/jacobi_oe.h
@@ -0,0 +1,169 @@
+#pragma once
+#include "basd_common.h"
+
+namespace basd {
+
+constexpr float kNull2 = 2.2737368e-13f;
+
+struct Rot {
+    float c, s, t;
+    float h;
+    bool apply;
+    bool strong;
+};
+
+__device__ __forceinline__ Rot make_rotation(float alpha, float beta, float gamma, float tol) {
+    Rot r{1.f, 0.f, 0.f, 0.f, false, false};
+    const float cosv = gamma * __builtin_amdgcn_rsqf(alpha) * __builtin_amdgcn_rsqf(beta);
+    if (!(fabsf(cosv) > tol)) return r;
+    r.strong = cosv * cosv > tol;
+    const float zeta = (beta - alpha) * __builtin_amdgcn_rcpf(2.f * gamma);
+    const float az = fabsf(zeta);
+    float t = az > 1e8f ? 0.5f * __builtin_amdgcn_rcpf(az)
+                        : __builtin_amdgcn_rcpf(az + __builtin_amdgcn_sqrtf(fmaf(zeta, zeta, 1.f)));
+    t = copysignf(t, zeta);
+    r.t = t;
+    r.c = __builtin_amdgcn_rsqf(fmaf(t, t, 1.f));
+    r.s = r.c * t;
+    const float pc = r.c * r.c, ec = fmaf(r.c, r.c, -pc);
+    const float ps = r.s * r.s, es = fmaf(r.s, r.s, -ps);
+    r.h = 0.5f * ((((1.f - pc) - ps) - ec) - es);
+    r.apply = true;
+    return r;
+}
+
+template <int LPP>
+__device__ __forceinline__ float pair_allsum(float x) {
+    static_assert(LPP == 4 || LPP == 8 || LPP == 16 || LPP == 32 || LPP == 64,
+                  "a pair is owned by a quad, half a DPP row, a row, two rows or a wave");
+    if constexpr (LPP == 4 || LPP == 8) {
+        x += dpp_get<0xB1>(x);
+        x += dpp_get<0x4E>(x);
+        if constexpr (LPP == 8) x += dpp_get<0x141>(x);
+        return x;
+    } else if constexpr (LPP == 32) {
+        x = row16_allsum(x);
+        auto r = __builtin_amdgcn_permlane16_swap(__float_as_uint(x), __float_as_uint(x), false, false);
+        return __uint_as_float(r[0]) + __uint_as_float(r[1]);
+    } else {
+        return LPP == 16 ? row16_allsum(x) : wave64_allsum(x);
+    }
+}
+
+typedef float f32x2 __attribute__((ext_vector_type(2)));
+
+template <int H>
+__device__ __forceinline__ int rotate_regs(f32x2 (&x)[H], f32x2 (&y)[H], float& a, float& b, float& dx, float& dy,
+                                           float tol, float null2, float& norm2_max, bool forced) {
+    f32x2 acc = {0.f, 0.f};
+#pragma unroll
+    for (int i = 0; i < H; ++i) acc = __builtin_elementwise_fma(x[i], y[i], acc);
+    const float g = pair_allsum<4>(acc.x + acc.y);
+    norm2_max = fmaxf(norm2_max, fmaxf(a, b));
+    Rot rot{1.f, 0.f, 0.f, 0.f, false, false};
+    if (fminf(a, b) > null2) rot = make_rotation(a, b, g, tol);
+    float c = rot.c, s = rot.s;
+    if (forced) { c = 0.f; s = 1.f; }
+    if (rot.apply || forced) {
+        const f32x2 c2 = {c, c}, s2 = {s, s};
+#pragma unroll
+        for (int i = 0; i < H; ++i) {
+            const f32x2 xi = x[i], yi = y[i];
+            x[i] = __builtin_elementwise_fma(c2, xi, -(s2 * yi));
+            y[i] = __builtin_elementwise_fma(s2, xi, c2 * yi);
+        }
+    }
+    if (forced) {
+        b = a; a = 0.f; dy = dx; dx = 0.f;
+    } else if (rot.apply) {
+        a = fmaxf(a - rot.t * g, 0.f);
+        b = b + rot.t * g;
+        dx += rot.h;
+        dy += rot.h;
+    }
+    return rot.strong ? 3 : (rot.apply ? 1 : 0);
+}
+
+__host__ __device__ constexpr int jacobi_oe_ld(int epl) { return 4 * epl + (((4 * epl / 8) % 2 == 0) ? 8 : 0); }
+
+template <int EPL>
+__device__ __forceinline__ void jacobi_oe_clear(float* __restrict__ lds, int n) {
+    const int G = ((n + 1) & ~1) / 2;
+    for (int idx = threadIdx.x; idx < (G + 1) * (jacobi_oe_ld(EPL) + 2); idx += blockDim.x) lds[idx] = 0.f;
+}
+
+template <int EPL>
+__device__ __forceinline__ int jacobi_oe_sweeps(f32x2 (&x)[EPL / 2], f32x2 (&y)[EPL / 2], float& dx, float& dy,
+                                                float* lds, int n, int max_sweeps, float tol) {
+    static_assert(EPL % 2 == 0, "row chunks come in pairs");
+    constexpr int H = EPL / 2;
+    constexpr int LD = jacobi_oe_ld(EPL);
+    const int tid = threadIdx.x;
+    const int n_even = (n + 1) & ~1, G = n_even / 2;
+    float* mail_n2 = lds + (G + 1) * LD;
+    float* mail_dev = mail_n2 + (G + 1);
+    __shared__ int s_norm2_bits;
+    const int g = tid >> 2, gl = tid & 3;
+    const bool active = g < G, last = g == G - 1;
+    if (tid == 0) s_norm2_bits = 0;
+    float a = 0.f, b = 0.f;
+    dx = 0.f;
+    dy = 0.f;
+    float* slot_lo = lds + (active ? g : 0) * LD + 2 * gl;
+    float* slot_hi = lds + (active ? g + 1 : 0) * LD + 2 * gl;
+    __syncthreads();
+
+    float null2 = 0.f;
+    int sweep = 0;
+    for (; sweep < max_sweeps && n > 1; ++sweep) {
+        int rotated = 0;
+        float norm2_max = 0.f;
+        if (active) {
+            f32x2 sa = {0.f, 0.f}, sb = {0.f, 0.f};
+#pragma unroll
+            for (int i = 0; i < H; ++i) {
+                sa = __builtin_elementwise_fma(x[i], x[i], sa);
+                sb = __builtin_elementwise_fma(y[i], y[i], sb);
+            }
+            a = pair_allsum<4>(sa.x + sa.y);
+            b = pair_allsum<4>(sb.x + sb.y);
+        }
+        for (int dr = 0; dr < G; ++dr) {
+            if (active) {
+                rotated |= rotate_regs<H>(x, y, a, b, dx, dy, tol, null2, norm2_max, false);
+#pragma unroll
+                for (int i = 0; i < H; ++i) *(f32x2*)(slot_lo + 8 * i) = y[i];
+                if (gl == 0) { mail_n2[g] = b; mail_dev[g] = dy; }
+            }
+            __syncthreads();
+            if (active) {
+#pragma unroll
+                for (int i = 0; i < H; ++i) y[i] = *(const f32x2*)(slot_hi + 8 * i);
+                b = mail_n2[g + 1];
+                dy = mail_dev[g + 1];
+                rotated |= rotate_regs<H>(x, y, a, b, dx, dy, tol, null2, norm2_max, last);
+                if (!last) {
+#pragma unroll
+                    for (int i = 0; i < H; ++i) *(f32x2*)(slot_hi + 8 * i) = x[i];
+                    if (gl == 0) { mail_n2[g + 1] = a; mail_dev[g + 1] = dx; }
+                }
+            }
+            __syncthreads();
+            if (active) {
+#pragma unroll
+                for (int i = 0; i < H; ++i) x[i] = *(const f32x2*)(slot_lo + 8 * i);
+                a = mail_n2[g];
+                dx = mail_dev[g];
+            }
+        }
+        if (active && gl == 0 && norm2_max > 0.f) atomicMax(&s_norm2_bits, __float_as_int(norm2_max));
+        if (!__syncthreads_or(rotated & 2)) {
+            ++sweep;
+            break;
+        }
+        null2 = kNull2 * __int_as_float(s_norm2_bits);
+    }
+    return sweep;
+}
+
+}
diff --git a/vit-inductive-bias-distillation_amd/csrc/procrustes.hip b/vit-inductive-bias-distillation_amd/csrc/procrustes.hip
--- a/vit-inductive-bias-distillation_amd/csrc/procrustes.hip
+++ b/vit-inductive-bias-distillation_amd/csrc/procrustes.hip
@@ -1,4 +1,4 @@
-#include "basd_common.h"
+#include "jacobi_oe.h"
 #include "../../include/basd_hip.h"
 
 namespace basd {
@@ -1020,6 +1020,329 @@
     }
 }
 
+constexpr int PCF_EPL = 16, PCF_THREADS = 128, PCF_TPW = 5;
+
+__host__ __device__ inline int pcf_tri(int n) { return ((n * (n + 1) / 2) + 1) & ~1; }
+__host__ __device__ inline int pcf_ldz(int n) { return (n + 3) & ~3; }
+
+__global__ void __launch_bounds__(PCF_THREADS) __attribute__((amdgpu_waves_per_eu(5))) procrustes_core_fused_kernel(
+    const float* __restrict__ Ap, int n, int D, const double* __restrict__ Lb_all, long l_batch_stride, int GB,
+    int max_sweeps, float tol, float* __restrict__ sigma_out, int* __restrict__ sweeps_out, int n_s,
+    const double* __restrict__ Gt, long g_batch_stride, const float* __restrict__ omega, const int* __restrict__ tap0,
+    const int* __restrict__ tap1, const float* __restrict__ lam, const float* __restrict__ tr_s, int tr_slabs,
+    float* __restrict__ tr_s_out, float* __restrict__ tr_t_out, float* __restrict__ nuc_out,
+    float* __restrict__ loss_out, float* __restrict__ Kp) {
+    constexpr int H = PCF_EPL / 2;
+    extern __shared__ __attribute__((aligned(16))) double pcf_lds[];
+    __shared__ float sg[64];
+    __shared__ double redd[4];
+    const int b = blockIdx.x, tid = threadIdx.x, lane = tid & 63;
+    const int wave = __builtin_amdgcn_readfirstlane(tid >> 6);
+    const int T2 = pcf_tri(n), ldz = pcf_ldz(n);
+    double* lb_tri = pcf_lds;
+    double* la_tri = pcf_lds + T2;
+    float* tile = (float*)pcf_lds;
+    float* xz = (float*)la_tri;
+
+    const int nt = (n + 15) / 16, ntiles = nt * (nt + 1) / 2, rows_pad = nt * 16;
+    const float* Pb = Ap + (long)b * n * D;
+    f64x4 acc[PCF_TPW];
+    int ti[PCF_TPW], tj[PCF_TPW];
+#pragma unroll
+    for (int t = 0; t < PCF_TPW; ++t) {
+        acc[t] = f64x4{0., 0., 0., 0.};
+        const int lin = wave + 2 * t;
+        int r = 0;
+        if (lin < ntiles) {
+            while ((r + 1) * (r + 2) / 2 <= lin) ++r;
+            ti[t] = r;
+            tj[t] = lin - r * (r + 1) / 2;
+        } else {
+            ti[t] = -1;
+            tj[t] = -1;
+        }
+    }
+    const int i16 = lane & 15, kq = lane >> 4;
+    for (int k0 = 0; k0 < D; k0 += G64_BK) {
+        __syncthreads();
+        for (int idx = tid; idx < rows_pad * (G64_BK / 4); idx += PCF_THREADS) {
+            const int r = idx / (G64_BK / 4), c4 = (idx - r * (G64_BK / 4)) * 4, k = k0 + c4;
+            float4 v = make_float4(0.f, 0.f, 0.f, 0.f);
+            if (r < n) {
+                const float* p = Pb + (long)r * D + k;
+                if (k + 3 < D) {
+                    v = *(const float4*)p;
+                } else {
+                    if (k < D) v.x = p[0];
+                    if (k + 1 < D) v.y = p[1];
+                    if (k + 2 < D) v.z = p[2];
+                }
+            }
+            *(float4*)(tile + r * G64_LD + c4) = v;
+        }
+        __syncthreads();
+#pragma unroll
+        for (int g = 0; g < G64_BK / 16; ++g) {
+#pragma unroll
+            for (int t = 0; t < PCF_TPW; ++t) {
+                if (ti[t] < 0) continue;
+                const float4 a = *(const float4*)(tile + (ti[t] * 16 + i16) * G64_LD + g * 16 + 4 * kq);
+                const float4 bb = *(const float4*)(tile + (tj[t] * 16 + i16) * G64_LD + g * 16 + 4 * kq);
+                acc[t] = __builtin_amdgcn_mfma_f64_16x16x4f64((double)a.x, (double)bb.x, acc[t], 0, 0, 0);
+                acc[t] = __builtin_amdgcn_mfma_f64_16x16x4f64((double)a.y, (double)bb.y, acc[t], 0, 0, 0);
+                acc[t] = __builtin_amdgcn_mfma_f64_16x16x4f64((double)a.z, (double)bb.z, acc[t], 0, 0, 0);
+                acc[t] = __builtin_amdgcn_mfma_f64_16x16x4f64((double)a.w, (double)bb.w, acc[t], 0, 0, 0);
+            }
+        }
+    }
+    __syncthreads();
+#pragma unroll
+    for (int t = 0; t < PCF_TPW; ++t) {
+        if (ti[t] < 0) continue;
+        const int col = tj[t] * 16 + (lane & 15);
+#pragma unroll
+        for (int r = 0; r < 4; ++r) {
+            const int row = ti[t] * 16 + (lane >> 4) + 4 * r;
+            if (row < n && col <= row) la_tri[pk(row, col, n)] = acc[t][r];
+        }
+    }
+    const double* Lg = Lb_all + (long)(b % GB) * l_batch_stride;
+    for (int idx = tid; idx < n * n; idx += PCF_THREADS) {
+        const int i = idx / n, j = idx - i * n;
+        if (j <= i) lb_tri[pk(i, j, n)] = Lg[idx];
+    }
+    __syncthreads();
+
+    double dmax = 0.;
+    for (int i = 0; i < n; ++i) dmax = fmax(dmax, la_tri[pk(i, i, n)]);
+    const double thr = dmax * (double)n * 1e-15;
+    double piv_p = 0., inv_p = 0.;
+    for (int j = 0; j < n; ++j) {
+        const double d = la_tri[pk(j, j, n)];
+        const double piv = d > thr ? sqrt(d) : 0.;
+        const double inv = piv > 0. ? 1. / piv : 0.;
+        if (j > 0)
+            for (int i = j - 1 + tid; i < n; i += PCF_THREADS)
+                la_tri[pk(i, j - 1, n)] = (i == j - 1) ? piv_p : la_tri[pk(i, j - 1, n)] * inv_p;
+        if (piv > 0.) {
+            for (int k = j + 1 + wave; k < n; k += PCF_THREADS / 64) {
+                const double ck = la_tri[pk(k, j, n)] * inv;
+                for (int i = k + lane; i < n; i += 64) {
+                    const double ci = la_tri[pk(i, j, n)] * inv;
+                    la_tri[pk(i, k, n)] -= ci * ck;
+                }
+            }
+        }
+        piv_p = piv;
+        inv_p = inv;
+        __syncthreads();
+    }
+    if (tid == 0) la_tri[pk(n - 1, n - 1, n)] = piv_p;
+    __syncthreads();
+
+    const int n_even = (n + 1) & ~1, G = n_even / 2;
+    const int g = tid >> 2, gl = tid & 3;
+    const bool active = g < G;
+    const int c0 = 2 * g, c1 = 2 * g + 1;
+    f32x2 x[H], y[H];
+#pragma unroll
+    for (int i = 0; i < H; ++i) {
+        const int r = 2 * gl + 8 * i;
+        double m00 = 0., m01 = 0., m10 = 0., m11 = 0.;
+        if (active && r < n) {
+            for (int k = c0 > r ? c0 : r; k < n; ++k) {
+                const double a0 = la_tri[pk(k, c0, n)];
+                const double a1 = k >= c1 ? la_tri[pk(k, c1, n)] : 0.;
+                const double b0 = lb_tri[pk(k, r, n)];
+                const double b1 = k >= r + 1 ? lb_tri[pk(k, r + 1, n)] : 0.;
+                m00 = fma(a0, b0, m00);
+                m01 = fma(a0, b1, m01);
+                m10 = fma(a1, b0, m10);
+                m11 = fma(a1, b1, m11);
+            }
+        }
+        x[i] = f32x2{(float)m00, (float)m01};
+        y[i] = f32x2{(float)m10, (float)m11};
+    }
+    __syncthreads();
+    jacobi_oe_clear<PCF_EPL>((float*)la_tri, n);
+
+    float dx, dy;
+    const int sweep = jacobi_oe_sweeps<PCF_EPL>(x, y, dx, dy, (float*)la_tri, n, max_sweeps, tol);
+    if (sweeps_out && tid == 0) sweeps_out[b] = sweep;
+
+    f32x2 sa = {0.f, 0.f}, sb = {0.f, 0.f};
+#pragma unroll
+    for (int i = 0; i < H; ++i) {
+        sa = __builtin_elementwise_fma(x[i], x[i], sa);
+        sb = __builtin_elementwise_fma(y[i], y[i], sb);
+    }
+    const float na = sqrtf(pair_allsum<4>(sa.x + sa.y)), nb = sqrtf(pair_allsum<4>(sb.x + sb.y));
+    const bool rev = sweep & 1;
+    const int cx = rev ? n_even - 1 - 2 * g : 2 * g, cy = rev ? n_even - 2 - 2 * g : 2 * g + 1;
+    if (active && gl == 0) {
+        if (cx < n) sg[cx] = sigma_out[(long)b * n + cx] = fmaf(na, dx, na);
+        if (cy < n) sg[cy] = sigma_out[(long)b * n + cy] = fmaf(nb, dy, nb);
+    }
+    if (Kp && active) {
+#pragma unroll
+        for (int i = 0; i < H; ++i) {
+            const int r = 2 * gl + 8 * i;
+            if (cx < n && r < n) xz[cx * ldz + r] = fmaf(x[i].x, dx, x[i].x);
+            if (cx < n && r + 1 < n) xz[cx * ldz + r + 1] = fmaf(x[i].y, dx, x[i].y);
+            if (cy < n && r < n) xz[cy * ldz + r] = fmaf(y[i].x, dy, y[i].x);
+            if (cy < n && r + 1 < n) xz[cy * ldz + r + 1] = fmaf(y[i].y, dy, y[i].y);
+        }
+    }
+    __syncthreads();
+    float smax = 0.f;
+    for (int j = 0; j < n; ++j) smax = fmaxf(smax, sg[j]);
+    const float nuc = wave64_allsum(lane < n ? sg[lane] : 0.f);
+    const int bt = b % GB;
+    const double* Gq = Gt + (long)bt * g_batch_stride;
+    double part = 0., part_hi = 0.;
+    for (int s = tid; s < n_s; s += 256) {
+        const double w = (double)omega[(long)bt * n_s + s];
+        if (tap0) {
+            const int i0 = tap0[s], i1 = tap1[s];
+            const double l1 = (double)lam[s], l0 = 1. - l1;
+            part += w * (l0 * l0 * Gq[(long)i0 * n + i0] + 2. * l0 * l1 * Gq[(long)i0 * n + i1] + l1 * l1 * Gq[(long)i1 * n + i1]);
+        } else {
+            part += w * Gq[(long)s * n + s];
+        }
+    }
+    for (int s = tid + PCF_THREADS; s < n_s; s += 256) {
+        const double w = (double)omega[(long)bt * n_s + s];
+        if (tap0) {
+            const int i0 = tap0[s], i1 = tap1[s];
+            const double l1 = (double)lam[s], l0 = 1. - l1;
+            part_hi += w * (l0 * l0 * Gq[(long)i0 * n + i0] + 2. * l0 * l1 * Gq[(long)i0 * n + i1] + l1 * l1 * Gq[(long)i1 * n + i1]);
+        } else {
+            part_hi += w * Gq[(long)s * n + s];
+        }
+    }
+    part = wave_sum(part);
+    part_hi = wave_sum(part_hi);
+    if (lane == 0) {
+        redd[wave] = part;
+        redd[2 + wave] = part_hi;
+    }
+    __syncthreads();
+    if (tid == 0) {
+        double trt = 0.;
+        for (int i = 0; i < 4; ++i) trt += redd[i];
+        float trs = 0.f;
+        for (int k = 0; k < tr_slabs; ++k) trs += tr_s[(long)b * tr_slabs + k];
+        tr_s_out[b] = trs;
+        tr_t_out[b] = (float)trt;
+        nuc_out[b] = nuc;
+        loss_out[b] = trs + (float)trt - 2.f * nuc;
+    }
+    if (!Kp) return;
+
+    const float thr_s = smax * (float)n * 1.1920929e-7f;
+    const float* X0 = xz + (cx < n ? cx : 0) * ldz;
+    const float* X1 = xz + (cy < n ? cy : 0) * ldz;
+#pragma unroll
+    for (int i = 0; i < H; ++i) {
+        const int a = 2 * gl + 8 * i;
+        float z00 = 0.f, z01 = 0.f, z10 = 0.f, z11 = 0.f;
+        if (active && a < n) {
+            const int rmax = a + 1 < n ? a + 1 : a;
+            for (int r = 0; r <= rmax; ++r) {
+                const float l0 = r <= a ? (float)lb_tri[pk(a, r, n)] : 0.f;
+                const float l1 = a + 1 < n ? (float)lb_tri[pk(a + 1, r, n)] : 0.f;
+                const float w0 = X0[r], w1 = X1[r];
+                z00 = fmaf(l0, w0, z00);
+                z01 = fmaf(l1, w0, z01);
+                z10 = fmaf(l0, w1, z10);
+                z11 = fmaf(l1, w1, z11);
+            }
+        }
+        x[i] = f32x2{z00, z01};
+        y[i] = f32x2{z10, z11};
+    }
+    float fx = 0.f, fy = 0.f;
+    if (cx < n) {
+        const float sv = sg[cx];
+        fx = sv > thr_s ? 1.f / (sv * sqrtf(sv)) : 0.f;
+    }
+    if (cy < n) {
+        const float sv = sg[cy];
+        fy = sv > thr_s ? 1.f / (sv * sqrtf(sv)) : 0.f;
+    }
+    __syncthreads();
+    if (active) {
+#pragma unroll
+        for (int i = 0; i < H; ++i) {
+            const int a = 2 * gl + 8 * i;
+            if (cx < n && a < ldz) xz[cx * ldz + a] = x[i].x * fx;
+            if (cx < n && a + 1 < ldz) xz[cx * ldz + a + 1] = x[i].y * fx;
+            if (cy < n && a < ldz) xz[cy * ldz + a] = y[i].x * fy;
+            if (cy < n && a + 1 < ldz) xz[cy * ldz + a + 1] = y[i].y * fy;
+        }
+    }
+    __syncthreads();
+    float* K = Kp + (long)b * n * n;
+    const int nq = ldz / 4;
+    for (int q = tid; q < nq * nq; q += PCF_THREADS) {
+        const int qa = q / nq, qb = q - qa * nq;
+        float kacc[4][4];
+#pragma unroll
+        for (int u = 0; u < 4; ++u)
+#pragma unroll
+            for (int v = 0; v < 4; ++v) kacc[u][v] = 0.f;
+        for (int c = 0; c < n; ++c) {
+            const float4 va = *(const float4*)(xz + c * ldz + 4 * qa);
+            const float4 vb = *(const float4*)(xz + c * ldz + 4 * qb);
+            const float za[4] = {va.x, va.y, va.z, va.w}, zb[4] = {vb.x, vb.y, vb.z, vb.w};
+#pragma unroll
+            for (int u = 0; u < 4; ++u)
+#pragma unroll
+                for (int v = 0; v < 4; ++v) kacc[u][v] = fmaf(za[u], zb[v], kacc[u][v]);
+        }
+#pragma unroll
+        for (int u = 0; u < 4; ++u)
+#pragma unroll
+            for (int v = 0; v < 4; ++v) {
+                const int ra = 4 * qa + u, rb = 4 * qb + v;
+                if (ra < n && rb < n) K[(long)ra * n + rb] = kacc[u][v];
+            }
+    }
+}
+
+static size_t pcf_lds_bytes(int n) {
+    const size_t tri = (size_t)n * (n + 1) / 2 * sizeof(double);
+    const int G = ((n + 1) & ~1) / 2;
+    const size_t mail = (size_t)(G + 1) * (jacobi_oe_ld(PCF_EPL) + 2) * sizeof(float);
+    const size_t xz = (size_t)n * pcf_ldz(n) * sizeof(float);
+    size_t region = tri > mail ? tri : mail;
+    if (xz > region) region = xz;
+    const size_t lds = (size_t)pcf_tri(n) * sizeof(double) + region;
+    const size_t chunk = (size_t)((n + 15) / 16) * 16 * G64_LD * sizeof(float);
+    return lds > chunk ? lds : chunk;
+}
+
+bool procrustes_core_fused_fits(int n, int d_s, int batch, const float* a_prime) {
+    return n <= 64 && jacobi_oe_epl(n, n, batch) == PCF_EPL && d_s > 0 && d_s % 4 == 0 &&
+           ((uintptr_t)a_prime & 15) == 0;
+}
+
+int procrustes_core_fused(const float* a_prime, int n, int d_s, int batch, const double* lb, long l_batch_stride,
+                          int lb_period, int max_sweeps, float* sigma, int* sweeps, int n_s, const double* gt,
+                          long g_batch_stride, const float* omega, const int* tap0, const int* tap1, const float* lam,
+                          const float* tr_part, int tr_slabs, float* tr_s, float* tr_t, float* nuc, float* loss,
+                          float* k_prime, hipStream_t stream) {
+    BASD_CHECK_ARG(a_prime && lb && sigma && gt && omega && tr_part && tr_s && tr_t && nuc && loss && batch > 0 &&
+                   lb_period > 0 && max_sweeps > 0 && tr_slabs > 0);
+    if (!procrustes_core_fused_fits(n, d_s, batch, a_prime)) return BASD_EUNSUPPORTED;
+    const float tol = 1.2e-7f * sqrtf((float)n);
+    procrustes_core_fused_kernel<<<batch, PCF_THREADS, pcf_lds_bytes(n), stream>>>(
+        a_prime, n, d_s, lb, l_batch_stride, lb_period, max_sweeps, tol, sigma, sweeps, n_s, gt, g_batch_stride, omega,
+        tap0, tap1, lam, tr_part, tr_slabs, tr_s, tr_t, nuc, loss, k_prime);
+    BASD_RETURN_LAST();
+}
+
 __global__ void __launch_bounds__(256) kprime_tiled_kernel(const float* __restrict__ W, long w_batch_stride,
                                                            const float* __restrict__ sigma, int n,
                                                            float* __restrict__ Kp) {
```

Result: slower. 149,100 images/s, median of 2 (-11.3%).
